# IwakuraRein/CIS-565-Final-VR-Raytracer

Hardware: AMD Instinct MI355X
Metric: Mrays/s (ClosestHit+AnyHit ray queries per second) of the 1080p ReSTIR DI+GI+denoise frame; ms_per_step = ms/frame (higher is better)
Workload: dtype f32

## Files before the change

cis-565-final-vr-raytracer_amd/csrc/dev_scene.h:

```cpp
#pragma once
#include <hip/hip_runtime.h>
#include "bvh8.h"
#include "../../include/rt_abi.h"

namespace rt {

struct DevInstance {
  float o2w[12];
  float w2o[12];
  uint32_t primMesh;
  uint32_t flags;
  uint32_t pad[2];
};

struct DevTexture {
  const uint8_t* bgra;
  int32_t w, h, wrapS, wrapT, filter, pad;
};

struct DevScene {
  const Node8* nodes;
  const Tri48* tris;
  const TriRef* triRef;
  const AlphaRec* alphaRec;
  const AlphaRec* alphaByTri;
  const DevInstance* instances;
  const rt_prim_mesh* primMeshes;
  const rt_vertex* vertices;
  const uint32_t* indices;
  const rt_material* materials;
  const DevTexture* textures;
  const rt_punc_light* puncLights;
  const rt_trig_light* trigLights;
  const float* env;
  const rt_impt_samp* envAccel;
  rt_light_buf_info lightInfo;
  int32_t envW, envH;
  uint32_t numTris, numNodes;
  const struct SkyPre* sky;
  int32_t stackEntries;
  int32_t coopLive;
  float triPad;
  int32_t stackTotal;
  uint2* stackOvf; uint2* stackOvfInd;
  uint32_t stackOvfThreads;
  int32_t gangMax;
};

struct SurfRec {
  rt_vec3 position, normal, ffnormal, emission;
  float roughness, metallic;
  uint32_t matID, seed;
};

struct DevFrame {
  uint4* thisG; const uint4* lastG;
  short2* motion;
  rt_direct_reservoir* thisDirectResv; const rt_direct_reservoir* lastDirectResv;
  rt_indirect_reservoir* thisIndirectResv; const rt_indirect_reservoir* lastIndirectResv;
  uint32_t* thisLightId; const uint32_t* lastLightId;
  float4* thisDirectResult; float4* thisIndirectResult;
  float4* denoiseDirA; float4* denoiseDirB; float4* denoiseIndA; float4* denoiseIndB;
  unsigned long long* counters;
  SurfRec* surf; uint32_t* status; uint32_t* qcount; uint32_t* waveProf;
  float4* geomN; float4* geomP; float4* geomNh; float4* geomPh;
  rt_direct_reservoir* tempDirectResv;
  double* postRowSums; float* postMean;
  float4* postMipD; float4* postMipI;
  uint32_t* tileOrder;
  int32_t W, H;
  int32_t histRow0, histRow1;
  uint32_t* histMiss;
  int32_t stackLds;
  int32_t pad4;
};

struct OmCamera {
  rt_mat4 lastProjView;
  rt_vec3 lastPosition; float pad;
};
struct DevObjMotion {
  uint32_t* instImage;
  const OmCamera* cams;
  uint32_t numInst, pad;
};

}
```

cis-565-final-vr-raytracer_amd/csrc/rt_api.cpp:

```cpp
#include <hip/hip_runtime.h>
#include <array>
#include <atomic>
#include <memory>
#include <mutex>
#include <cmath>
#include <cstdio>
#include <map>
#include <cstdlib>
#include <chrono>
#include <cstring>
#include <string>
#include <thread>
#include <unordered_map>
#include <vector>
#include "../../include/rt_abi.h"
#include "../../include/rt_cpus.h"
#include "bvh8_builder.h"
#include "stages.h"
#include "reference.h"
#include "svgf.h"
#include "gi_spatial.h"
#include "taa.h"
#include "refit.h"
#include "accel_build.h"
// ... 304 lines not shown
  return e;
}

template <class T> static int upload(rt_ctx* c, std::vector<void*>& pool, const T* src, size_t count, const T** out)
{
  void* d = nullptr;
  size_t bytes = std::max<size_t>(count, 1) * sizeof(T);
  RT_HIP(c, hipMalloc(&d, bytes));
  pool.push_back(d);
  if(count && src) RT_HIP(c, hipMemcpy(d, src, count * sizeof(T), hipMemcpyHostToDevice));
  else RT_HIP(c, hipMemset(d, 0, bytes));
  *out = static_cast<const T*>(d);
  return RT_OK;
}
template <class T> static int allocZeroed(rt_ctx* c, std::vector<void*>& pool, size_t count, T** out)
{
  const T* const noSource = nullptr;
  const T* p = nullptr;
  const int rc = upload(c, pool, noSource, count, &p);
  *out = const_cast<T*>(p);
  return rc;
}
static void freePool(std::vector<void*>& pool) { for(void* p : pool) (void)hipFree(p); pool.clear(); }
struct LoadTimer {
  const bool on = getenv("RESTIR_BVH_TIMING") && atoi(getenv("RESTIR_BVH_TIMING")) != 0;
  std::chrono::steady_clock::time_point t = std::chrono::steady_clock::now();
  void lap(const char* what) { if(!on) return; const auto n = std::chrono::steady_clock::now(); fprintf(stderr, "[scene load] %-34s %.3f s\n", what, std::chrono::duration<double>(n - t).count()); t = n; }
};
static int ensureStackOverflow(rt_ctx* c);
static int syncHostVertices(rt_ctx* c, int mesh = -1);
static int allocObjectMotion(rt_ctx* c);
static void reopenPriorityDecision(rt_ctx* c);
static void hashBytes(const void* p, size_t n, uint64_t& h0, uint64_t& h1);
static int stackLdsEnv() { static const int v = getenv("RESTIR_STACK_LDS") ? std::max(2, atoi(getenv("RESTIR_STACK_LDS"))) : 0; return v; }
static int stackLdsMin() { return stackLdsEnv() ? stackLdsEnv() : 6; }

static size_t elemBytes(int id)
{
  switch(id) {
    case RT_BUF_GBUFFER0: case RT_BUF_GBUFFER1: return 16;
    case RT_BUF_MOTION: return 4;
    case RT_BUF_DIRECT_RESV0: case RT_BUF_DIRECT_RESV1: case RT_BUF_DIRECT_RESV_TEMP: return sizeof(rt_direct_reservoir);
    case RT_BUF_INDIRECT_RESV0: case RT_BUF_INDIRECT_RESV1: case RT_BUF_INDIRECT_RESV_TEMP: return sizeof(rt_indirect_reservoir);
    case RT_BUF_LIGHT_ID0: case RT_BUF_LIGHT_ID1: case RT_BUF_LDR: return 4;
    default: return 16;
  }
}
#ifndef RT_WAVEPROF
#define RT_WAVEPROF 0
#endif
static constexpr size_t WAVEPROF_RECORDS = 1 << 17;
static constexpr int RT_PAD_ROWS = 128;
static bool halfRes(int id) { return id == RT_BUF_INDIRECT_RESV0 || id == RT_BUF_INDIRECT_RESV1 || id == RT_BUF_INDIRECT_RESV_TEMP; }

extern "C" {

uint32_t rt_abi_version(void) { return (RT_ABI_VERSION_MAJOR << 16) | RT_ABI_VERSION_MINOR; }

const char* rt_last_error(rt_ctx* ctx) { return ctx ? ctx->err.c_str() : g_createErr.c_str(); }

}
int rtCreateWithLevels(rt_ctx** out, int device, const int* levels);
extern "C" {
int rt_create(rt_ctx** out, int device) { return rtCreateWithLevels(out, device, nullptr); }
}
int rtCreateWithLevels(rt_ctx** out, int device, const int* levels)
{
  if(!out) { g_createErr = "rt_create: out is NULL"; return RT_ERR_INVALID_ARG; }
  *out = nullptr;
  int n = 0;
  if(hipGetDeviceCount(&n) != hipSuccess || n <= 0) { g_createErr = "rt_create: no HIP device (this library has no CPU path)"; return RT_ERR_NO_DEVICE; }
  if(device < 0 || device >= n) { g_createErr = "rt_create: device index out of range"; return RT_ERR_INVALID_ARG; }
  if(hipSetDevice(device) != hipSuccess) { g_createErr = "rt_create: hipSetDevice failed"; return RT_ERR_HIP; }
  rt_ctx* c = new(std::nothrow) rt_ctx();
  if(!c) { g_createErr = "rt_create: out of host memory"; return RT_ERR_OOM; }
  g_liveCtx.fetch_add(1);
  c->device = device;
  {
    prioSpec(c->prio); c->prioFromEnv = getenv("RESTIR_PRIO") != nullptr; c->prioDecided = c->prioFromEnv;
    if(levels) { for(int i = 0; i < 3; i++) c->prio[i] = std::max(-1, std::min(1, levels[i])); c->prioDecided = c->prioExplicit = true; }
    bool ok = createStreamLevel(&c->ownStream, c->prio[0]) == hipSuccess;
    if(!ok) { g_createErr = "rt_create: hipStreamCreate failed"; rt_destroy(c); return RT_ERR_HIP; }
    c->mainIdx = g_streamsCreated.load() - 1;
    c->stream = c->ownStream;
    for(int i = 0; i < 4; i++) {
      ok = ok && hipEventCreateWithFlags(&c->evD[i], hipEventDisableTiming) == hipSuccess;
      ok = ok && hipEventCreateWithFlags(&c->evI[i], hipEventDisableTiming) == hipSuccess;
      ok = ok && hipEventCreateWithFlags(&c->evDone[i], hipEventDisableTiming) == hipSuccess;
    }
    ok = ok && hipEventCreateWithFlags(&c->evFork, hipEventDisableTiming) == hipSuccess;
    ok = ok && hipEventCreateWithFlags(&c->evJoin, hipEventDisableTiming) == hipSuccess;
    if(!ok) { g_createErr = "rt_create: creating the internal events failed"; rt_destroy(c); return RT_ERR_HIP; }
  }
  if(const char* e = getenv("RESTIR_OVERLAP")) c->overlap = atoi(e);
  if(hipMalloc(reinterpret_cast<void**>(&c->dCounters), 8 * sizeof(unsigned long long)) != hipSuccess) { g_createErr = "rt_create: hipMalloc failed"; rt_destroy(c); return RT_ERR_OOM; }
  (void)hipMemset(c->dCounters, 0, 8 * sizeof(unsigned long long));
  *out = c;
  return RT_OK;
}

extern "C" {

int rt_destroy(rt_ctx* c)
{
  if(!c) return RT_ERR_INVALID_ARG;
  (void)hipSetDevice(c->device);
  (void)syncAll(c);
  freePool(c->sceneAllocs); freePool(c->accelAllocs); freePool(c->scratchAllocs); freePool(c->ovfAllocs); freePool(c->rebuildAllocs);
  freePool(c->skinAllocs); freePool(c->deformAllocs);
  for(int i = 0; i < RT_BUF_COUNT; i++) if(c->bufs[i]) (void)hipFree(c->bufs[i]);
  for(void* p : {c->spareG, c->spareMotion, c->spareG2, c->spareMotion2, c->spareDirRes, c->omInst, c->omInstSpare, c->omInstSpare2, c->omTable}) if(p) (void)hipFree(p);
  for(void* p : c->indA) if(p && p != c->bufs[RT_BUF_DENOISE_IND_A]) (void)hipFree(p);
  for(hipStream_t& q : c->indStreams) { if(q) (void)hipStreamDestroy(q); q = nullptr; }
  for(hipStream_t& q : c->sideStreams) { if(q) (void)hipStreamDestroy(q); q = nullptr; }
  c->indStream = c->sideStream = nullptr;
  if(c->indStream) (void)hipStreamDestroy(c->indStream);
  for(int i = 0; i < 4; i++) { if(c->evD[i]) (void)hipEventDestroy(c->evD[i]); if(c->evI[i]) (void)hipEventDestroy(c->evI[i]); if(c->evDone[i]) (void)hipEventDestroy(c->evDone[i]); }
  if(c->dCounters) (void)hipFree(c->dCounters);
  if(c->dSky) (void)hipFree(c->dSky);
  if(c->dPick) (void)hipFree(c->dPick);
  if(c->refAcc) (void)hipFree(c->refAcc);
  if(c->refMean) (void)hipFree(c->refMean);
  freeSvgfHistory(c);
  freeGiSpatial(c);
  freeTaaHistory(c);
  for(auto& E : c->evSets) for(int i = 0; i < rt_ctx::MAX_EV; i++) (void)hipEventDestroy(E.ev[i]);
  if(c->ownStream) (void)hipStreamDestroy(c->ownStream);
  if(c->sideStream) (void)hipStreamDestroy(c->sideStream);
  if(c->evFork) (void)hipEventDestroy(c->evFork);
  if(c->evJoin) (void)hipEventDestroy(c->evJoin);
  for(hipEvent_t e : c->evRefit) if(e) (void)hipEventDestroy(e);
  for(hipEvent_t e : c->evDeform) if(e) (void)hipEventDestroy(e);
  for(hipEvent_t e : c->evRebuild) if(e) (void)hipEventDestroy(e);
  delete c;
  if(g_liveCtx.fetch_sub(1) == 1) { std::lock_guard<std::mutex> one(g_accelMutex); g_accelCache.reset(); }
  return RT_OK;
}

int rt_set_stream(rt_ctx* c, void* s)
{
  if(!c) return RT_ERR_INVALID_ARG;
  c->stream = s ? static_cast<hipStream_t>(s) : c->ownStream;
  return RT_OK;
}

int rt_sync(rt_ctx* c)
{
  if(!c) return RT_ERR_INVALID_ARG;
  RT_HIP(c, hipSetDevice(c->device));
  RT_HIP(c, syncAll(c));
  return RT_OK;
}

int rt_upload_scene(rt_ctx* c, const rt_scene_desc* d)
{
  if(!c) return RT_ERR_INVALID_ARG;
  if(!d || !d->primMeshes || !d->vertices || !d->indices || !d->instances || !d->materials || d->numMaterials == 0)
    return fail(c, RT_ERR_INVALID_ARG, "rt_upload_scene: missing geometry/material arrays");
  for(uint32_t i = 0; i < d->numInstances; i++)
    if(d->instances[i].primMesh >= d->numPrimMeshes) return fail(c, RT_ERR_INVALID_ARG, "rt_upload_scene: instance references a missing prim mesh");
  for(uint32_t i = 0; i < d->numPrimMeshes; i++) {
    const rt_prim_mesh& pm = d->primMeshes[i];
    if(uint64_t(pm.firstIndex) + pm.indexCount > d->numIndices || uint64_t(pm.vertexOffset) + pm.vertexCount > d->numVertices || pm.indexCount % 3 != 0)
      return fail(c, RT_ERR_INVALID_ARG, "rt_upload_scene: prim mesh range out of bounds");
    if(pm.materialIndex >= int32_t(d->numMaterials)) return fail(c, RT_ERR_INVALID_ARG, "rt_upload_scene: material index out of range");
    for(uint32_t k = 0; k < pm.indexCount; k++)
      if(d->indices[pm.firstIndex + k] >= pm.vertexCount) return fail(c, RT_ERR_INVALID_ARG, "rt_upload_scene: vertex index beyond the prim mesh's vertex range");
  }
  const int32_t nTex = d->textures ? int32_t(d->numTextures) : 0;
  for(uint32_t i = 0; i < d->numMaterials; i++) {
    const rt_material& m = d->materials[i];
    const int32_t ids[5] = {m.pbrBaseColorTexture, m.pbrMetallicRoughnessTexture, m.emissiveTexture, m.normalTexture, m.transmissionTexture};
    for(int32_t id : ids)
      if(id < -1 || id >= nTex) return fail(c, RT_ERR_INVALID_ARG, "rt_upload_scene: material references a missing texture");
  }
  if(d->trigLights)
    for(uint32_t i = 0; i < d->lightInfo.trigLightSize; i++)
      if(d->trigLights[i].matIndex >= d->numMaterials || d->trigLights[i].impSamp.alias < 0 || uint32_t(d->trigLights[i].impSamp.alias) >= d->lightInfo.trigLightSize)
        return fail(c, RT_ERR_INVALID_ARG, "rt_upload_scene: triangle light with a bad material or alias index");
  if(d->puncLights)
    for(uint32_t i = 0; i < d->lightInfo.puncLightSize; i++)
      if(d->puncLights[i].impSamp.alias < 0 || uint32_t(d->puncLights[i].impSamp.alias) >= d->lightInfo.puncLightSize)
        return fail(c, RT_ERR_INVALID_ARG, "rt_upload_scene: punctual light with a bad alias index");
  if(d->envRgba32f && d->envAccel && d->envWidth > 0 && d->envHeight > 0) {
    const int64_t n = int64_t(d->envWidth) * d->envHeight;
    for(int64_t i = 0; i < n; i++)
      if(d->envAccel[i].alias < 0 || d->envAccel[i].alias >= n) return fail(c, RT_ERR_INVALID_ARG, "rt_upload_scene: environment alias table entry out of range");
  }
  RT_HIP(c, hipSetDevice(c->device));
  RT_HIP(c, syncAll(c));
  LoadTimer lt;
  freePool(c->sceneAllocs); freePool(c->accelAllocs); freePool(c->rebuildAllocs);
  freePool(c->skinAllocs); freePool(c->deformAllocs);
  c->deform = rt_ctx::Deform{};
  c->refit = rt_ctx::Refit{};
  c->rebuild = rt_ctx::Rebuild{};
  c->haveScene = c->haveAccel = false;
  c->refN = 0;
  c->svgfValid = false;
  c->taaValid = false;
  c->omPrev.clear(); c->omMoved.clear(); c->omPending = false;
  c->ds = DevScene{};
  c->ds.sky = (c->sunAndSky.in_use == 1) ? static_cast<const SkyPre*>(c->dSky) : nullptr;
  c->primMeshes.assign(d->primMeshes, d->primMeshes + d->numPrimMeshes);
  c->vertices.assign(d->vertices, d->vertices + d->numVertices);
  c->indices.assign(d->indices, d->indices + d->numIndices);
  c->instances.assign(d->instances, d->instances + d->numInstances);
  c->materials.assign(d->materials, d->materials + d->numMaterials);

  int rc;
  if((rc = upload(c, c->sceneAllocs, d->primMeshes, d->numPrimMeshes, &c->ds.primMeshes))) return rc;
  if((rc = upload(c, c->sceneAllocs, d->vertices, size_t(d->numVertices), &c->ds.vertices))) return rc;
  if((rc = upload(c, c->sceneAllocs, d->indices, size_t(d->numIndices), &c->ds.indices))) return rc;
  if((rc = upload(c, c->sceneAllocs, d->materials, d->numMaterials, &c->ds.materials))) return rc;
  if((rc = upload(c, c->sceneAllocs, d->puncLights, d->puncLights ? d->lightInfo.puncLightSize : 0, &c->ds.puncLights))) return rc;
  if((rc = upload(c, c->sceneAllocs, d->trigLights, d->trigLights ? d->lightInfo.trigLightSize : 0, &c->ds.trigLights))) return rc;
  c->ds.lightInfo = d->lightInfo;
  if(!d->puncLights) c->ds.lightInfo.puncLightSize = 0;
  if(!d->trigLights) c->ds.lightInfo.trigLightSize = 0;
  lt.lap("geometry copies + uploads");
  c->hostAlpha.clear();
  std::vector<const uint8_t*> alphaSrc;
  std::vector<DevTexture> texs(std::max<uint32_t>(d->numTextures, 1));
  static const uint8_t white[4] = {255, 255, 255, 255};
  for(uint32_t i = 0; i < uint32_t(texs.size()); i++) {
    rt_texture t{white, 1, 1, RT_WRAP_REPEAT, RT_WRAP_REPEAT, RT_FILTER_LINEAR, 0};
    if(i < d->numTextures && d->textures && d->textures[i].bgra8 && d->textures[i].width > 0 && d->textures[i].height > 0) t = d->textures[i];
    const uint8_t* dp = nullptr;
    if((rc = upload(c, c->sceneAllocs, t.bgra8, size_t(t.width) * t.height * 4, &dp))) return rc;
    texs[i] = DevTexture{dp, t.width, t.height, t.wrapS, t.wrapT, t.magFilter, 0};
    c->hostAlpha.emplace_back(size_t(t.width) * t.height);
    alphaSrc.push_back(t.bgra8);
  }
  lt.lap("texture uploads");
  {
    c->alphaHash.assign(c->hostAlpha.size(), {0ull, 0ull});
    std::atomic<size_t> next{0};
    auto work = [&] {
      for(;;) {
        const size_t i = next.fetch_add(1);
        if(i >= c->hostAlpha.size()) return;
        std::vector<uint8_t>& a = c->hostAlpha[i];
        const uint8_t* src = alphaSrc[i];
        for(size_t k = 0; k < a.size(); k++) a[k] = src[k * 4 + 3];
        uint64_t h0 = 0x243F6A8885A308D3ull, h1 = 0x13198A2E03707344ull;
        hashBytes(a.data(), a.size(), h0, h1);
        c->alphaHash[i] = {h0, h1};
      }
    };
    const size_t nt = std::min<size_t>(c->hostAlpha.size(), size_t(rt_cpu_budget()));
    std::vector<std::thread> pool;
    for(size_t k = 1; k < nt; k++) pool.emplace_back(work);
    work();
    for(auto& th : pool) th.join();
  }
  lt.lap("alpha planes + hashes");
  if((rc = upload(c, c->sceneAllocs, texs.data(), texs.size(), &c->ds.textures))) return rc;
  c->devTextures = texs;
  if(d->envRgba32f && d->envWidth > 0 && d->envHeight > 0) {
    const size_t n = size_t(d->envWidth) * d->envHeight;
    if((rc = upload(c, c->sceneAllocs, d->envRgba32f, n * 4, &c->ds.env))) return rc;
    if(d->envAccel) { if((rc = upload(c, c->sceneAllocs, d->envAccel, n, &c->ds.envAccel))) return rc; }
    else {
      std::vector<rt_impt_samp> a(n, rt_impt_samp{0, 1.0f, 0.0f, 0.0f});
      if((rc = upload(c, c->sceneAllocs, a.data(), n, &c->ds.envAccel))) return rc;
    }
    c->ds.envW = d->envWidth; c->ds.envH = d->envHeight;
  } else {
    const float black[4] = {0, 0, 0, 0};
    const rt_impt_samp one{0, 1.0f, 0.0f, 0.0f};
    if((rc = upload(c, c->sceneAllocs, black, 4, &c->ds.env))) return rc;
    if((rc = upload(c, c->sceneAllocs, &one, 1, &c->ds.envAccel))) return rc;
    c->ds.envW = c->ds.envH = 1;
  }
  RT_HIP(c, hipDeviceSynchronize());
  c->haveScene = true;
  reopenPriorityDecision(c);
  return RT_OK;
}


static void hashBytes(const void* p, size_t n, uint64_t& h0, uint64_t& h1)
{
  const unsigned char* b = static_cast<const unsigned char*>(p);
  size_t i = 0;
  for(; i + 8 <= n; i += 8) {
    uint64_t w; memcpy(&w, b + i, 8);
    h0 = (h0 ^ w) * 0x9E3779B97F4A7C15ull; h0 ^= h0 >> 29;
    h1 = (h1 + w) * 0xC2B2AE3D27D4EB4Full; h1 ^= h1 >> 31;
  }
  uint64_t w = 0; memcpy(&w, b + i, n - i); w |= uint64_t(n) << 56;
  h0 = (h0 ^ w) * 0x9E3779B97F4A7C15ull; h0 ^= h0 >> 29;
  h1 = (h1 + w) * 0xC2B2AE3D27D4EB4Full; h1 ^= h1 >> 31;
}
#define RT_HASH_VEC(v) do { const uint64_t n_ = (v).size(); hashBytes(&n_, 8, h0, h1); if(n_) hashBytes((v).data(), n_ * sizeof((v)[0]), h0, h1); } while(0)
static void sceneKey(const rt_ctx* c, uint64_t& h0, uint64_t& h1)
{
  h0 = 0x243F6A8885A308D3ull; h1 = 0x13198A2E03707344ull;
  RT_HASH_VEC(c->primMeshes); RT_HASH_VEC(c->vertices); RT_HASH_VEC(c->indices); RT_HASH_VEC(c->instances); RT_HASH_VEC(c->materials);
  for(size_t i = 0; i < c->devTextures.size(); i++) {
    const DevTexture& t = c->devTextures[i];
    const int meta[5] = {t.w, t.h, t.wrapS, t.wrapT, t.filter};
    hashBytes(meta, sizeof(meta), h0, h1);
    if(i < c->alphaHash.size()) { const uint64_t n_ = c->hostAlpha[i].size(); hashBytes(&n_, 8, h0, h1); hashBytes(c->alphaHash[i].data(), 16, h0, h1); }
  }
  for(const char* name : {"RESTIR_BVH_SPLIT", "RESTIR_BVH_SPLIT_BUDGET", "RESTIR_BVH_SPLIT_ALPHA", "RESTIR_BVH_SPLIT_WORK", "RESTIR_BVH_ROTATE", "RESTIR_BVH_ROTATE_GG",
                           "RESTIR_BVH_REINSERT", "RESTIR_BVH_PAR_MIN", "RESTIR_BVH_SEQ_MAX"}) {
    const char* v = getenv(name);
    hashBytes(name, strlen(name), h0, h1);
    if(v) hashBytes(v, strlen(v) + 1, h0, h1);
  }
}
#undef RT_HASH_VEC
static int buildHostAccel(rt_ctx* c, HostAccel& out)
{
  LoadTimer lt;
  rt_scene_desc d{};
  d.numPrimMeshes = uint32_t(c->primMeshes.size()); d.primMeshes = c->primMeshes.data();
  d.numVertices = c->vertices.size(); d.vertices = c->vertices.data();
  d.numIndices = c->indices.size(); d.indices = c->indices.data();
  d.numInstances = uint32_t(c->instances.size()); d.instances = c->instances.data();
  BuildOutput& bo = out.bo;
  int threads = rt_cpu_budget();
  if(!buildBvh8(d, bo, threads > 0 ? threads : 1)) return fail(c, RT_ERR_INVALID_ARG, "rt_build_accel: BVH8 build failed");
  if(bo.maxDepth > STACK_MAX) {
    bo = BuildOutput{};
    if(!buildBvh8(d, bo, threads > 0 ? threads : 1, true)) return fail(c, RT_ERR_INVALID_ARG, "rt_build_accel: BVH8 build failed");
  }
  if(bo.maxDepth > STACK_MAX) return fail(c, RT_ERR_INVALID_ARG, "rt_build_accel: BVH8 deeper than the traversal stack");
  lt.lap("buildBvh8");
  std::vector<AlphaRec>& alpha = out.alpha; alpha.assign(1, AlphaRec{});
  std::vector<int32_t>& alphaTex = out.alphaTex; alphaTex.assign(1, -1);
  struct KeyHash { size_t operator()(const std::array<uint32_t, 12>& k) const { uint64_t h = 1469598103934665603ull; for(uint32_t w : k) { h ^= w; h *= 1099511628211ull; } return size_t(h ^ (h >> 29)); } };
  std::unordered_map<std::array<uint32_t, 12>, std::array<uint32_t, 4>, KeyHash> ommCache;
  ommCache.reserve(1 << 16);
  std::vector<uint32_t> alphaOf;
  if(bo.tris.size() > bo.triRef.size()) alphaOf.assign(bo.triRef.size(), 0u);
  std::vector<std::array<uint32_t, 4>> ommOf;
  for(Tri48& T : bo.tris) {
    if(T.flags & TRI_OPAQUE) continue;
    if(!alphaOf.empty() && alphaOf[T.globalId]) { T.alphaIdx = alphaOf[T.globalId]; memcpy(T.omm, ommOf[T.alphaIdx].data(), sizeof(T.omm)); continue; }
    const TriRef ref = bo.triRef[T.globalId];
    const rt_prim_mesh& pm = c->primMeshes[c->instances[ref.inst].primMesh];
    const rt_material& m = c->materials[size_t(pm.materialIndex > 0 ? pm.materialIndex : 0)];
    const uint32_t* ix = &c->indices[pm.firstIndex + 3 * ref.prim];
    AlphaRec a{};
    int32_t tex = -1;
    const rt_vec2 t0 = c->vertices[pm.vertexOffset + ix[0]].texcoord, t1 = c->vertices[pm.vertexOffset + ix[1]].texcoord, t2 = c->vertices[pm.vertexOffset + ix[2]].texcoord;
    a.uv0x = t0.x; a.uv0y = t0.y; a.uv1x = t1.x; a.uv1y = t1.y; a.uv2x = t2.x; a.uv2y = t2.y;
    a.baseAlpha = m.pbrBaseColorFactor.w; a.cutoff = m.alphaCutoff; a.alphaMode = m.alphaMode;
    if(m.pbrBaseColorTexture > -1 && size_t(m.pbrBaseColorTexture) < c->devTextures.size()) {
      const DevTexture& t = c->devTextures[size_t(m.pbrBaseColorTexture)];
      tex = m.pbrBaseColorTexture; a.w = t.w; a.h = t.h; a.wrapS = t.wrapS; a.wrapT = t.wrapT; a.filter = t.filter;
    }
    T.alphaIdx = uint32_t(alpha.size());
    alpha.push_back(a); alphaTex.push_back(tex);
    std::array<uint32_t, 12> key{};
    memcpy(key.data(), &a.uv0x, 8 * sizeof(float));
    key[8] = uint32_t(m.pbrBaseColorTexture); key[9] = uint32_t(a.alphaMode); key[10] = uint32_t(a.wrapS) ^ (uint32_t(a.wrapT) << 16); key[11] = uint32_t(a.filter);
    auto it = ommCache.find(key);
    if(it == ommCache.end()) {
      std::array<uint32_t, 4> o{};
      const std::vector<uint8_t>* al = (tex >= 0 && size_t(tex) < c->hostAlpha.size()) ? &c->hostAlpha[size_t(m.pbrBaseColorTexture)] : nullptr;
      buildOpacityMap(a, al, o.data());
      it = ommCache.emplace(key, o).first;
    }
    memcpy(T.omm, it->second.data(), sizeof(T.omm));
    if(!alphaOf.empty()) { alphaOf[T.globalId] = T.alphaIdx; ommOf.resize(alpha.size()); ommOf[T.alphaIdx] = it->second; }
  }
  lt.lap("alpha records + micro-maps");
  return RT_OK;
}

int rt_build_accel(rt_ctx* c)
{
  if(!c) return RT_ERR_INVALID_ARG;
  if(!c->haveScene) return fail(c, RT_ERR_NO_SCENE, "rt_build_accel: no scene uploaded");
  RT_HIP(c, hipSetDevice(c->device));
  RT_HIP(c, syncAll(c));
  { const int rc = syncHostVertices(c); if(rc) return rc; }
  freePool(c->accelAllocs); freePool(c->rebuildAllocs);
  c->refit = rt_ctx::Refit{};
  c->rebuild = rt_ctx::Rebuild{};
  c->haveAccel = false;
  c->refN = 0;
  c->svgfValid = false;
  c->taaValid = false;
  std::shared_ptr<const HostAccel> ha;
  LoadTimer lt;
  {
    std::lock_guard<std::mutex> one(g_accelMutex);
    uint64_t k0, k1;
    sceneKey(c, k0, k1);
    lt.lap("scene key");
    if(g_accelCache && g_accelCache->key0 == k0 && g_accelCache->key1 == k1) ha = g_accelCache;
    else {
      auto fresh = std::make_shared<HostAccel>();
      fresh->key0 = k0; fresh->key1 = k1;
      const int rc = buildHostAccel(c, *fresh);
      if(rc) return rc;
      ha = fresh; g_accelCache = ha;
    }
  }
  lt.lap("host products (build or cache)");
  const BuildOutput& bo = ha->bo;
  int rc;
  {
    std::vector<AlphaRec> alpha = ha->alpha;
    for(size_t i = 0; i < alpha.size(); i++) if(ha->alphaTex[i] >= 0) alpha[i].bgra = c->devTextures[size_t(ha->alphaTex[i])].bgra;
    if((rc = upload(c, c->accelAllocs, alpha.data(), alpha.size(), &c->ds.alphaRec))) return rc;
    std::vector<AlphaRec> byTri(bo.tris.size(), AlphaRec{});
    for(size_t i = 0; i < bo.tris.size(); i++) if(!(bo.tris[i].flags & TRI_OPAQUE)) byTri[i] = alpha[bo.tris[i].alphaIdx];
    if((rc = upload(c, c->accelAllocs, byTri.data(), byTri.size(), &c->ds.alphaByTri))) return rc;
  }
  if((rc = upload(c, c->accelAllocs, bo.nodes.data(), bo.nodes.size(), &c->ds.nodes))) return rc;
  if((rc = upload(c, c->accelAllocs, bo.tris.data(), bo.tris.size(), &c->ds.tris))) return rc;
  if((rc = upload(c, c->accelAllocs, bo.triRef.data(), bo.triRef.size(), &c->ds.triRef))) return rc;
  if((rc = upload(c, c->accelAllocs, bo.instances.data(), bo.instances.size(), &c->ds.instances))) return rc;
  c->ds.numNodes = uint32_t(bo.nodes.size()); c->ds.numTris = uint32_t(bo.tris.size());
  c->ds.stackTotal = std::max(8, ((bo.maxDepth + 1 + 3) / 4) * 4);
  c->ds.stackEntries = c->ds.stackTotal;
  c->ds.triPad = bo.pad;
  { const char* e = getenv("RESTIR_COOP"); c->ds.coopLive = e ? std::max(0, std::min(64, atoi(e))) : 4; }
  { const char* e = getenv("RESTIR_GANG"); c->ds.gangMax = e ? std::max(0, std::min(7, atoi(e))) : 4; }
  c->numNodes = bo.nodes.size(); c->numTris = bo.triRef.size(); c->maxDepth = bo.maxDepth;
  c->numRefs = bo.tris.size(); c->spatialSplits = size_t(bo.spatialSplits); c->sahNodeSteps = bo.sahNodeSteps; c->sahTriSteps = bo.sahTriSteps;
  RT_HIP(c, hipDeviceSynchronize());
  lt.lap("uploads (tree, alpha records)");
  c->haveAccel = true;
  reopenPriorityDecision(c);
  return ensureStackOverflow(c);
}

int rt_resize(rt_ctx* c, int w, int h)
{
  if(!c) return RT_ERR_INVALID_ARG;
  if(w <= 0 || h <= 0 || w > 32767 || h > 32767) return fail(c, RT_ERR_INVALID_ARG, "rt_resize: size must be in 1..32767 (RG16_SINT motion vectors)");
  RT_HIP(c, hipSetDevice(c->device));
  RT_HIP(c, syncAll(c));
  reopenPriorityDecision(c);
  for(void*& p : c->indA) { if(p && p != c->bufs[RT_BUF_DENOISE_IND_A]) (void)hipFree(p); p = nullptr; }
  for(int i = 0; i < RT_BUF_COUNT; i++) { if(c->bufs[i]) (void)hipFree(c->bufs[i]); c->bufs[i] = nullptr; c->bufBytes[i] = 0; }
  for(void** p : {&c->spareG, &c->spareMotion, &c->spareG2, &c->spareMotion2, &c->spareDirRes}) if(*p) { (void)hipFree(*p); *p = nullptr; }
  c->W = c->H = 0;
  for(void* p : {static_cast<void*>(c->refAcc), static_cast<void*>(c->refMean)}) if(p) (void)hipFree(p);
  c->refAcc = nullptr; c->refMean = nullptr; c->refN = 0;
  freeSvgfHistory(c);
  freeGiSpatial(c);
  freeTaaHistory(c);
  freeObjectMotion(c);
  const size_t n = size_t(w) * h, nh = size_t(w / 2) * (h / 2);
  for(int i = 0; i < RT_BUF_COUNT; i++) {
    const size_t bytes = (halfRes(i) ? nh : n) * elemBytes(i);
    const size_t alloc = bytes + (halfRes(i) ? size_t(w / 2) * (RT_PAD_ROWS / 2) : size_t(w) * RT_PAD_ROWS) * elemBytes(i) + 16;
    RT_HIP(c, hipMalloc(&c->bufs[i], alloc));
    RT_HIP(c, hipMemset(c->bufs[i], (i == RT_BUF_LIGHT_ID0 || i == RT_BUF_LIGHT_ID1) ? 0xff : 0, alloc));
    c->bufBytes[i] = bytes; c->bufAlloc[i] = alloc;
    if(i == RT_BUF_DENOISE_IND_A) {
      c->indA[0] = c->bufs[i];
      RT_HIP(c, hipMalloc(&c->indA[1], alloc));
      RT_HIP(c, hipMemset(c->indA[1], 0, alloc));
    }
    if(i == RT_BUF_GBUFFER0 || i == RT_BUF_MOTION) {
      for(void** spare : {(i == RT_BUF_MOTION) ? &c->spareMotion : &c->spareG, (i == RT_BUF_MOTION) ? &c->spareMotion2 : &c->spareG2}) {
        RT_HIP(c, hipMalloc(spare, alloc));
        RT_HIP(c, hipMemset(*spare, 0, alloc));
      }
    }
    if(i == RT_BUF_DIRECT_RESULT0) {
      RT_HIP(c, hipMalloc(&c->spareDirRes, alloc));
      RT_HIP(c, hipMemset(c->spareDirRes, 0, alloc));
    }
  }
  freePool(c->scratchAllocs);
  c->scratch = DevFrame{};
  auto alloc = [&](size_t bytes, void** out) -> int {
    RT_HIP(c, hipMalloc(out, std::max<size_t>(bytes, 256)));
    c->scratchAllocs.push_back(*out);
    RT_HIP(c, hipMemset(*out, 0, std::max<size_t>(bytes, 256)));
    return RT_OK;
  };
  DevFrame& X = c->scratch;
  int rc;
#define RT_SCRATCH(field, count, T) if((rc = alloc(size_t(count) * sizeof(T), reinterpret_cast<void**>(&X.field)))) return rc
  RT_SCRATCH(surf, n, SurfRec); RT_SCRATCH(status, n, uint32_t); RT_SCRATCH(qcount, 256, uint32_t);
  RT_SCRATCH(geomN, n, float4); RT_SCRATCH(geomP, n, float4); RT_SCRATCH(geomNh, nh, float4); RT_SCRATCH(geomPh, nh, float4);
  RT_SCRATCH(postRowSums, size_t(h) * 6, double); RT_SCRATCH(postMean, 8, float);
  RT_SCRATCH(postMipD, n + 64, float4); RT_SCRATCH(postMipI, n + 64, float4);
  RT_SCRATCH(tileOrder, (size_t(w / 2 + 7) / 8) * (size_t(h / 2 + 7) / 8 + 16 * 2) + 64 + 4096, uint32_t);
#if RT_WAVEPROF
  RT_SCRATCH(waveProf, WAVEPROF_RECORDS * 16, uint32_t);
#endif
#undef RT_SCRATCH
  RT_HIP(c, hipDeviceSynchronize());
  c->W = w; c->H = h;
  if(c->objMotion != RT_OBJECT_MOTION_OFF && (rc = allocObjectMotion(c))) return rc;
  return ensureStackOverflow(c);
}

static int ensureStackOverflow(rt_ctx* c)
{
  freePool(c->ovfAllocs);
  c->ds.stackOvf = c->ds.stackOvfInd = nullptr; c->ds.stackOvfThreads = 0;
  if(!(stackLdsEnv() || c->overlap >= 2)) return RT_OK;
  if(!c->haveAccel || c->W <= 0 || c->ds.stackTotal <= stackLdsMin()) return RT_OK;
  const size_t tilesX = size_t(c->W + 7) / 8, tilesY = size_t(c->H + 7) / 8;
  const size_t blocks = std::max<size_t>(16384, tilesX * tilesY + 8 * tilesX + 1024);
  const size_t bytes = blocks * 64 * size_t(c->ds.stackTotal - stackLdsMin()) * sizeof(uint2);
  void* p[2] = {nullptr, nullptr};
  for(int i = 0; i < 2; i++) { RT_HIP(c, hipMalloc(&p[i], bytes)); c->ovfAllocs.push_back(p[i]); }
  c->ds.stackOvf = static_cast<uint2*>(p[0]); c->ds.stackOvfInd = static_cast<uint2*>(p[1]);
  c->ds.stackOvfThreads = uint32_t(blocks * 64);
  return RT_OK;
}

int rt_set_camera(rt_ctx* c, const rt_scene_camera* cam)
{
  if(!c || !cam) return RT_ERR_INVALID_ARG;
  if(std::memcmp(&c->cam.viewInverse, &cam->viewInverse, sizeof(rt_mat4)) != 0 || std::memcmp(&c->cam.projInverse, &cam->projInverse, sizeof(rt_mat4)) != 0) c->refN = 0;
  c->cam = *cam;
  return RT_OK;
}

static void selectFrame(rt_ctx* c, int frames) { if(c->indA[0]) c->bufs[RT_BUF_DENOISE_IND_A] = c->indA[frames & 1]; }

static hipError_t ensureOverlapStreams(rt_ctx* c)
{
  if(c->sideStream && c->indStream) return hipSuccess;
  hipError_t e = hipSuccess;
  hipStream_t& side = c->sideStreams[c->prio[2] + 1];
  hipStream_t& ind = c->indStreams[c->prio[1] + 1];
  if(!side) { e = createStreamLevel(&side, c->prio[2]); if(e == hipSuccess) c->sideIdx[c->prio[2] + 1] = g_streamsCreated.load() - 1; }
  if(e == hipSuccess && !ind) { e = createStreamLevel(&ind, c->prio[1]); if(e == hipSuccess) c->indIdx[c->prio[1] + 1] = g_streamsCreated.load() - 1; }
  c->sideStream = side; c->indStream = ind;
  return e;
}

static constexpr float PRIO_FILTER_SHARE = 0.30f;
static int prioProbeFrames() { static const int n = getenv("RESTIR_PRIO_PROBE") ? std::max(1, atoi(getenv("RESTIR_PRIO_PROBE"))) : 3; return n; }
static void reopenPriorityDecision(rt_ctx* c)
{
  if(c->prioExplicit || c->prioFromEnv) return;
  c->prioDecided = false; c->filterShare = -1.f; c->probeFrames = 0; c->denoiseSeen = -1;
  c->prio[1] = 1; c->prio[2] = 0;
  c->indStream = c->sideStream = nullptr;
}

static int allocSvgfHistory(rt_ctx* c)
{
  const size_t n = size_t(c->W) * c->H, nh = size_t(c->W / 2) * (c->H / 2);
  const size_t bytes[4] = {n * sizeof(float4), nh * sizeof(float4), n * sizeof(float2), nh * sizeof(float2)};
  for(auto& par : c->svgfHist)
    for(int k = 0; k < 4; k++) {
      if(hipMalloc(&par[k], std::max<size_t>(bytes[k], 256)) != hipSuccess) { par[k] = nullptr; freeSvgfHistory(c); return fail(c, RT_ERR_OOM, "rt_render_frame: hipMalloc of the SVGF history failed"); }
      RT_HIP(c, hipMemset(par[k], 0, std::max<size_t>(bytes[k], 256)));
    }
  RT_HIP(c, hipDeviceSynchronize());
  c->svgfValid = false; c->svgfParity = -1;
  return RT_OK;
}

static SvgfArgs svgfArgs(const rt_ctx* c, const DevFrame& F, const rt_state& st, int frames, bool ind, bool histValid)
{
  SvgfArgs A{};
  const int cur = frames & 1, prev = (frames + 1) & 1, k = ind ? 1 : 0;
  A.thisG = F.thisG; A.lastG = F.lastG; A.motion = F.motion;
  A.noisy = ind ? F.denoiseIndA : F.thisDirectResult;
  A.bufA = ind ? F.thisIndirectResult : F.denoiseDirA;
  A.bufB = ind ? F.denoiseIndA : F.denoiseDirB;
  A.out = ind ? F.denoiseIndB : F.thisDirectResult;
  A.geomN = ind ? F.geomNh : F.geomN; A.geomP = ind ? F.geomPh : F.geomP;
  A.prevC = static_cast<const float4*>(c->svgfHist[prev][k]); A.prevM = static_cast<const float2*>(c->svgfHist[prev][2 + k]);
  A.histC = static_cast<float4*>(c->svgfHist[cur][k]); A.histM = static_cast<float2*>(c->svgfHist[cur][2 + k]);
  A.W = c->W; A.H = c->H;
  A.bx = ind ? c->W / 2 : c->W; A.by = ind ? c->H / 2 : c->H;
  A.histValid = histValid ? 1 : 0;
  A.cap = c->den.historyCap;
  A.alphaC = c->den.alphaColor; A.alphaM = c->den.alphaMoments;
  A.phiLum = ind ? c->den.phiLumIndirect : c->den.phiLumDirect;
  A.sigN = ind ? st.sigNormalIndirect : st.sigNormalDirect;
  A.sigD = ind ? st.sigDepthIndirect : st.sigDepthDirect;
  return A;
}

static int allocGiSpatial(rt_ctx* c)
{
  const size_t bytes = std::max<size_t>(size_t(c->W / 2) * (c->H / 2) * sizeof(rt_indirect_reservoir), 256);
  if(hipMalloc(&c->gisResv, bytes) != hipSuccess) { c->gisResv = nullptr; return fail(c, RT_ERR_OOM, "rt_render_frame: hipMalloc of the GI spatial reservoirs failed"); }
  RT_HIP(c, hipMemset(c->gisResv, 0, bytes));
  RT_HIP(c, hipDeviceSynchronize());
  c->gisWritten = false;
  return RT_OK;
}

static GiSpatialArgs giSpatialArgs(const rt_ctx* c, const DevFrame& F)
{
  GiSpatialArgs A{};
  A.thisG = F.thisG; A.resv = F.thisIndirectResv;
  A.out = static_cast<rt_indirect_reservoir*>(c->gisResv);
  A.indA = F.denoiseIndA;
  A.W = c->W; A.H = c->H;
  A.mode = c->gis.mode; A.samples = c->gis.samples; A.radius = c->gis.radius;
  A.normalThreshold = c->gis.normalThreshold; A.depthThreshold = c->gis.depthThreshold; A.jacobianMax = c->gis.jacobianMax;
  return A;
}

static int allocObjectMotion(rt_ctx* c)
{
  const size_t bytes = size_t(c->W) * c->H * sizeof(uint32_t);
  for(void** p : {&c->omInst, &c->omInstSpare, &c->omInstSpare2}) {
    if(*p) continue;
    RT_HIP(c, hipMalloc(p, std::max<size_t>(bytes, 256)));
    RT_HIP(c, hipMemset(*p, 0xff, std::max<size_t>(bytes, 256)));
  }
  RT_HIP(c, hipDeviceSynchronize());
  return RT_OK;
}
static int allocTaaHistory(rt_ctx* c)
{
  const size_t n = size_t(c->W) * c->H;
  const size_t bytes[3] = {n * sizeof(float4), n * sizeof(float4), n * sizeof(float)};
  for(auto& par : c->taaHist)
    for(int k = 0; k < 3; k++) {
      if(hipMalloc(&par[k], std::max<size_t>(bytes[k], 256)) != hipSuccess) { par[k] = nullptr; freeTaaHistory(c); return fail(c, RT_ERR_OOM, "rt_render_frame: hipMalloc of the TAA history failed"); }
      RT_HIP(c, hipMemset(par[k], 0, std::max<size_t>(bytes[k], 256)));
    }
  RT_HIP(c, hipDeviceSynchronize());
  c->taaValid = false; c->taaLast = -1; c->taaHeld[0] = c->taaHeld[1] = false;
  return RT_OK;
}

static TaaArgs taaArgs(const rt_ctx* c, const DevFrame& F, int frames, bool histValid)
{
  TaaArgs A{};
  const int cur = frames & 1, prev = (frames + 1) & 1;
  A.thisG = F.thisG; A.lastG = F.lastG;
  A.curD = F.thisDirectResult; A.curI = F.thisIndirectResult;
  A.prevD = static_cast<const float4*>(c->taaHist[prev][0]); A.prevI = static_cast<const float4*>(c->taaHist[prev][1]);
  A.prevN = static_cast<const float*>(c->taaHist[prev][2]);
  A.outD = static_cast<float4*>(c->taaHist[cur][0]); A.outI = static_cast<float4*>(c->taaHist[cur][1]); A.outN = static_cast<float*>(c->taaHist[cur][2]);
  A.W = c->W; A.H = c->H;
  A.histValid = histValid ? 1 : 0;
  A.alpha = c->taa.alpha; A.clipGamma = c->taa.clipGamma;
  return A;
}

static DevFrame makeFrame(rt_ctx* c, int frames)
{
  selectFrame(c, frames);
  const int cur = frames & 1, last = (frames + 1) & 1;
  DevFrame F{};
  F.stackLds = stackLdsEnv() ? stackLdsEnv() : (c->overlap >= 2 ? 6 : 0);
  F.thisG = static_cast<uint4*>(c->bufs[RT_BUF_GBUFFER0 + cur]); F.lastG = static_cast<const uint4*>(c->bufs[RT_BUF_GBUFFER0 + last]);
  F.motion = static_cast<short2*>(c->bufs[RT_BUF_MOTION]);
  F.thisDirectResv = static_cast<rt_direct_reservoir*>(c->bufs[RT_BUF_DIRECT_RESV0 + cur]);
  F.lastDirectResv = static_cast<const rt_direct_reservoir*>(c->bufs[RT_BUF_DIRECT_RESV0 + last]);
  F.thisIndirectResv = static_cast<rt_indirect_reservoir*>(c->bufs[RT_BUF_INDIRECT_RESV0 + cur]);
  F.lastIndirectResv = static_cast<const rt_indirect_reservoir*>(c->bufs[RT_BUF_INDIRECT_RESV0 + last]);
  F.tempDirectResv = static_cast<rt_direct_reservoir*>(c->bufs[RT_BUF_DIRECT_RESV_TEMP]);
  F.thisLightId = static_cast<uint32_t*>(c->bufs[RT_BUF_LIGHT_ID0 + cur]); F.lastLightId = static_cast<const uint32_t*>(c->bufs[RT_BUF_LIGHT_ID0 + last]);
  F.thisDirectResult = static_cast<float4*>(c->bufs[RT_BUF_DIRECT_RESULT0 + cur]);
  F.thisIndirectResult = static_cast<float4*>(c->bufs[RT_BUF_INDIRECT_RESULT0 + cur]);
  F.denoiseDirA = static_cast<float4*>(c->bufs[RT_BUF_DENOISE_DIR_A]); F.denoiseDirB = static_cast<float4*>(c->bufs[RT_BUF_DENOISE_DIR_B]);
  F.denoiseIndA = static_cast<float4*>(c->bufs[RT_BUF_DENOISE_IND_A]); F.denoiseIndB = static_cast<float4*>(c->bufs[RT_BUF_DENOISE_IND_B]);
  F.counters = c->counting ? c->dCounters : nullptr;
  F.W = c->W; F.H = c->H;
  const DevFrame& X = c->scratch;
  F.surf = X.surf; F.status = X.status; F.qcount = X.qcount; F.waveProf = X.waveProf;
  F.histRow0 = c->histRow0; F.histRow1 = c->histRow1; F.histMiss = X.qcount + 250;
  F.geomN = X.geomN; F.geomP = X.geomP; F.geomNh = X.geomNh; F.geomPh = X.geomPh; F.tileOrder = X.tileOrder; F.postRowSums = X.postRowSums; F.postMean = X.postMean;
  return F;
}

static int checkReady(rt_ctx* c, const rt_state* st)
{
  if(!c || !st) return RT_ERR_INVALID_ARG;
  if(!c->haveScene) return fail(c, RT_ERR_NO_SCENE, "no scene uploaded");
  if(!c->haveAccel) return fail(c, RT_ERR_NO_ACCEL, "rt_build_accel has not been called");
  if(c->W == 0 || st->size.x != c->W || st->size.y != c->H) return fail(c, RT_ERR_NO_TARGET, "RtxState.size does not match rt_resize");
  return RT_OK;
}

int rt_run_stage(rt_ctx* c, const rt_state* st, int frames, int stage, int level, int rowBegin, int rowEnd)
{
  int rc = checkReady(c, st);
  if(rc) return rc;
  if(stage < 0 || stage >= RT_STAGE_COUNT) return fail(c, RT_ERR_INVALID_ARG, "rt_run_stage: unknown stage");
  if(c->den.mode == RT_DENOISER_SVGF && (stage == RT_STAGE_DENOISE_DIRECT || stage == RT_STAGE_DENOISE_INDIRECT))
    return fail(c, RT_ERR_INVALID_ARG, "rt_run_stage: the denoise stages are the A-Trous chain; this context is in SVGF mode (rt_set_denoiser), which only rt_render_frame runs");
  if(c->gis.mode != RT_GI_SPATIAL_OFF && stage == RT_STAGE_INDIRECT)
    return fail(c, RT_ERR_INVALID_ARG, "rt_run_stage: this context has GI spatial reuse on (rt_set_gi_spatial), whose pass after the indirect stage only rt_render_frame runs");
  if(c->taa.mode != RT_TAA_OFF)
    return fail(c, RT_ERR_INVALID_ARG, "rt_run_stage: this context has TAA on (rt_set_taa), whose jittered camera and resolve pass only rt_render_frame runs");
  if(rowBegin < 0 || (rowBegin & 7)) return fail(c, RT_ERR_INVALID_ARG, "rt_run_stage: rowBegin must be a non-negative multiple of 8");
  {
    const bool spatial = st->ReSTIRState == RT_RESTIR_SPATIAL || st->ReSTIRState == RT_RESTIR_SPATIOTEMPORAL;
    const int maxLevel = stage == RT_STAGE_DENOISE_DIRECT ? 3 : (stage == RT_STAGE_DENOISE_INDIRECT ? 4 : ((stage == RT_STAGE_DIRECT && spatial) ? 2 : 0));
    if(level < 0 || level > maxLevel)
      return fail(c, RT_ERR_INVALID_ARG, "rt_run_stage: level out of range for this stage (RT_STAGE_DIRECT levels 1 / 2 exist in the spatial modes only)");
  }
  RT_HIP(c, hipSetDevice(c->device));
  RT_HIP(c, joinInFlight(c));
  DevFrame F = makeFrame(c, frames);
  if(stage == RT_STAGE_INDIRECT) F.histMiss = c->scratch.qcount + 251;
  const hipError_t e = stageLauncher(c, *st, stage, rowBegin, rowEnd)(c->stream, c->ds, F, *st, c->cam, stage, level, rowBegin, rowEnd);
  if(e == hipErrorInvalidValue) return fail(c, RT_ERR_INVALID_ARG, "rt_run_stage: level out of range for this stage (RT_STAGE_DIRECT levels 1 / 2 exist in the spatial modes only)");
  if(e == hipErrorInvalidConfiguration) return fail(c, RT_ERR_HIP, "rt_run_stage: the traversal-stack overflow area is missing or too small for this launch (internal sizing error)");
  RT_HIP(c, e);
  return RT_OK;
}

int rt_render_frame(rt_ctx* c, const rt_state* st, int frames)
{
  int rc = checkReady(c, st);
  if(rc) return rc;
  RT_HIP(c, hipSetDevice(c->device));
  if(c->evUsed == rt_ctx::MAX_SETS) { RT_HIP(c, syncAll(c)); harvestTimings(c); }
  if(c->evUsed == c->evSets.size()) {
    rt_ctx::EvSet E{};
    for(int i = 0; i < rt_ctx::MAX_EV; i++) RT_HIP(c, hipEventCreate(&E.ev[i]));
    c->evSets.push_back(E);
  }
  if(c->prioDecided && !c->prioExplicit && !c->prioFromEnv && c->denoiseSeen >= 0 && (st->denoise > 0) != (c->denoiseSeen > 0)) { RT_HIP(c, syncAll(c)); reopenPriorityDecision(c); }
  const bool svgf = c->den.mode == RT_DENOISER_SVGF && st->denoise > 0;
  if(svgf && !c->svgfHist[0][0]) { RT_HIP(c, syncAll(c)); if((rc = allocSvgfHistory(c))) return rc; }
  const bool gis = c->gis.mode != RT_GI_SPATIAL_OFF;
  if(gis && !c->gisResv) { RT_HIP(c, syncAll(c)); if((rc = allocGiSpatial(c))) return rc; }
  const bool taa = c->taa.mode == RT_TAA_ON && st->debugging_mode == 0;
  if(taa && !c->taaHist[0][0]) { RT_HIP(c, syncAll(c)); if((rc = allocTaaHistory(c))) return rc; }
  rt_scene_camera cam = c->cam;
  if(taa) (void)rt_taa_jitter_camera(&c->cam, frames, c->taa.jitterPhases, c->W, c->H, &cam);
  const bool om = c->objMotion == RT_OBJECT_MOTION_ON && !c->counting && c->omInst;
  bool omMotion = false;
  if(c->objMotion == RT_OBJECT_MOTION_ON) {
    const size_t nInst = c->instances.size();
    if(c->omPending) for(size_t i = 0; i < nInst && !omMotion; i++) omMotion = c->omMoved[i] && std::memcmp(c->omPrev[i].data(), c->instances[i].objectToWorld, 48) != 0;
    if(omMotion && c->counting)
      return fail(c, RT_ERR_INVALID_ARG, "rt_render_frame: instances are in motion with object motion vectors on (rt_set_object_motion) and counting on (rt_set_counting): the counting build has no object-motion form");
    if(omMotion) {
      if(c->omTableRows < nInst) {
        RT_HIP(c, syncAll(c));
        if(c->omTable) { (void)hipFree(c->omTable); c->omTable = nullptr; c->omTableRows = 0; }
        RT_HIP(c, hipMalloc(&c->omTable, nInst * sizeof(OmCamera)));
        c->omTableRows = nInst;
      }
      c->omHost.resize(nInst);
      for(size_t i = 0; i < nInst; i++) {
        rt_scene_camera ci = cam;
        if(c->omMoved[i]) (void)rt_object_motion_camera(&cam, c->omPrev[i].data(), c->instances[i].objectToWorld, &ci);
        c->omHost[i].lastProjView = ci.lastProjView; c->omHost[i].lastPosition = ci.lastPosition; c->omHost[i].pad = 0.f;
      }
    }
  }
  const bool decide = c->overlap >= 2 && !c->prioDecided && c->spareG && c->spareMotion;
  if(decide) { RT_HIP(c, syncAll(c)); harvestTimings(c); }
  const double tracedBefore = c->accStage[RT_STAGE_DIRECT] + c->accStage[RT_STAGE_INDIRECT];
  const double filterBefore = c->accStage[RT_STAGE_DENOISE_DIRECT] + c->accStage[RT_STAGE_DENOISE_INDIRECT] + c->accStage[RT_STAGE_COMPOSE];
  rt_ctx::EvSet& E = c->evSets[c->evUsed];
  if(c->overlap >= 1 && !decide) RT_HIP(c, ensureOverlapStreams(c));
  const bool pipelined = !decide && c->overlap >= 2 && c->sideStream && c->indStream && c->spareG && c->spareMotion;
  if(pipelined) {
    if(c->overlap >= 3 && c->spareG2 && c->spareMotion2 && c->spareDirRes) {
      void*& g = c->bufs[RT_BUF_GBUFFER0 + (frames & 1)]; void* t = g; g = c->spareG; c->spareG = c->spareG2; c->spareG2 = t;
      void*& m = c->bufs[RT_BUF_MOTION]; t = m; m = c->spareMotion; c->spareMotion = c->spareMotion2; c->spareMotion2 = t;
      if(c->omInst) { t = c->omInst; c->omInst = c->omInstSpare; c->omInstSpare = c->omInstSpare2; c->omInstSpare2 = t; }
      std::swap(c->bufs[RT_BUF_DIRECT_RESULT0 + (frames & 1)], c->spareDirRes);
    } else {
      std::swap(c->bufs[RT_BUF_GBUFFER0 + (frames & 1)], c->spareG);
      std::swap(c->bufs[RT_BUF_MOTION], c->spareMotion);
      if(c->omInst) std::swap(c->omInst, c->omInstSpare);
    }
  } else {
    RT_HIP(c, joinInFlight(c));
  }
  const DevFrame F = makeFrame(c, frames);
  const DevObjMotion OM{static_cast<uint32_t*>(c->omInst), omMotion ? static_cast<const OmCamera*>(c->omTable) : nullptr, uint32_t(c->instances.size()), 0u};
  int k = 0, lastMain = 0, lastSide = 0, lastInd = 0;
  auto record = [&](hipStream_t strm, int stage) -> int {
    const hipError_t e = hipEventRecord(E.ev[k], strm);
    if(e != hipSuccess) { c->err = std::string("hipEventRecord: ") + hipGetErrorString(e); return RT_ERR_HIP; }
    int& last = (strm == c->stream) ? lastMain : (strm == c->indStream ? lastInd : lastSide);
    E.stage[k] = stage; E.prev[k] = last; last = k; k++;
    return RT_OK;
  };
  auto run = [&](hipStream_t strm, int stage, int level) -> int {
    hipError_t e = (om && (stage == RT_STAGE_DIRECT || stage == RT_STAGE_INDIRECT)) ? omStageLauncher(c, *st, stage)(strm, c->ds, F, OM, *st, cam, stage, level, 0, 0)
                                                                                     : stageLauncher(c, *st, stage, 0, 0)(strm, c->ds, F, *st, cam, stage, level, 0, 0);
    if(e != hipSuccess) { c->err = std::string("launchStage: ") + hipGetErrorString(e); return RT_ERR_HIP; }
    return record(strm, stage);
  };
  auto direct = [&](hipStream_t strm) -> int {
    if(om && omMotion) RT_HIP(c, hipMemcpyAsync(c->omTable, c->omHost.data(), c->omHost.size() * sizeof(OmCamera), hipMemcpyHostToDevice, strm));
    const int r = run(strm, RT_STAGE_DIRECT, 0);
    if(r == RT_OK) {
      if(om) c->omInstValid = true;
      if(c->omPending) { std::fill(c->omMoved.begin(), c->omMoved.end(), uint8_t(0)); c->omPending = false; }
    }
    return r;
  };
  SvgfArgs svgfA[2] = {};
  if(svgf) {
    const bool histOk = c->svgfValid && c->svgfParity == ((frames + 1) & 1);
    svgfA[0] = svgfArgs(c, F, *st, frames, false, histOk);
    svgfA[1] = svgfArgs(c, F, *st, frames, true, histOk);
    c->svgfParity = frames & 1;
  }
  if(st->denoise == 0 || svgf) c->svgfValid = false;
  auto svgfEnqueued = [&]() { if(svgf) c->svgfValid = true; };
  auto filters = [&](hipStream_t strm, bool ind) -> int {
    const int stage = ind ? RT_STAGE_DENOISE_INDIRECT : RT_STAGE_DENOISE_DIRECT;
    int r;
    if(!svgf) {
      for(int i = 0; i < (ind ? 5 : 4); i++) if((r = run(strm, stage, i))) return r;
      return RT_OK;
    }
    for(int s = 0; s < svgfSteps(ind); s++) {
      const hipError_t e = launchSvgfStep(strm, svgfA[ind ? 1 : 0], cam, ind, s);
      if(e != hipSuccess) { c->err = std::string("launchSvgfStep: ") + hipGetErrorString(e); return RT_ERR_HIP; }
      if((r = record(strm, stage))) return r;
    }
    return RT_OK;
// ... 774 lines not shown
  if(int rc = needTree(c, "rt_update_instances")) return rc;
  if(count && (!ids || !xf)) return fail(c, RT_ERR_INVALID_ARG, "rt_update_instances: NULL ids / matrices");
  const size_t nInst = c->instances.size();
  std::vector<DevInstance> rows(count);
  std::vector<uint8_t> flip(count, 0);
  {
    std::vector<bool> seen(nInst, false);
    for(uint32_t k = 0; k < count; k++) {
      if(ids[k] >= nInst) return fail(c, RT_ERR_INVALID_ARG, "rt_update_instances: instance id out of range");
      if(seen[ids[k]]) return fail(c, RT_ERR_INVALID_ARG, "rt_update_instances: duplicate instance id");
      seen[ids[k]] = true;
      for(int a = 0; a < 12; a++) if(!std::isfinite(xf[12 * k + a])) return fail(c, RT_ERR_INVALID_ARG, "rt_update_instances: non-finite matrix entry");
      DevInstance& di = rows[k];
      memcpy(di.o2w, xf + 12 * k, sizeof(di.o2w));
      float det;
      inverseAffine(di.o2w, di.w2o, &det);
      if(!(det != 0.0f) || !std::isfinite(det)) return fail(c, RT_ERR_INVALID_ARG, "rt_update_instances: singular matrix");
      for(int a = 0; a < 12; a++) if(!std::isfinite(di.w2o[a])) return fail(c, RT_ERR_INVALID_ARG, "rt_update_instances: the matrix has no finite inverse");
      di.primMesh = c->instances[ids[k]].primMesh; di.flags = c->instances[ids[k]].flags; di.pad[0] = di.pad[1] = 0;
      flip[k] = det < 0.0f;
    }
  }
  RT_HIP(c, hipSetDevice(c->device));
  RT_HIP(c, syncAll(c));
  int rc;
  if((rc = ensureRefitState(c))) return rc;
  rt_ctx::Refit& R = c->refit;
  for(uint32_t k = 0; k < count; k++) if((rc = syncHostVertices(c, int(c->instances[ids[k]].primMesh)))) return rc;
  std::vector<uint8_t> moved(nInst, 0);
  if(c->omPrev.size() != nInst) { c->omPrev.assign(nInst, std::array<float, 12>{}); c->omMoved.assign(nInst, 0); c->omPending = false; }
  for(uint32_t k = 0; k < count; k++) {
    const uint32_t i = ids[k];
    if(!c->omMoved[i]) {
      memcpy(c->omPrev[i].data(), c->instances[i].objectToWorld, sizeof(rows[k].o2w));
      c->omMoved[i] = 1; c->omPending = true;
    }
    memcpy(c->instances[i].objectToWorld, rows[k].o2w, sizeof(rows[k].o2w));
    R.inst[i] = rows[k];
    R.instMax[i] = instanceCoordMax(c, i, rows[k].o2w);
    R.flip[i] = flip[k];
    moved[i] = 1;
  }
  hipStream_t s = c->stream;
  RT_HIP(c, hipEventRecord(c->evRefit[0], s));
  DevInstance* dInst = const_cast<DevInstance*>(c->ds.instances);
  if(count * 4 > nInst) RT_HIP(c, hipMemcpyAsync(dInst, R.inst.data(), nInst * sizeof(DevInstance), hipMemcpyHostToDevice, s));
  else for(uint32_t k = 0; k < count; k++) RT_HIP(c, hipMemcpyAsync(dInst + ids[k], &rows[k], sizeof(DevInstance), hipMemcpyHostToDevice, s));
  return refitTail(c, moved);
}

int rt_update_lights(rt_ctx* c, const rt_trig_light* trig, uint32_t numTrig, const rt_punc_light* punc, uint32_t numPunc, const rt_light_buf_info* info)
{
  if(!c) return RT_ERR_INVALID_ARG;
  if(!c->haveScene) return fail(c, RT_ERR_NO_SCENE, "rt_update_lights: no scene uploaded");
  if(!info || numTrig != c->ds.lightInfo.trigLightSize || numPunc != c->ds.lightInfo.puncLightSize || info->trigLightSize != numTrig || info->puncLightSize != numPunc)
    return fail(c, RT_ERR_INVALID_ARG, "rt_update_lights: the light counts must equal the uploaded ones");
  if((numTrig && !trig) || (numPunc && !punc)) return fail(c, RT_ERR_INVALID_ARG, "rt_update_lights: NULL light array");
  for(uint32_t i = 0; i < numTrig; i++)
    if(trig[i].matIndex >= c->materials.size() || trig[i].impSamp.alias < 0 || uint32_t(trig[i].impSamp.alias) >= numTrig)
      return fail(c, RT_ERR_INVALID_ARG, "rt_update_lights: triangle light with a bad material or alias index");
  for(uint32_t i = 0; i < numPunc; i++)
    if(punc[i].impSamp.alias < 0 || uint32_t(punc[i].impSamp.alias) >= numPunc) return fail(c, RT_ERR_INVALID_ARG, "rt_update_lights: punctual light with a bad alias index");
  RT_HIP(c, hipSetDevice(c->device));
  RT_HIP(c, syncAll(c));
  if(numTrig) RT_HIP(c, hipMemcpy(const_cast<rt_trig_light*>(c->ds.trigLights), trig, numTrig * sizeof(rt_trig_light), hipMemcpyHostToDevice));
  if(numPunc) RT_HIP(c, hipMemcpy(const_cast<rt_punc_light*>(c->ds.puncLights), punc, numPunc * sizeof(rt_punc_light), hipMemcpyHostToDevice));
  c->ds.lightInfo.trigSampProb = info->trigSampProb;
  c->refN = 0;
  return RT_OK;
}

int rt_rebuild_accel(rt_ctx* c)
{
  if(int rc = needTree(c, "rt_rebuild_accel")) return rc;
  RT_HIP(c, hipSetDevice(c->device));
  RT_HIP(c, syncAll(c));
  int rc;
  if((rc = ensureRefitState(c))) return rc;
  rt_ctx::Refit& R = c->refit;
  rt_ctx::Rebuild& B = c->rebuild;
  const uint32_t n = uint32_t(c->numTris);
  hipStream_t s = c->stream;
  if(!B.ready) {
    const hipError_t e = accelBuildAlloc(B.work, B.set, n, c->rebuildAllocs);
    if(e != hipSuccess) {
      freePool(c->rebuildAllocs); B = rt_ctx::Rebuild{};
      c->err = std::string("rt_rebuild_accel: ") + hipGetErrorString(e);
      return e == hipErrorOutOfMemory ? RT_ERR_OOM : RT_ERR_HIP;
    }
    hipError_t e1 = launchAccelTable(s, c->ds.tris, c->ds.numTris, B.work);
    for(hipEvent_t& e2 : c->evRebuild) if(e1 == hipSuccess && !e2) e1 = hipEventCreate(&e2);
    if(e1 != hipSuccess) {
      (void)hipStreamSynchronize(s);
      freePool(c->rebuildAllocs); B = rt_ctx::Rebuild{};
      c->err = std::string("rt_rebuild_accel: ") + hipGetErrorString(e1);
      return e1 == hipErrorOutOfMemory ? RT_ERR_OOM : RT_ERR_HIP;
    }
    B.ready = true;
  }
  const float triPad = triPadOf(R.instMax);
  const std::vector<uint32_t> flipBits = instanceBits(c->instances.size(), [&](size_t i) { return R.flip[i] != 0; });
  const size_t words = flipBits.size();
  const std::vector<uint32_t> all(words, 0xffffffffu);
  rt_rebuild_stats st{};
  st.triangles = n; st.triPad = triPad;
  RT_HIP(c, hipEventRecord(c->evRebuild[0], s));
  if(n > 0) {
    const int target = B.cur == 0 ? 1 : 0;
    const AccelBuildSet& T = B.set[target];
    RT_HIP(c, hipMemcpyAsync(R.dDirty, all.data(), words * 4, hipMemcpyHostToDevice, s));
    RT_HIP(c, hipMemcpyAsync(R.dFlip, flipBits.data(), words * 4, hipMemcpyHostToDevice, s));
    RT_HIP(c, hipMemsetAsync(R.dCounters, 0, 16, s));
    RefitArgs a{};
    a.nodes = T.nodes; a.tris = T.tris; a.triRef = c->ds.triRef; a.instances = c->ds.instances;
    a.primMeshes = c->ds.primMeshes; a.vertices = c->ds.vertices; a.indices = c->ds.indices;
    a.dirtyBits = R.dDirty; a.flipBits = R.dFlip; a.recNode = T.recNode; a.nodeDirty = B.work.nodeDirty; a.counters = R.dCounters;
    a.numRecs = n; a.pad = triPad; a.full = 1;
    AccelBuildResult res;
    hipError_t he = hipSuccess;
    const int br = accelBuildRun(s, B.work, T, a, c->ds.alphaRec, STACK_MAX, c->evRebuild + 1, res, &he);
    if(br == ACCEL_BUILD_HIP) { c->err = std::string("rt_rebuild_accel: ") + hipGetErrorString(he); return he == hipErrorOutOfMemory ? RT_ERR_OOM : RT_ERR_HIP; }
    if(br == ACCEL_BUILD_TOO_DEEP) return fail(c, RT_ERR_INVALID_ARG, "rt_rebuild_accel: BVH8 deeper than the traversal stack");
    if(br != ACCEL_BUILD_OK) { c->err = std::string("rt_rebuild_accel: ") + accelBuildWhy(br); return RT_ERR_HIP; }
    RT_HIP(c, hipEventRecord(c->evRebuild[3], s));
    RT_HIP(c, hipStreamSynchronize(s));
    const int depth = int(res.levels.size());
    const int stackTotal = std::max(8, ((depth + 1 + 3) / 4) * 4);
    const DevScene old = c->ds;
    c->ds.nodes = T.nodes; c->ds.tris = T.tris; c->ds.alphaByTri = T.alphaByTri;
    c->ds.numNodes = res.nodes; c->ds.numTris = n;
    if(stackTotal != old.stackTotal) {
      c->ds.stackTotal = stackTotal; c->ds.stackEntries = stackTotal;
      if((rc = ensureStackOverflow(c))) {
        const std::string msg = c->err;
        c->ds = old; c->ds.stackOvf = c->ds.stackOvfInd = nullptr; c->ds.stackOvfThreads = 0;
        (void)ensureStackOverflow(c);
        c->err = msg;
        return rc;
      }
    }
    B.cur = target;
    c->ds.triPad = triPad;
    c->numNodes = res.nodes; c->numRefs = n; c->spatialSplits = 0; c->maxDepth = depth;
    c->sahNodeSteps = c->sahTriSteps = 0;
    R.levels = res.levels; R.dRecNode = T.recNode; R.dNodeDirty = B.work.nodeDirty; R.treePad = triPad;
    st.nodes = res.nodes; st.levels = uint32_t(depth); st.maxDepth = uint32_t(depth);
    (void)hipEventElapsedTime(&st.ms, c->evRebuild[0], c->evRebuild[3]);
    (void)hipEventElapsedTime(&st.sortMs, c->evRebuild[1], c->evRebuild[2]);
  } else {
    st.nodes = uint32_t(c->numNodes); st.levels = st.maxDepth = uint32_t(c->maxDepth);
  }
  c->refN = 0;
  B.stats = st;
  return RT_OK;
}

int rt_get_rebuild_stats(rt_ctx* c, rt_rebuild_stats* out)
{
  if(!c || !out) return RT_ERR_INVALID_ARG;
  *out = c->rebuild.stats;
  return RT_OK;
}

int rt_get_refit_stats(rt_ctx* c, rt_refit_stats* out)
{
  if(!c || !out) return RT_ERR_INVALID_ARG;
  *out = c->refit.stats;
  return RT_OK;
}

int rt_accel_readback(rt_ctx* c, int which, void* dst, size_t bytes)
{
  if(!c) return RT_ERR_INVALID_ARG;
  if(!c->haveAccel) return fail(c, RT_ERR_NO_ACCEL, "rt_accel_readback: rt_build_accel has not run");
  const void* src = nullptr; size_t want = 0;
  switch(which) {
    case RT_ACCEL_NODES: src = c->ds.nodes; want = size_t(c->ds.numNodes) * sizeof(Node8); break;
    case RT_ACCEL_TRIS: src = c->ds.tris; want = size_t(c->ds.numTris) * sizeof(Tri48); break;
    case RT_ACCEL_INSTANCES: src = c->ds.instances; want = c->instances.size() * sizeof(DevInstance); break;
    default: return fail(c, RT_ERR_INVALID_ARG, "rt_accel_readback: which must be RT_ACCEL_NODES / _TRIS / _INSTANCES");
  }
  if(bytes != want || (want && !dst)) return fail(c, RT_ERR_INVALID_ARG, "rt_accel_readback: size mismatch");
  RT_HIP(c, hipSetDevice(c->device));
  RT_HIP(c, syncAll(c));
  if(want) RT_HIP(c, hipMemcpy(dst, src, want, hipMemcpyDeviceToHost));
  return RT_OK;
}

}

static int syncHostVertices(rt_ctx* c, int mesh)
{
  rt_ctx::Deform& D = c->deform;
  for(size_t k = 0; k < D.skins.size(); k++) {
    if(!D.stale[k] || (mesh >= 0 && uint32_t(mesh) != D.skins[k].primMesh)) continue;
    const rt_prim_mesh& pm = c->primMeshes[D.skins[k].primMesh];
    if(pm.vertexCount) RT_HIP(c, hipMemcpy(c->vertices.data() + pm.vertexOffset, c->ds.vertices + pm.vertexOffset, size_t(pm.vertexCount) * sizeof(rt_vertex), hipMemcpyDeviceToHost));
    D.stale[k] = 0;
  }
  return RT_OK;
}

static int ensureDeformBuffers(rt_ctx* c)
{
  rt_ctx::Deform& D = c->deform;
  if(D.dOut) return RT_OK;
  const size_t nInst = c->instances.size();
  int rc;
  if((rc = allocZeroed(c, c->deformAllocs, std::max<size_t>(nInst, 1), &D.dCoordJobs))) return rc;
  if((rc = allocZeroed(c, c->deformAllocs, nInst + 1, &D.dOut))) return rc;
  for(hipEvent_t& e : c->evDeform) if(!e) RT_HIP(c, hipEventCreate(&e));
  return RT_OK;
}

static int deformRefit(rt_ctx* c, const char* who, const std::vector<uint32_t>& meshes, const std::vector<SkinJob>* skinJobs, const std::vector<uint32_t>* skinIds,
                       uint32_t verticesWritten, uint32_t bytesCopied)
{
  rt_ctx::Refit& R = c->refit;
  rt_ctx::Deform& D = c->deform;
  const size_t nInst = c->instances.size();
  hipStream_t s = c->stream;
  std::vector<uint8_t> deformed(c->primMeshes.size(), 0);
  for(uint32_t m : meshes) deformed[m] = 1;
  std::vector<CoordJob> jobs;
  std::vector<uint8_t> dirty(nInst, 0);
  uint32_t threads = 0;
  for(uint32_t i = 0; i < nInst; i++) {
    const uint32_t m = c->instances[i].primMesh;
    if(!deformed[m]) continue;
    dirty[i] = 1;
    const rt_prim_mesh& pm = c->primMeshes[m];
    CoordJob j{};
    j.threadBase = threads; j.indexCount = pm.indexCount; j.firstIndex = pm.firstIndex; j.instance = i;
    j.vertexBase = skinJobs ? D.restFirst[size_t(D.skinOfMesh[m])] : pm.vertexOffset;
    jobs.push_back(j);
    threads += (pm.indexCount + 63u) & ~63u;
  }
  std::vector<uint32_t> out(jobs.size() + 1, 0u);
  if(!skinJobs) RT_HIP(c, hipMemsetAsync(D.dOut, 0, 4, s));
  if(!jobs.empty()) {
    RT_HIP(c, hipMemsetAsync(D.dOut + 1, 0, jobs.size() * 4, s));
    RT_HIP(c, hipMemcpyAsync(D.dCoordJobs, jobs.data(), jobs.size() * sizeof(CoordJob), hipMemcpyHostToDevice, s));
    CoordMaxArgs ca{};
    ca.vertices = skinJobs ? D.dStaged : c->ds.vertices; ca.indices = c->ds.indices; ca.instances = c->ds.instances; ca.jobs = D.dCoordJobs;
    ca.numJobs = uint32_t(jobs.size()); ca.numThreads = threads; ca.out = D.dOut + 1;
    RT_HIP(c, launchInstCoordMax(s, ca));
  }
  RT_HIP(c, hipMemcpyAsync(out.data(), D.dOut, out.size() * 4, hipMemcpyDeviceToHost, s));
  RT_HIP(c, hipStreamSynchronize(s));
  if(skinJobs && out[0] != 0u) { c->err = std::string(who) + ": the pose yields a non-finite position"; return RT_ERR_INVALID_ARG; }
  if(skinJobs) {
    for(size_t k = 0; k < skinJobs->size(); k++) {
      const SkinJob& j = (*skinJobs)[k];
      const rt_prim_mesh& pm = c->primMeshes[D.skins[(*skinIds)[k]].primMesh];
      if(j.count) RT_HIP(c, hipMemcpyAsync(const_cast<rt_vertex*>(c->ds.vertices) + pm.vertexOffset, D.dStaged + j.restFirst, size_t(j.count) * sizeof(rt_vertex), hipMemcpyDeviceToDevice, s));
      D.stale[(*skinIds)[k]] = 1;
    }
    RT_HIP(c, hipEventRecord(c->evDeform[1], s));
  }
  for(size_t k = 0; k < jobs.size(); k++) memcpy(&R.instMax[jobs[k].instance], &out[1 + k], 4);
  if(const int rc = refitTail(c, dirty)) return rc;
  D.stats = rt_deform_stats{};
  D.stats.meshes = uint32_t(meshes.size()); D.stats.vertices = verticesWritten; D.stats.instances = uint32_t(jobs.size()); D.stats.vertexBytesCopied = bytesCopied;
  D.stats.ms = R.stats.ms;
  if(skinJobs) (void)hipEventElapsedTime(&D.stats.skinMs, c->evDeform[0], c->evDeform[1]);
  return RT_OK;
}

extern "C" {

int rt_update_vertices(rt_ctx* c, uint32_t primMesh, uint32_t firstVertex, uint32_t count, const rt_vertex* rows)
{
  if(int rc = needTree(c, "rt_update_vertices")) return rc;
  if(primMesh >= c->primMeshes.size()) return fail(c, RT_ERR_INVALID_ARG, "rt_update_vertices: prim mesh out of range");
  const rt_prim_mesh& pm = c->primMeshes[primMesh];
  if(uint64_t(firstVertex) + count > pm.vertexCount) return fail(c, RT_ERR_INVALID_ARG, "rt_update_vertices: vertex range outside the prim mesh");
  if(count && !rows) return fail(c, RT_ERR_INVALID_ARG, "rt_update_vertices: NULL rows");
  if(!c->deform.skinOfMesh.empty() && c->deform.skinOfMesh[primMesh] >= 0) return fail(c, RT_ERR_INVALID_ARG, "rt_update_vertices: the prim mesh has a skin");
  const size_t base = size_t(pm.vertexOffset) + firstVertex;
  for(uint32_t k = 0; k < count; k++) {
    const rt_vertex& v = rows[k];
    if(!std::isfinite(v.position.x) || !std::isfinite(v.position.y) || !std::isfinite(v.position.z)) return fail(c, RT_ERR_INVALID_ARG, "rt_update_vertices: non-finite position");
    if(memcmp(&v.texcoord, &c->vertices[base + k].texcoord, sizeof(rt_vec2)) != 0)
      return fail(c, RT_ERR_INVALID_ARG, "rt_update_vertices: texcoord differs from the uploaded row (alpha records and micro-maps were derived from it)");
  }
  RT_HIP(c, hipSetDevice(c->device));
  RT_HIP(c, syncAll(c));
  int rc;
  if((rc = ensureRefitState(c))) return rc;
  if((rc = ensureDeformBuffers(c))) return rc;
  hipStream_t s = c->stream;
  RT_HIP(c, hipEventRecord(c->evRefit[0], s));
  std::vector<uint32_t> meshes;
  if(count) {
    memcpy(c->vertices.data() + base, rows, size_t(count) * sizeof(rt_vertex));
    RT_HIP(c, hipMemcpyAsync(const_cast<rt_vertex*>(c->ds.vertices) + base, c->vertices.data() + base, size_t(count) * sizeof(rt_vertex), hipMemcpyHostToDevice, s));
    meshes.push_back(primMesh);
  }
  return deformRefit(c, "rt_update_vertices", meshes, nullptr, nullptr, count, count * uint32_t(sizeof(rt_vertex)));
}

int rt_set_skins(rt_ctx* c, uint32_t numSkins, const rt_skin* skins, uint64_t numInfluences, const rt_skin_influence* influences)
{
  if(!c) return RT_ERR_INVALID_ARG;
  if(!c->haveScene) return fail(c, RT_ERR_NO_SCENE, "rt_set_skins: no scene uploaded");
  if(numSkins && !skins) return fail(c, RT_ERR_INVALID_ARG, "rt_set_skins: NULL skins");
  std::vector<int32_t> skinOfMesh(c->primMeshes.size(), -1);
// ... 159 lines not shown
```

cis-565-final-vr-raytracer_amd/csrc/shading.h:

```cpp
#pragma once
#include "traverse.h"
#include "sky.h"
#ifndef RT_SKY
#define RT_SKY 0
#endif

namespace rt {

RT_DEV uint32_t tea(uint32_t val0, uint32_t val1)
{
  uint32_t v0 = val0, v1 = val1, s0 = 0;
#pragma unroll
  for(uint32_t n = 0; n < 16; n++) {
    s0 += 0x9e3779b9u;
    v0 += ((v1 << 4) + 0xa341316cu) ^ (v1 + s0) ^ ((v1 >> 5) + 0xc8013ea4u);
    v1 += ((v0 << 4) + 0xad90777du) ^ (v0 + s0) ^ ((v0 >> 5) + 0x7e95761eu);
  }
  return v0;
}

constexpr float M_PI_F = 3.14159265358979323846f;
constexpr float M_1_OVER_PI_F = 0.318309886183790671538f;
constexpr float InvalidPdf = -1.0f;
constexpr float Pi = M_PI_F;
// ... 71 lines not shown
  if((nv.x < 3.402823466e+38f) && !rt_isinf(nv.x)) {
    const float d = 32767.0f / ((rt_abs(nv.x) + rt_abs(nv.y)) + rt_abs(nv.z));
    int x = rt_ftoi(rintf(nv.x * d));
    int y = rt_ftoi(rintf(nv.y * d));
    if(nv.z < 0.0f) {
      const int maskx = x >> 31, masky = y >> 31;
      const int tmp = 32767 + maskx + masky;
      const int tmpx = x;
      x = (tmp - (y ^ masky)) ^ maskx;
      y = (tmp - (tmpx ^ maskx)) ^ masky;
    }
    uint32_t packed = (uint32_t(y + 32767) << 16) | (uint32_t(x + 32767) & 0xffffu);
    if(packed == ~0u) return ~0x1u;
    return packed;
  }
  return ~0u;
}
RT_DEV float short_to_floatm11(int v)
{
  return (v >= 0) ? (rt_u2f(0x3F800000u | (uint32_t(v) << 8)) - 1.0f) : (rt_u2f((0x80000000u | 0x3F800000u) | (uint32_t(-v) << 8)) + 1.0f);
}
RT_DEV f3 decompress_unit_vec(uint32_t packed)
{
  if(packed != ~0u) {
    int x = int(packed & 0xFFFFu) - 32767;
    int y = int(packed >> 16) - 32767;
    const int maskx = x >> 31, masky = y >> 31;
    const int tmp0 = 32767 + maskx + masky;
    const int ymask = y ^ masky;
    const int tmp1 = tmp0 - (x ^ maskx);
    const int z = tmp1 - ymask;
    float zf;
    if(z < 0) {
      x = (tmp0 - ymask) ^ maskx;
      y = tmp1 ^ masky;
      zf = rt_u2f((0x80000000u | 0x3F800000u) | (uint32_t(-z) << 8)) + 1.0f;
    } else {
      zf = rt_u2f(0x3F800000u | (uint32_t(z) << 8)) - 1.0f;
    }
    return normalize(mk3(short_to_floatm11(x), short_to_floatm11(y), zf));
  }
  return mk3(3.402823466e+38f);
}

RT_DEV float resvToScalar(f3 x) { return luminance(x); }
RT_DEV bool resvInvalidW(float w) { return rt_isnan(w) || w < 0.0f; }

RT_DEV m3 localRefMatrix(f3 n)
{
  f3 t = (rt_abs(n.y) > 0.9999f) ? mk3(0.0f, 0.0f, 1.0f) : mk3(0.0f, 1.0f, 0.0f);
  f3 b = normalize(cross(n, t));
  t = cross(b, n);
  return m3{t, b, n};
}
RT_DEV f3 localToWorld(f3 n, f3 v) { return normalize(mul(localRefMatrix(n), v)); }
RT_DEV f3 sampleHemisphereCosine(f3 n, f2 r)
{
  f2 d = toConcentricDisk(r);
  float z = rt_sqrt(1.0f - dot(d, d));
  return localToWorld(n, mk3(d.x, d.y, z));
}
RT_DEV float satDot(f3 a, f3 b) { return rt_max(dot(a, b), 0.0f); }
RT_DEV float absDot(f3 a, f3 b) { return rt_abs(dot(a, b)); }
RT_DEV f3 FresnelSchlick(float cosTheta, f3 f0)
{
  float cos4 = 1.0f - cosTheta;
  cos4 *= cos4;
  cos4 *= cos4;
  return mix(f0, mk3(1.0f), cos4 * (1.0f - cosTheta));
}
RT_DEV float SchlickG(float cosTheta, float alpha) { float a = alpha * 0.5f; return cosTheta / (cosTheta * (1.0f - a) + a); }
RT_DEV float SmithG(float cosWo, float cosWi, float alpha) { return SchlickG(rt_abs(cosWo), alpha) * SchlickG(rt_abs(cosWi), alpha); }
RT_DEV float GTR2Distrib(float cosTheta, float alpha)
{
  if(cosTheta < 1e-6f) return 0.0f;
  float aa = alpha * alpha;
  float nom = aa;
  float denom = cosTheta * cosTheta * (aa - 1.0f) + 1.0f;
  denom = denom * denom * Pi;
  return nom / denom;
}
RT_DEV float GTR2Pdf(f3 n, f3 m, f3 wo, float alpha)
{
  return GTR2Distrib(dot(n, m), alpha) * SchlickG(dot(n, wo), alpha) * absDot(m, wo) / absDot(n, wo);
}
RT_DEV f3 GTR2Sample(f3 n, f3 wo, float alpha, f2 r)
{
  m3 transMat = localRefMatrix(n);
  m3 transInv = inverse(transMat);
  f3 vh = normalize(mul(transInv, wo) * mk3(alpha, alpha, 1.0f));
  float lenSq = vh.x * vh.x + vh.y * vh.y;
  f3 t = lenSq > 0.0f ? mk3(-vh.y, vh.x, 0.0f) / rt_sqrt(lenSq) : mk3(1.0f, 0.0f, 0.0f);
  f3 b = cross(vh, t);
  f2 p = toConcentricDisk(r);
  float s = 0.5f * (vh.z + 1.0f);
  p.y = (1.0f - s) * rt_sqrt(1.0f - p.x * p.x) + s * p.y;
  f3 h = (t * p.x + b * p.y) + vh * rt_sqrt(rt_max(0.0f, 1.0f - dot(p, p)));
  h = mk3(h.x * alpha, h.y * alpha, rt_max(0.0f, h.z));
  return normalize(mul(transMat, h));
}
RT_DEV f3 metallicWorkflowBSDF(const Material& mat, f3 n, f3 wo, f3 wi)
{
  f3 baseColor = mat.albedo;
  float alpha = mat.roughness, metallic = mat.metallic;
  f3 h = normalize(wo + wi);
  float cosO = dot(n, wo), cosI = dot(n, wi);
  if(cosI * cosO < 1e-7f) return mk3(0.0f);
  f3 f = FresnelSchlick(dot(h, wo), mix(mk3(.08f), baseColor, metallic));
  float g = SmithG(cosO, cosI, alpha);
  float d = GTR2Distrib(dot(n, h), alpha);
  return mix(baseColor * PiInv * (1.0f - metallic), mk3(g * d / (4.0f * cosI * cosO)), f);
}
RT_DEV float metallicWorkflowPdf(const Material& mat, f3 n, f3 wo, f3 wi)
{
  float alpha = mat.roughness, metallic = mat.metallic;
  f3 h = normalize(wo + wi);
  return mixf(satDot(n, wi) * PiInv, GTR2Pdf(n, h, wo, alpha) / (4.0f * absDot(h, wo)), 1.0f / (2.0f - metallic));
}
RT_DEV float metallicWorkflowSample(const Material& mat, f3 n, f3 wo, f3 r, f3& bsdf, f3& dir)
{
  float alpha = mat.roughness, metallic = mat.metallic;
  if(r.z > (1.0f / (2.0f - metallic))) dir = sampleHemisphereCosine(n, mk2(r.x, r.y));
  else {
    f3 h = GTR2Sample(n, wo, alpha, mk2(r.x, r.y));
    dir = -reflect(wo, h);
  }
  if(dot(n, dir) < 0.0f) return InvalidPdf;
  bsdf = metallicWorkflowBSDF(mat, n, wo, dir);
  return metallicWorkflowPdf(mat, n, wo, dir);
}

struct Ctx {
  const DevScene& S;
  const rt_state& rtx;
  const rt_scene_camera& cam;
  uint2* stack;
  uint32_t seed;
  i2 imageCoords;
  RayHit hit;
  uint32_t lastLightId;
  TravCounters tc;
  uint32_t nClosest, nAny, nShaded, nRis;

  RT_DEV Ctx(const DevScene& s, const rt_state& r, const rt_scene_camera& c, uint2* st)
      : S(s), rtx(r), cam(c), stack(st), seed(0), imageCoords{0, 0}, lastLightId(0xffffffffu), tc{0, 0}, nClosest(0), nAny(0), nShaded(0), nRis(0)
  {
    hit.t = RT_INFINITY; hit.gid = 0xffffffffu; hit.u = hit.v = 0.f;
  }

#if RT_WAVEPROF
  uint32_t cycClosest = 0, cycAny = 0;
  RT_DEV void ClosestHit(const Ray& r) { nClosest++; const uint64_t c0 = clock64(); traceRay<false>(S, r.origin, r.direction, RT_INFINITY, seed, stack, hit, tc); cycClosest += uint32_t(clock64() - c0); }
  RT_DEV bool AnyHit(const Ray& r, float maxDist) { nAny++; RayHit h; const uint64_t c0 = clock64(); const bool f = traceRay<true>(S, r.origin, r.direction, maxDist, seed, stack, h, tc); cycAny += uint32_t(clock64() - c0); return f; }
#else
  RT_DEV void ClosestHit(const Ray& r) { nClosest++; traceRay<false>(S, r.origin, r.direction, RT_INFINITY, seed, stack, hit, tc); }
  RT_DEV bool AnyHit(const Ray& r, float maxDist) { nAny++; RayHit h; return traceRay<true>(S, r.origin, r.direction, maxDist, seed, stack, h, tc); }
#endif

  RT_DEV static f4 SRGBtoLINEAR(f4 c) { return mk4(rt_pow(c.x, 2.2f), rt_pow(c.y, 2.2f), rt_pow(c.z, 2.2f), c.w); }
  RT_DEV void GetMaterials(State& state, const Ray& r) const
  {
    const rt_material material = S.materials[state.matID];
    m3 TBN{state.tangent, state.bitangent, state.normal};
    if(material.normalTexture > -1) {
      f3 normalVector = xyz(sampleTexture(S, material.normalTexture, state.texCoord));
      normalVector = normalize(normalVector * 2.0f - mk3(1.0f));
      normalVector = normalVector * mk3(material.normalTextureScale, material.normalTextureScale, 1.0f);
      state.normal = normalize(mul(TBN, normalVector));
      state.ffnormal = dot(state.normal, r.direction) <= 0.0f ? state.normal : -state.normal;
      CreateCoordinateSystem(state.ffnormal, state.tangent, state.bitangent);
    }
    state.mat.emission = mk3(material.emissiveFactor);
    if(material.emissiveTexture > -1) state.mat.emission *= xyz(SRGBtoLINEAR(sampleTexture(S, material.emissiveTexture, state.texCoord)));
    state.isEmitter = ((state.mat.emission.x + state.mat.emission.y + state.mat.emission.z) > 1e-3f);
    {
      float perceptualRoughness = material.pbrRoughnessFactor;
      float metallic = material.pbrMetallicFactor;
      if(material.pbrMetallicRoughnessTexture > -1) {
        f4 mr = sampleTexture(S, material.pbrMetallicRoughnessTexture, state.texCoord);
        perceptualRoughness = mr.y * perceptualRoughness;
        metallic = mr.z * metallic;
      }
      f4 baseColor = mk4(material.pbrBaseColorFactor.x, material.pbrBaseColorFactor.y, material.pbrBaseColorFactor.z, material.pbrBaseColorFactor.w);
      if(material.pbrBaseColorTexture > -1) baseColor = baseColor * SRGBtoLINEAR(sampleTexture(S, material.pbrBaseColorTexture, state.texCoord));
      state.mat.albedo = xyz(baseColor);
      state.mat.metallic = metallic;
      state.mat.roughness = perceptualRoughness;
    }
    state.mat.roughness = rt_max(state.mat.roughness, 0.001f);
    state.mat.transmission = material.transmissionFactor;
    if(material.transmissionTexture > -1) state.mat.transmission *= sampleTexture(S, material.transmissionTexture, state.texCoord).x;
    state.mat.ior = material.ior;
    state.eta = dot(state.normal, state.ffnormal) > 0.0f ? (1.0f / state.mat.ior) : state.mat.ior;
  }

  RT_DEV State GetState(f3 rayDir)
  {
    nShaded++;
    State state = zeroState();
    const TriRef ref = S.triRef[hit.gid];
    const DevInstance* inst = &S.instances[ref.inst];
    const rt_prim_mesh geo = S.primMeshes[inst->primMesh];
    const float* o2w = inst->o2w;
    const float* w2o = inst->w2o;
    const f3 bary = mk3((1.0f - hit.u) - hit.v, hit.u, hit.v);
    const uint32_t* tri = &S.indices[geo.firstIndex + 3 * ref.prim];
    const rt_vertex attr0 = S.vertices[geo.vertexOffset + tri[0]];
    const rt_vertex attr1 = S.vertices[geo.vertexOffset + tri[1]];
    const rt_vertex attr2 = S.vertices[geo.vertexOffset + tri[2]];
    const uint32_t matIndex = uint32_t(geo.materialIndex > 0 ? geo.materialIndex : 0);

    const f3 pos0 = mk3(attr0.position), pos1 = mk3(attr1.position), pos2 = mk3(attr2.position);
    const f3 position = (pos0 * bary.x + pos1 * bary.y) + pos2 * bary.z;
    const f3 world_position = xformPoint(o2w, position);
    const f3 wpos0 = xformPoint(o2w, pos0), wpos1 = xformPoint(o2w, pos1), wpos2 = xformPoint(o2w, pos2);

    const f3 nrm0 = decompress_unit_vec(attr0.normal), nrm1 = decompress_unit_vec(attr1.normal), nrm2 = decompress_unit_vec(attr2.normal);
    const f3 normal = normalize((nrm0 * bary.x + nrm1 * bary.y) + nrm2 * bary.z);
    const f3 world_normal = normalize(xformNormal(w2o, normal));
    const f3 geom_normal = normalize(cross(pos1 - pos0, pos2 - pos0));
    const f3 wgeom_normal = normalize(xformNormal(w2o, geom_normal));

    const float h0 = (rt_f2u(attr0.texcoord.y) & 1u) == 1u ? 1.0f : -1.0f;
    const f3 tng0 = decompress_unit_vec(attr0.tangent), tng1 = decompress_unit_vec(attr1.tangent), tng2 = decompress_unit_vec(attr2.tangent);
    f3 tangent = (tng0 * bary.x + tng1 * bary.y) + tng2 * bary.z;
    tangent = normalize(tangent);
    f3 world_tangent = normalize(xformDir(o2w, tangent));
    world_tangent = normalize(world_tangent - dot(world_tangent, world_normal) * world_normal);
    const f3 world_binormal = cross(world_normal, world_tangent) * h0;

    const f2 uv0 = mk2(attr0.texcoord.x, rt_u2f(rt_f2u(attr0.texcoord.y) & ~1u));
    const f2 uv1 = mk2(attr1.texcoord.x, rt_u2f(rt_f2u(attr1.texcoord.y) & ~1u));
    const f2 uv2 = mk2(attr2.texcoord.x, rt_u2f(rt_f2u(attr2.texcoord.y) & ~1u));
    const f2 texcoord0 = (uv0 * bary.x + uv1 * bary.y) + uv2 * bary.z;

    state.position = world_position;
    state.normal = (dot(world_normal, wgeom_normal) > 0.0f) ? world_normal : -world_normal;
    state.ffnormal = dot(state.normal, rayDir) <= 0.0f ? state.normal : -state.normal;
    state.texCoord = texcoord0;
    state.tangent = world_tangent;
    state.bitangent = world_binormal;
    state.matID = matIndex;
    state.area = length(cross(wpos1 - wpos0, wpos2 - wpos0)) * 0.5f;
    return state;
  }

  RT_DEV f4 EnvSample(f3& radiance)
  {
    if(RT_SKY && S.sky) {
      const SkyPre& P = *S.sky;
      f3 T, B;
      CreateCoordinateSystem(P.rawSunDir, T, B);
      f3 d;
      d.x = rnd(seed) * P.sampleRadius;
      d.y = rnd(seed) * P.sampleRadius;
      d.z = rt_sqrt(rt_max(0.0f, (1.0f - d.x * d.x) - d.y * d.y));
      const f3 lightDir = normalize((T * d.x + B * d.y) + P.rawSunDir * d.z);
      radiance = skyfn::evaluate(P, lightDir);
      lastLightId = 0xBFFFFFFFu;
      radiance *= rtx.hdrMultiplier;
      return mk4(lightDir, 0.5f);
    }
    float r0 = rnd(seed), r1 = rnd(seed), r2 = rnd(seed);
    f3 xi = mk3(r0, r1, r2);
    const uint32_t width = uint32_t(S.envW), height = uint32_t(S.envH);
    const uint32_t size = width * height;
    const uint32_t idx = min(rt_ftou(xi.x * float(size)), size - 1);
    const rt_impt_samp sample_data = S.envAccel[idx];
    uint32_t env_idx; float pdf;
    if(xi.y < sample_data.q) { env_idx = idx; xi.y /= sample_data.q; pdf = sample_data.pdf; }
    else { env_idx = uint32_t(sample_data.alias); xi.y = (xi.y - sample_data.q) / (1.0f - sample_data.q); pdf = sample_data.aliasPdf; }
    lastLightId = 0x80000000u | env_idx;
    const uint32_t px = env_idx % width;
    const uint32_t py = env_idx / width;
    const float u = (float(px) + xi.y) / float(width);
    const float phi = u * (2.0f * M_PI_F) - M_PI_F;
    const float sin_phi = rt_sin(phi), cos_phi = rt_cos(phi);
    const float step_theta = M_PI_F / float(height);
    const float theta0 = float(py) * step_theta;
    const float cos_theta = rt_cos(theta0) * (1.0f - xi.z) + rt_cos(theta0 + step_theta) * xi.z;
    const float theta = rt_acos(cos_theta);
    const float sin_theta = rt_sin(theta);
    const float v = theta * M_1_OVER_PI_F;
    f3 lightDir = mk3(cos_phi * sin_theta, cos_theta, sin_phi * sin_theta);
    radiance = xyz(sampleEnv(S, mk2(u, v)));
    radiance *= rtx.hdrMultiplier;
    return mk4(lightDir, pdf);
  }

  RT_DEV static bool IsPdfInvalid(float p) { return p <= 1e-8f || rt_isnan(p); }
  RT_DEV bool Occlusion(const Ray& ray, f3 statePos, float dist)
  {
    return AnyHit(ray, ((dist - rt_abs(ray.origin.x - statePos.x)) - rt_abs(ray.origin.y - statePos.y)) - rt_abs(ray.origin.z - statePos.z));
  }
  RT_DEV f3 Sample(const Material& mat, f3 V, f3 N, f3& L, float& pdf)
  {
    float r0 = rnd(seed), r1 = rnd(seed), r2 = rnd(seed);
    f3 bsdf = mk3(0.0f);
    pdf = metallicWorkflowSample(mat, N, V, mk3(r0, r1, r2), bsdf, L);
    return bsdf;
  }
  RT_DEV f3 EnvRadiance(f3 dir) const
  {
    if(RT_SKY && S.sky) return skyfn::evaluate(*S.sky, dir) * rtx.hdrMultiplier;
    return xyz(sampleEnv(S, GetSphericalUv(dir))) * rtx.hdrMultiplier;
  }
  RT_DEV f3 EnvEval(f3 dir, float& pdf) const
  {
    if(RT_SKY && S.sky) { pdf = 0.5f * rtx.environmentProb; return skyfn::evaluate(*S.sky, dir) * rtx.hdrMultiplier; }
// ... 133 lines not shown
```

cis-565-final-vr-raytracer_amd/csrc/stages.hip:

```cpp
#ifndef RT_SKY
#define RT_SKY 0
#endif
#ifndef RT_COUNT
#define RT_COUNT 0
#endif
#ifndef RT_LAT
#define RT_LAT 0
#endif
#ifndef RT_OM
#define RT_OM 0
#endif
#if RT_OM && RT_COUNT
#error "object motion vectors have no counting build"
#endif
#if RT_OM
#define RT_OM_PARAM , const DevObjMotion& OM
#define RT_OM_KPARAM , DevObjMotion OM
#define RT_OM_ARG , OM
#else
#define RT_OM_PARAM
#define RT_OM_KPARAM
#define RT_OM_ARG
#endif
#if RT_LAT && RT_COUNT
// ... 26 lines not shown
#else
#define RT_VARIANT base
#endif
#include "stage_common.h"
#include <algorithm>

namespace rt {
namespace RT_VARIANT {

#ifndef RT_DIRECT_LB
#define RT_DIRECT_LB 5
#endif
struct DirectCont {
  State state; f3 wo, radiance; i2 motionIdx;
  rt_direct_reservoir resv; uint32_t lid;
  float pdf;
#if RT_OM
  uint32_t inst;
#endif
  int kind;
};
RT_DEV float occlusionDist(const Ray& ray, f3 statePos, float dist)
{
  return ((dist - rt_abs(ray.origin.x - statePos.x)) - rt_abs(ray.origin.y - statePos.y)) - rt_abs(ray.origin.z - statePos.z);
}
RT_DEV bool directPre(Ctx& c, const DevFrame& F RT_OM_PARAM, const rt_state& st, i2 px, const Ray& r, DirectCont& K, Ray& shadowRay, float& shadowDist)
{
  const size_t index = size_t(px.y) * st.size.x + px.x;
  K.kind = 0; K.radiance = mk3(0.0f);
  if(c.hit.t >= RT_INFINITY) {
    F.thisG[index] = make_uint4(rt_f2u(RT_INFINITY), 0u, 0u, RT_INVALID_MAT_ID);
    storeMotion(F, px, i2{0, 0});
#if RT_OM
    OM.instImage[index] = 0xffffffffu;
#endif
    K.radiance = c.EnvRadiance(r.direction);
    return false;
  }
  State& state = K.state;
  state = c.GetState(r.direction);
  c.GetMaterials(state, r);
#if RT_OM
  K.inst = gLoadU32(&c.S.triRef[c.hit.gid].inst);
  OM.instImage[index] = K.inst;
  K.motionIdx = createMotionIndexOm(c, OM, K.inst, state.position);
#else
  K.motionIdx = createMotionIndex(c, state.position);
#endif
  const uint4 gInfo = encodeGeometryInfo(state, c.hit.t);
  storeMotion(F, px, K.motionIdx);
  F.thisG[index] = gInfo;
  if(st.debugging_mode > RT_DBG_INDIRECT_STAGE) { K.radiance = c.DebugInfo(state); return false; }
  if(state.isEmitter) { K.radiance = state.mat.emission; return false; }
  K.wo = -r.direction;
  state.mat.albedo = mk3(1.0f);
  K.resv = zeroDirectResv();
  K.lid = 0xffffffffu;
  if(st.ReSTIRState == RT_RESTIR_NONE) {
    K.kind = 2;
    rt_light_sample ls;
    K.pdf = c.SampleDirectLightNoVisibility(state.position, ls);
    K.resv.lightSample = ls;
    if(Ctx::IsPdfInvalid(K.pdf)) return false;
    shadowRay = Ray{OffsetRay(state.position, state.ffnormal), mk3(ls.wi)};
    shadowDist = occlusionDist(shadowRay, state.position, ls.dist);
    return true;
  }
  K.kind = 1;
  return risCandidatesNoVisibility(c, state, K.wo, K.resv, K.lid, shadowRay, shadowDist);
}
RT_DEV void directPost(Ctx& c, const DevFrame& F RT_OM_PARAM, const rt_state& st, const rt_scene_camera& cam, i2 px, DirectCont& K, bool occluded)
{
  const size_t index = size_t(px.y) * st.size.x + px.x;
  const bool spatial = st.ReSTIRState == RT_RESTIR_SPATIAL || st.ReSTIRState == RT_RESTIR_SPATIOTEMPORAL;
  bool deferred = false;
  f3 radiance = K.radiance;
  if(K.kind != 0) {
    State& state = K.state;
    const f3 wo = K.wo;
    f3 direct = mk3(0.0f);
    if(K.kind == 2) {
      const rt_light_sample ls = K.resv.lightSample;
      if(!Ctx::IsPdfInvalid(K.pdf) && !occluded)
        direct = mk3(ls.Li) * metallicWorkflowBSDF(state.mat, state.ffnormal, wo, mk3(ls.wi)) * rt_max(dot(state.ffnormal, mk3(ls.wi)), 0.0f) / K.pdf;
    } else {
      rt_direct_reservoir& resv = K.resv;
      uint32_t lid = K.lid;
      if(occluded) resv.weight = 0.0f;
      if(st.ReSTIRState == RT_RESTIR_TEMPORAL || st.ReSTIRState == RT_RESTIR_SPATIOTEMPORAL) {
#if RT_OM
        const float reprojDepth = length(omLastPosition(OM, cam, K.inst) - state.position);
#else
        const float reprojDepth = length(mk3(cam.lastPosition) - state.position);
#endif
        rt_direct_reservoir temporal; uint32_t tlid = 0xffffffffu;
        if(findTemporalNeighborDirect(F, st, state.normal, reprojDepth, state.matID, K.motionIdx, temporal, tlid)) {
          if(!resvInvalidW(temporal.weight)) { if(resvMerge(resv, temporal, rnd(c.seed))) lid = tlid; }
        }
      }
      rt_direct_reservoir tempResv = resv;
      if(resvInvalidW(tempResv.weight)) { tempResv.num = 0; tempResv.weight = 0.f; }
      resvClamp(tempResv, st.RISSampleNum * st.reservoirClamp);
      F.thisDirectResv[index] = tempResv;
      F.thisLightId[index] = lid;
      if(spatial) {
        if(resvInvalidW(resv.weight)) { resv.num = 0; resv.weight = 0.f; }
        F.tempDirectResv[index] = resv;
        SurfRec sr;
        sr.position = toR(state.position); sr.normal = toR(state.normal); sr.ffnormal = toR(state.ffnormal); sr.emission = toR(state.mat.emission);
        sr.roughness = state.mat.roughness; sr.metallic = state.mat.metallic; sr.matID = state.matID; sr.seed = c.seed;
        F.surf[index] = sr;
        deferred = true;
      } else {
        const rt_light_sample ls = resv.lightSample;
        if(!resvInvalidW(resv.weight)) {
          f3 LiBsdf = mk3(ls.Li) * metallicWorkflowBSDF(state.mat, state.ffnormal, wo, mk3(ls.wi));
          direct = LiBsdf / resvToScalar(LiBsdf) * resv.weight / float(resv.num);
        }
      }
    }
    if(rt_isnan(direct.x) || rt_isnan(direct.y) || rt_isnan(direct.z)) direct = mk3(0.0f);
    radiance = HDRToLDR(c.clampRadiance(state.mat.emission + direct));
  }
  if(spatial) F.status[index] = deferred ? 1u : 0u;
  if(!deferred) {
    const f3 pixelColor = c.clampRadiance(radiance);
    storeImg(F.thisDirectResult, F, px, mk4(pixelColor, 1.0f));
  }
}

#if RT_LAT
struct WideLds { uint2* stacks; float4* pool; unsigned char* list; uint32_t* ctrl; };
__host__ __device__ inline size_t wideWaveStride(int stackEntries) { return size_t(stackEntries) * WIDE_RAYS + GANG_BOX_UINT2; }
RT_DEV WideLds wideLds(uint2* base, int stackEntries, int nWaves)
{
  WideLds L;
  L.stacks = base;
  L.pool = reinterpret_cast<float4*>(base + size_t(nWaves) * wideWaveStride(stackEntries));
  L.list = reinterpret_cast<unsigned char*>(L.pool + 128 * POOL_SLOT_F4);
  L.ctrl = reinterpret_cast<uint32_t*>(L.list + 128);
  return L;
}
inline size_t wideLdsBytes(int stackEntries, int nWaves) { return size_t(nWaves) * wideWaveStride(stackEntries) * sizeof(uint2) + 128 * 32 + 128 + 16; }
RT_DEV void poolPublish(const WideLds& L, bool hasC, bool hasS)
{
  const int lane = int(threadIdx.x) & 63;
  const unsigned long long lt = (1ull << lane) - 1ull;
  const unsigned long long mC = __ballot(hasC ? 1 : 0), mS = __ballot(hasS ? 1 : 0);
  const int nC = __popcll(mC);
  if(hasC) L.list[__popcll(mC & lt)] = (unsigned char)(lane * 2);
  if(hasS) L.list[nC + __popcll(mS & lt)] = (unsigned char)((lane * 2 + 1) | 0x80);
  if(lane == 0) { L.ctrl[0] = uint32_t(nC + __popcll(mS)); L.ctrl[1] = 0u; L.ctrl[2] = 0u; }
}
RT_DEV void groupTrace(const DevScene& S, const WideLds& L, TravCounters& tc)
{
  __syncthreads();
  const int wave = int(threadIdx.x) >> 6;
  tracePoolWide(S, L.pool, L.list, int(L.ctrl[0]), &L.ctrl[1], L.stacks + size_t(wave) * wideWaveStride(S.stackEntries), tc);
  __syncthreads();
}

#ifndef RT_LAT_DIRECT_WAVES
#define RT_LAT_DIRECT_WAVES 4
#endif
__global__ __launch_bounds__(512, RT_LAT_DIRECT_WAVES) void k_direct_stage(DevScene S, DevFrame F RT_OM_KPARAM, rt_state st, rt_scene_camera cam, int rowBegin, int rowEnd, int tilesX, int tilesY)
{
  extern __shared__ uint2 s_stack[];
  const TileCoord tile = tileOf(tilesX, tilesY);
  if(!tile.valid) return;
  const int wave = int(threadIdx.x) >> 6, lane = int(threadIdx.x) & 63;
  const WideLds L = wideLds(s_stack, S.stackEntries, int(blockDim.x) >> 6);
  const i2 px{tile.x * 8 + (lane & 7), rowBegin + tile.y * 8 + (lane >> 3)};
  const bool mine = wave == 0 && !(px.x >= st.size.x || px.y >= rowEnd);
#if RT_WAVEPROF
  const uint64_t p0 = clock64(), w0 = wall_clock64();
  uint64_t p1 = 0, p2 = 0, p3 = 0, p4 = 0;
#endif
  Ctx c(S, st, cam, nullptr);
  Ray r{mk3(0.0f), mk3(0.0f)};
  if(mine) {
    c.imageCoords = px;
    c.seed = tea(uint32_t(st.size.x) * uint32_t(px.y) + uint32_t(px.x), st.time);
    r = c.raySpawn(px, i2{st.size.x, st.size.y});
    c.nClosest++;
    poolPut(L.pool, lane * 2, r.origin, r.direction, RT_INFINITY, c.seed);
  }
  if(wave == 0) poolPublish(L, mine, false);
#if RT_WAVEPROF
  p1 = clock64();
#endif
  groupTrace(S, L, c.tc);
#if RT_WAVEPROF
  p2 = clock64();
#endif
  DirectCont K;
  Ray shadowRay{mk3(0.0f), mk3(0.0f)};
  float shadowDist = 0.0f;
  bool wantShadow = false;
  if(mine) {
    c.hit = poolGet(L.pool, lane * 2);
    wantShadow = directPre(c, F RT_OM_ARG, st, px, r, K, shadowRay, shadowDist);
    if(wantShadow) { c.nAny++; poolPut(L.pool, lane * 2 + 1, shadowRay.origin, shadowRay.direction, shadowDist, c.seed); }
  }
  if(wave == 0) poolPublish(L, false, wantShadow);
#if RT_WAVEPROF
  p3 = clock64();
#endif
  groupTrace(S, L, c.tc);
#if RT_WAVEPROF
  p4 = clock64();
#endif
  if(mine) directPost(c, F RT_OM_ARG, st, cam, px, K, wantShadow && poolGet(L.pool, lane * 2 + 1).gid != 0xffffffffu);
#if RT_WAVEPROF
  {
    uint32_t* rec = F.waveProf + size_t(blockIdx.x) * 16;
    const uint64_t p5 = clock64();
    if(wave == 0 && lane == 0) {
      rec[0] = uint32_t(tile.x); rec[1] = uint32_t(tile.y); rec[2] = uint32_t(p5 - p0); rec[3] = uint32_t(p2 - p1); rec[4] = uint32_t(p4 - p3);
      rec[7] = uint32_t(p1 - p0); rec[10] = uint32_t(p3 - p2); rec[11] = uint32_t(p5 - p4); rec[15] = uint32_t(wall_clock64() - w0);
    }
    if(lane == 0) { atomicMax(&rec[5], c.tc.rN); atomicMax(&rec[6], c.tc.rT); atomicMax(&rec[8], c.tc.cN); atomicMax(&rec[9], c.tc.cT); atomicAdd(&rec[12], c.tc.rC); atomicAdd(&rec[13], c.tc.rN + c.tc.rT);
      uint32_t* acc = F.waveProf + size_t(65535) * 16;
      for(int k = 0; k < 7; k++) atomicAdd(&acc[k], c.tc.ph[k] >> 4);
      atomicAdd(&acc[7], c.tc.ph[7]);
      atomicAdd(&acc[8], c.tc.cT >> 4);
      for(int k = 0; k < 3; k++) atomicAdd(&acc[9 + k], c.tc.nph[k] >> 4);
      atomicAdd(&acc[12], c.tc.nph[3]); }
  }
#endif
}
#else
__global__ __launch_bounds__(64, RT_DIRECT_LB) void k_direct_stage(DevScene S, DevFrame F RT_OM_KPARAM, rt_state st, rt_scene_camera cam, int rowBegin, int rowEnd, int tilesX, int tilesY)
{
  extern __shared__ uint2 s_stack[];
#if RT_WAVEPROF
  const uint64_t prof_c0 = clock64(), prof_w0 = wall_clock64();
#endif
  const TileCoord tile = tileOf(tilesX, tilesY);
  if(!tile.valid) return;
  const int lane = int(threadIdx.x);
  const i2 px{tile.x * 8 + (lane & 7), rowBegin + tile.y * 8 + (lane >> 3)};
  if(px.x >= st.size.x || px.y >= rowEnd) return;

  Ctx c(S, st, cam, s_stack + lane);
  c.imageCoords = px;
  c.seed = tea(uint32_t(st.size.x) * uint32_t(px.y) + uint32_t(px.x), st.time);
  const Ray r = c.raySpawn(px, i2{st.size.x, st.size.y});
  c.ClosestHit(r);
  DirectCont K;
  Ray shadowRay{mk3(0.0f), mk3(0.0f)};
  float shadowDist = 0.0f;
  const bool wantShadow = directPre(c, F RT_OM_ARG, st, px, r, K, shadowRay, shadowDist);
  const bool occluded = wantShadow && c.AnyHit(shadowRay, shadowDist);
  directPost(c, F RT_OM_ARG, st, cam, px, K, occluded);
  flushCounters(F, c);
#if RT_WAVEPROF
  waveProfFlush(F, c, tile.x, tile.y, prof_c0, prof_w0);
#endif
}
#endif

#if !RT_LAT && !RT_OM
__global__ __launch_bounds__(64) void k_direct_spatial(DevScene S, DevFrame F, rt_state st, rt_scene_camera cam, int rowBegin, int rowEnd, int tilesX, int tilesY)
{
  __shared__ uint32_t s_nb[100 * 9];
  const TileCoord tile = tileOf(tilesX, tilesY);
  if(!tile.valid) return;
  const int lane = int(threadIdx.x);
  const i2 px{tile.x * 8 + (lane & 7), rowBegin + tile.y * 8 + (lane >> 3)};
  const int nbx0 = tile.x * 8 - 1, nby0 = rowBegin + tile.y * 8 - 1;
  {
    const uint32_t* src = reinterpret_cast<const uint32_t*>(F.tempDirectResv);
    for(int k = lane; k < 100; k += 64) {
      const int rx = nbx0 + k % 10, ry = nby0 + k / 10;
      if(rx >= 0 && ry >= 0 && rx < st.size.x && ry < st.size.y) {
        const size_t o = (size_t(ry) * st.size.x + rx) * 9;
#pragma unroll
        for(int w = 0; w < 9; w++) s_nb[k * 9 + w] = src[o + w];
      }
    }
    __syncthreads();
  }
  if(px.x >= st.size.x || px.y >= rowEnd) return;
  const size_t index = size_t(px.y) * st.size.x + px.x;
  if(F.status[index] != 1u) return;
  Ctx c(S, st, cam, nullptr);
  c.imageCoords = px;
  const SurfRec sr = F.surf[index];
  c.seed = sr.seed;
  rt_direct_reservoir resv = F.tempDirectResv[index];
  const uint4 g = F.thisG[index];
  const f3 pnorm = decompress_unit_vec(g.y);
  const float pdepth = rt_u2f(g.x), depth = pdepth;
  const f3 normal = mk3(sr.normal), ffnormal = mk3(sr.ffnormal);
  const i2 size{st.size.x, st.size.y};
  rt_direct_reservoir spatial = zeroDirectResv();
  for(int round = 0; round < 2; round++) {
    rt_direct_reservoir agg = zeroDirectResv();
    bool valid = false;
    for(int i = 0; i < 5; i++) {
      const float r0 = rnd(c.seed), r1 = rnd(c.seed);
      const f2 p = toConcentricDisk(mk2(r0, r1));
      const i2 q{rt_ftoi((float(px.x) + p.x) + 0.5f), rt_ftoi((float(px.y) + p.y) + 0.5f)};
      if(!inBound(q, size)) continue;
      if(dot(normal, pnorm) < 0.5f || rt_abs(depth - pdepth) > depth * 0.1f) continue;
      rt_direct_reservoir nb;
      {
        const uint32_t* e = s_nb + ((q.y - nby0) * 10 + (q.x - nbx0)) * 9;
        uint32_t* d = reinterpret_cast<uint32_t*>(&nb);
#pragma unroll
        for(int w = 0; w < 9; w++) d[w] = e[w];
      }
      if(!resvInvalidW(nb.weight)) { resvMerge(agg, nb, rnd(c.seed)); valid = true; }
    }
    if(valid && !resvInvalidW(agg.weight)) resvMerge(spatial, agg, rnd(c.seed));
  }
  if(!resvInvalidW(spatial.weight)) resvMerge(resv, spatial, rnd(c.seed));
  const Ray r = c.raySpawn(px, size);
  const f3 wo = -r.direction;
  Material mat;
  mat.albedo = mk3(1.0f); mat.emission = mk3(sr.emission); mat.metallic = sr.metallic; mat.roughness = sr.roughness; mat.ior = 0.f; mat.transmission = 0.f;
  f3 direct = mk3(0.0f);
  const rt_light_sample ls = resv.lightSample;
  if(!resvInvalidW(resv.weight)) {
    const f3 LiBsdf = mk3(ls.Li) * metallicWorkflowBSDF(mat, ffnormal, wo, mk3(ls.wi));
    direct = LiBsdf / resvToScalar(LiBsdf) * resv.weight / float(resv.num);
  }
  if(rt_isnan(direct.x) || rt_isnan(direct.y) || rt_isnan(direct.z)) direct = mk3(0.0f);
  const f3 radiance = HDRToLDR(c.clampRadiance(mat.emission + direct));
  storeImg(F.thisDirectResult, F, px, mk4(c.clampRadiance(radiance), 1.0f));
}

__global__ __launch_bounds__(64) void k_direct_gen(DevScene S, DevFrame F, rt_state st, rt_scene_camera cam, int rowBegin, int rowEnd, int tilesX, int tilesY)
{
  extern __shared__ uint2 s_stack[];
  const TileCoord tile = tileOf(tilesX, tilesY);
  if(!tile.valid) return;
  const int lane = int(threadIdx.x);
  const i2 px{tile.x * 8 + (lane & 7), rowBegin + tile.y * 8 + (lane >> 3)};
  if(px.x >= st.size.x || px.y >= rowEnd) return;
  Ctx c(S, st, cam, s_stack + lane);
  c.imageCoords = px;
  const size_t index = size_t(px.y) * st.size.x + px.x;
  c.seed = tea(uint32_t(st.size.x) * uint32_t(px.y) + uint32_t(px.x), st.time);
  const Ray r = c.raySpawn(px, i2{st.size.x, st.size.y});
  c.ClosestHit(r);
  rt_direct_reservoir resv = zeroDirectResv();
  uint32_t lid = 0xffffffffu;
  if(c.hit.t >= RT_INFINITY * 0.8f) {
    uint4 g = make_uint4(rt_f2u(RT_INFINITY), 0u, 0u, RT_INVALID_MAT_ID);
    updateGeometryAlbedo(g, c.EnvRadiance(r.direction));
    F.thisG[index] = g;
    storeMotion(F, px, i2{0, 0});
  } else {
    State state = c.GetState(r.direction);
    c.GetMaterials(state, r);
    storeMotion(F, px, createMotionIndex(c, state.position));
    uint4 g = encodeGeometryInfo(state, c.hit.t);
    if(st.debugging_mode > RT_DBG_INDIRECT_STAGE) updateGeometryAlbedo(g, c.DebugInfo(state));
    else if(state.isEmitter) updateGeometryAlbedo(g, state.mat.emission);
    else {
      state.mat.albedo = mk3(1.0f);
      risCandidates(c, state, -r.direction, resv, lid);
    }
    F.thisG[index] = g;
  }
  F.thisDirectResv[index] = resv;
  F.thisLightId[index] = lid;
  flushCounters(F, c);
}

__global__ __launch_bounds__(64) void k_direct_reuse(DevScene S, DevFrame F, rt_state st, rt_scene_camera cam, int rowBegin, int rowEnd, int tilesX, int tilesY)
{
  const TileCoord tile = tileOf(tilesX, tilesY);
  if(!tile.valid) return;
  const int lane = int(threadIdx.x);
  const i2 px{tile.x * 8 + (lane & 7), rowBegin + tile.y * 8 + (lane >> 3)};
  if(px.x >= st.size.x || px.y >= rowEnd) return;
  Ctx c(S, st, cam, nullptr);
  c.imageCoords = px;
  const int index = px.y * st.size.x + px.x;
  c.seed = tea(uint32_t(index + st.size.x * st.size.y), st.time);
  const Ray ray = c.raySpawn(px, i2{st.size.x, st.size.y});
  GState state; float depth;
  if(!stateFromGBuffer(F.thisG[index], ray, state, depth)) { storeImg(F.thisDirectResult, F, px, mk4(0, 0, 0, 0)); return; }
  f3 direct = mk3(0.0f);
  rt_direct_reservoir resv = F.thisDirectResv[index];
  uint32_t lid = F.thisLightId[index];
  const rt_light_sample ls = resv.lightSample;
  const i2 motionIdx = loadMotion(F, px);
  if(st.ReSTIRState == RT_RESTIR_TEMPORAL || st.ReSTIRState == RT_RESTIR_SPATIOTEMPORAL) {
    const float reprojDepth = length(mk3(cam.lastPosition) - state.position);
    rt_direct_reservoir temporal; uint32_t tlid = 0xffffffffu;
    if(findTemporalNeighborDirect(F, st, state.normal, reprojDepth, state.matID, motionIdx, temporal, tlid)) {
      if(!resvInvalidW(temporal.weight)) { if(resvMerge(resv, temporal, rnd(c.seed))) lid = tlid; }
    }
  }
  if(!resvInvalidW(resv.weight)) direct = mk3(ls.Li);
  resvClamp(resv, st.RISSampleNum * st.reservoirClamp);
  if(resvInvalidW(resv.weight)) { resv.num = 0; resv.weight = 0.f; }
  if(rt_isnan(direct.x) || rt_isnan(direct.y) || rt_isnan(direct.z)) direct = mk3(0.0f);
// ... 63 lines not shown
template <int K>
RT_DEV void indirectSingleBounceTiles(const DevScene& S, const DevFrame& F RT_OM_PARAM, const rt_state& st, const rt_scene_camera& cam, int rowBegin, int rowEnd, int tilesX,
                                      const uint32_t* tiles , int nTilesHere, uint2* s_stack)
{
  const int lane = int(threadIdx.x);
  const i2 indSize{st.size.x / 2, st.size.y / 2};
  float4* pool = reinterpret_cast<float4*>(s_stack + size_t(S.stackEntries) * 64);
#if RT_WAVEPROF
  const uint64_t prof_c0 = clock64(), prof_w0 = wall_clock64();
#endif
  Ctx c(S, st, cam, s_stack + lane);
  struct Path { i2 px; uint32_t seed; float primSamplePdf; f3 a, b, pend; bool hasSurface, nvSet, shadow; };
  Path P[K];
  uint32_t have = 0;
#pragma unroll
  for(int k = 0; k < K; k++) {
    Path& p = P[k];
    p.hasSurface = false; p.nvSet = false; p.shadow = false; p.primSamplePdf = 0.0f; p.a = mk3(0.0f); p.b = mk3(0.0f); p.pend = mk3(0.0f);
    const int t = int(tiles[k < nTilesHere ? k : 0]);
    const int ty = t / tilesX, tx = t - ty * tilesX;
    p.px = i2{tx * 8 + (lane & 7), rowBegin + ty * 8 + (lane >> 3)};
    p.seed = tea(uint32_t(indSize.x) * uint32_t(p.px.y) + uint32_t(p.px.x), st.time);
    if(lane == 0) (void)rnd(p.seed);
    const bool inImage = k < nTilesHere && !(p.px.x >= indSize.x || p.px.y >= indSize.y || p.px.y >= rowEnd);
    if(!inImage) continue;
    const Ray ray = c.raySpawn(p.px, indSize);
    GState g0; float depth;
    if(!stateFromGBuffer(loadG(F.thisG, F, i2{p.px.x * 2, p.px.y * 2}), ray, g0, depth)) { storeImg(F.denoiseIndA, F, p.px, mk4(0, 0, 0, 0)); continue; }
    p.hasSurface = true;
    g0.position += g0.ffnormal * 2e-2f;
    Material m = g0.mat; m.albedo = mk3(1.0f);
    if(st.maxDepth < 1) continue;
    c.seed = p.seed;
    f3 wi = mk3(0.0f); float pdf = 0.0f;
    (void)c.Sample(m, -ray.direction, g0.ffnormal, wi, pdf);
    p.seed = c.seed;
    if(Ctx::IsPdfInvalid(pdf)) continue;
    p.primSamplePdf = pdf; p.nvSet = true; p.a = wi;
    c.nClosest++;
    poolPut(pool, k * 64 + lane, OffsetRay(g0.position, g0.ffnormal), wi, RT_INFINITY, p.seed);
    have |= 1u << k;
  }
  tracePoolTiles<K, false>(S, pool, have, c.stack, c.tc);
  uint32_t haveS = 0;
#pragma unroll
  for(int k = 0; k < K; k++) {
    Path& p = P[k];
    if(!((have >> k) & 1u)) continue;
    const f3 wi = p.a;
    c.hit = poolGet(pool, k * 64 + lane);
    const Ray ray0 = c.raySpawn(p.px, indSize);
    GState g0; float depth;
    stateFromGBuffer(loadG(F.thisG, F, i2{p.px.x * 2, p.px.y * 2}), ray0, g0, depth);
    g0.position += g0.ffnormal * 2e-2f;
    if(c.hit.t >= RT_INFINITY - 1e-4f) {
      p.a = g0.position + wi * RT_INFINITY * 0.8f; p.b = -wi;
      continue;
    }
    const Ray ray{OffsetRay(g0.position, g0.ffnormal), wi};
    State state = c.GetState(ray.direction);
    c.GetMaterials(state, ray);
    p.a = state.position; p.b = state.ffnormal;
    if(state.isEmitter || st.maxDepth < 2) continue;
    c.seed = p.seed;
    const f3 wo = -ray.direction;
    if(st.MIS > 0) {
      rt_light_sample ls;
      const float lightPdf = c.SampleDirectLightNoVisibility(state.position, ls);
      if(!Ctx::IsPdfInvalid(lightPdf)) {
        const f3 lwi = mk3(ls.wi);
        const f3 so = OffsetRay(state.position, state.ffnormal);
        const float maxDist = ((ls.dist - rt_abs(so.x - state.position.x)) - rt_abs(so.y - state.position.y)) - rt_abs(so.z - state.position.z);
        c.nAny++;
        poolPut(pool, k * 64 + lane, so, lwi, maxDist, c.seed);
        haveS |= 1u << k; p.shadow = true;
        const float BSDFPdf = metallicWorkflowPdf(state.mat, state.ffnormal, wo, lwi);
        const float weight = MISw(st, lightPdf, BSDFPdf);
        p.pend = mk3(ls.Li) * metallicWorkflowBSDF(state.mat, state.ffnormal, wo, lwi) * absDot(state.ffnormal, lwi) * mk3(1.0f) / lightPdf * weight;
      }
    }
    f3 w2 = mk3(0.0f); float pdf2 = 0.0f;
    (void)c.Sample(state.mat, wo, state.ffnormal, w2, pdf2);
    p.seed = c.seed;
  }
  tracePoolTiles<K, true>(S, pool, haveS, c.stack, c.tc);
#pragma unroll
  for(int k = 0; k < K; k++) {
    Path& p = P[k];
    if(!p.hasSurface) continue;
    rt_gi_sample gi = newGISample();
    const Ray ray0 = c.raySpawn(p.px, indSize);
    GState primState; float depth;
    stateFromGBuffer(loadG(F.thisG, F, i2{p.px.x * 2, p.px.y * 2}), ray0, primState, depth);
    primState.position += primState.ffnormal * 2e-2f;
    if(p.nvSet) { gi.xv = toR(primState.position); gi.nv = toR(primState.ffnormal); gi.xs = toR(p.a); gi.ns = toR(p.b); }
    if(p.shadow && poolGet(pool, k * 64 + lane).gid == 0xffffffffu) gi.L = toR(mk3(gi.L) + p.pend);
    c.seed = p.seed;
    c.imageCoords = p.px;
    restirIndirectFinish(c, F RT_OM_ARG, st, cam, p.px, indSize, primState, -ray0.direction, gi, p.primSamplePdf);
  }
#if RT_WAVEPROF
  { const int t0 = int(tiles[0]); waveProfFlush(F, c, (t0 % tilesX) | 0x20000, t0 / tilesX, prof_c0, prof_w0); }
#endif
  flushCounters(F, c);
}

#endif

#ifndef RT_INDIRECT_LB
#define RT_INDIRECT_LB 5
#endif
#if RT_LAT
__global__ __launch_bounds__(512, 4) void k_indirect_stage(DevScene S, DevFrame F RT_OM_KPARAM, rt_state st, rt_scene_camera cam, int rowBegin, int rowEnd, int tilesX, int tilesY, int cap,
                                                       const uint32_t* lists, uint32_t* counts, int subShift, int sbK, int genericBlocks)
#else
__global__ __launch_bounds__(64, RT_INDIRECT_LB) void k_indirect_stage(DevScene S, DevFrame F RT_OM_KPARAM, rt_state st, rt_scene_camera cam, int rowBegin, int rowEnd, int tilesX, int tilesY, int cap,
                                                          const uint32_t* lists, uint32_t* counts, int subShift, int sbK, int genericBlocks)
#endif
{
  extern __shared__ uint2 s_stack[];
#if RT_WAVEPROF
  const uint64_t prof_c0 = clock64(), prof_w0 = wall_clock64();
#endif
  TileCoord tile;
  const int part = (int(blockIdx.x) >> 3) & ((1 << subShift) - 1);
  {
    const int L = int(blockIdx.x), xcd = L & 7;
    const int nf = int(counts[xcd * 2]), nb = int(counts[xcd * 2 + 1]);
#if !RT_LAT
    if(sbK > 0 && L >= genericBlocks) {
      const int w = (L - genericBlocks) >> 3, first = w * sbK;
      if(first >= nb) return;
      uint32_t t[3] = {0u, 0u, 0u};
      const int n = min(sbK, nb - first);
      for(int k = 0; k < n; k++) t[k] = lists[size_t(xcd) * cap + (cap - 1 - (first + k))];
      if(sbK == 3) indirectSingleBounceTiles<3>(S, F RT_OM_ARG, st, cam, rowBegin, rowEnd, tilesX, t, n, s_stack);
      else indirectSingleBounceTiles<2>(S, F RT_OM_ARG, st, cam, rowBegin, rowEnd, tilesX, t, n, s_stack);
      return;
    }
#endif
    const int k = (L >> 3) >> subShift;
    tile.valid = sbK > 0 ? (k < nf) : (k < nf + nb);
    const uint32_t t = tile.valid ? lists[size_t(xcd) * cap + (k < nf ? k : cap - 1 - (k - nf))] : 0u;
    tile.y = int(t) / tilesX; tile.x = int(t) - tile.y * tilesX;
  }
  if(!tile.valid) return;
#if RT_LAT
  const WideLds WL = wideLds(s_stack, S.stackEntries, int(blockDim.x) >> 6);
  if((int(threadIdx.x) >> 6) != 0) {
    TravCounters htc{};
    for(;;) {
      __syncthreads();
      if(WL.ctrl[2] != 0u) break;
      tracePoolWide(S, WL.pool, WL.list, int(WL.ctrl[0]), &WL.ctrl[1], WL.stacks + size_t(int(threadIdx.x) >> 6) * wideWaveStride(S.stackEntries), htc);
      __syncthreads();
    }
    return;
  }
#endif
  const int lane = int(threadIdx.x);
  const i2 indSize{st.size.x / 2, st.size.y / 2};
  const int rowsPerPart = 8 >> subShift;
  const bool hasPixel = (lane >> 3) < rowsPerPart;
  const i2 px{tile.x * 8 + (lane & 7), rowBegin + tile.y * 8 + part * rowsPerPart + (lane >> 3)};
#if RT_LAT
  Ctx c(S, st, cam, nullptr);
#else
  Ctx c(S, st, cam, s_stack + lane);
#endif
  c.imageCoords = px;
  c.seed = tea(uint32_t(indSize.x) * uint32_t(px.y) + uint32_t(px.x), st.time);
  int mb = 0;
  if(lane == 0) {
    if(part == 0) mb = rnd(c.seed) < 0.25f ? 1 : 0;
    else { uint32_t s0 = tea(uint32_t(indSize.x) * uint32_t(rowBegin + tile.y * 8) + uint32_t(tile.x * 8), st.time); mb = rnd(s0) < 0.25f ? 1 : 0; }
  }
  const bool multiBounce = __builtin_amdgcn_readfirstlane(mb) != 0;
#if RT_LAT
  float4* pool = WL.pool;
#else
  float4* pool = reinterpret_cast<float4*>(s_stack + size_t(S.stackEntries) * 64);
#endif
  const bool inImage = hasPixel && !(px.x >= indSize.x || px.y >= indSize.y || px.y >= rowEnd);
  Ray ray = c.raySpawn(px, indSize);

  GState g0; float depth;
  bool alive = inImage && stateFromGBuffer(loadG(F.thisG, F, i2{px.x * 2, px.y * 2}), ray, g0, depth);
  const bool hasSurface = alive;
  if(inImage && !hasSurface) storeImg(F.denoiseIndA, F, px, mk4(0, 0, 0, 0));
  if(!alive) { g0 = GState{}; }
  g0.position += g0.ffnormal * 2e-2f;

  f3 throughput = mk3(multiBounce ? 4.0f : 1.0f);
  const f3 primWo = -ray.direction;
  const GState primState = g0;
  rt_gi_sample gi = newGISample();
  float primSamplePdf = 0.0f;
  State state = zeroState();
  state.position = g0.position; state.normal = g0.normal; state.ffnormal = g0.ffnormal; state.mat = g0.mat; state.matID = g0.matID;
  state.mat.albedo = mk3(1.0f);
  for(int depthI = 1; depthI <= st.maxDepth; depthI++) {
    bool hasShadow = false, hasBounce = false;
    f3 pendingAdd = mk3(0.0f), sampleWi = mk3(0.0f);
    float samplePdf = 0.0f;
    if(alive) {
      const f3 wo = -ray.direction;
      if(depthI > 1 && st.MIS > 0) {
        rt_light_sample ls;
        const float lightPdf = c.SampleDirectLightNoVisibility(state.position, ls);
        if(!Ctx::IsPdfInvalid(lightPdf)) {
          const f3 wi = mk3(ls.wi);
          const f3 so = OffsetRay(state.position, state.ffnormal);
          const float maxDist = ((ls.dist - rt_abs(so.x - state.position.x)) - rt_abs(so.y - state.position.y)) - rt_abs(so.z - state.position.z);
          c.nAny++;
          poolPut(pool, lane * 2 + 1, so, wi, maxDist, c.seed);
          hasShadow = true;
          const float BSDFPdf = metallicWorkflowPdf(state.mat, state.ffnormal, wo, wi);
          const float weight = MISw(st, lightPdf, BSDFPdf);
          pendingAdd = mk3(ls.Li) * metallicWorkflowBSDF(state.mat, state.ffnormal, wo, wi) * absDot(state.ffnormal, wi) * throughput / lightPdf * weight;
        }
      }
      const f3 sampleBSDF = c.Sample(state.mat, wo, state.ffnormal, sampleWi, samplePdf);
      if(Ctx::IsPdfInvalid(samplePdf)) alive = false;
      else if(depthI > 1 && !multiBounce) alive = false;
      else {
        if(depthI > 1) throughput *= sampleBSDF / samplePdf * absDot(state.ffnormal, sampleWi);
        else {
          primSamplePdf = samplePdf;
          gi.xv = toR(state.position);
          gi.nv = toR(state.ffnormal);
        }
        ray.origin = OffsetRay(state.position, state.ffnormal);
        ray.direction = sampleWi;
        c.nClosest++;
        poolPut(pool, lane * 2, ray.origin, ray.direction, RT_INFINITY, c.seed);
        hasBounce = true;
      }
    }
    if(__ballot((hasShadow || hasBounce) ? 1 : 0) == 0ull) break;
#if RT_LAT
    poolPublish(WL, hasBounce, hasShadow);
#if RT_WAVEPROF
    { const uint64_t g0 = clock64(); groupTrace(S, WL, c.tc); c.cycClosest += uint32_t(clock64() - g0); c.cycAny++; }
#else
    groupTrace(S, WL, c.tc);
#endif
#else
    tracePool(S, pool, hasBounce, hasShadow, c.stack, c.tc);
#endif
    if(hasShadow && poolGet(pool, lane * 2 + 1).gid == 0xffffffffu) gi.L = toR(mk3(gi.L) + pendingAdd);
    if(hasBounce) {
      c.hit = poolGet(pool, lane * 2);
      if(c.hit.t >= RT_INFINITY - 1e-4f) {
        if(depthI > 1) {
          float lightPdf;
          const f3 Li = c.EnvEval(sampleWi, lightPdf);
          const float weight = MISw(st, samplePdf, lightPdf);
          gi.L = toR(mk3(gi.L) + Li * throughput * weight);
        } else {
          gi.xs = toR(state.position + sampleWi * RT_INFINITY * 0.8f);
          gi.ns = toR(-sampleWi);
        }
        alive = false;
      } else {
        state = c.GetState(ray.direction);
        c.GetMaterials(state, ray);
        if(state.isEmitter) {
          if(depthI > 1) {
            float lightPdf;
            const f3 Li = c.LightEval(state, c.hit.t, sampleWi, lightPdf);
            const float weight = MISw(st, samplePdf, lightPdf);
            gi.L = toR(mk3(gi.L) + Li * throughput * weight);
          } else {
            gi.xs = toR(state.position);
            gi.ns = toR(state.ffnormal);
          }
          alive = false;
        } else if(depthI == 1) { gi.xs = toR(state.position); gi.ns = toR(state.ffnormal); }
      }
    }
  }
#if RT_LAT
  if(lane == 0) WL.ctrl[2] = 1u;
  __syncthreads();
#endif
#if RT_WAVEPROF
  waveProfFlush(F, c, tile.x | (multiBounce ? 0x10000 : 0), tile.y, prof_c0, prof_w0);
#endif
  if(!hasSurface) { flushCounters(F, c); return; }

  restirIndirectFinish(c, F RT_OM_ARG, st, cam, px, indSize, primState, primWo, gi, primSamplePdf);
  flushCounters(F, c);
}

hipError_t launchStage(hipStream_t stream, const DevScene& Sin, const DevFrame& F RT_OM_PARAM, const rt_state& st, const rt_scene_camera& cam, int stage, int level,
                       int rowBegin, int rowEnd)
{
  DevScene S = Sin;
#if RT_LAT
  S.stackEntries = S.stackTotal + (S.gangMax > 0 ? GANG_EXTRA : 0);
  const int nWaves = 8;
#else
  S.stackEntries = F.stackLds > 0 ? std::min(F.stackLds, S.stackTotal) : S.stackTotal;
#endif
  if(stage == RT_STAGE_INDIRECT) S.stackOvf = Sin.stackOvfInd;
  const bool needOvf = S.stackTotal > S.stackEntries;
  const bool half = stage == RT_STAGE_INDIRECT;
  const int gw = half ? st.size.x / 2 : st.size.x, gh = half ? st.size.y / 2 : st.size.y;
  if(rowEnd <= 0 || rowEnd > gh) rowEnd = gh;
  if(rowBegin < 0) rowBegin = 0;
  if(rowBegin >= rowEnd || gw <= 0) return hipSuccess;
  const int tilesX = (gw + 7) / 8, tilesY = (rowEnd - rowBegin + 7) / 8;
  const dim3 grid(tileGrid(tilesX, tilesY)), block(64);
  const size_t lds = size_t(S.stackEntries) * 64 * sizeof(uint2);
  const bool spatial = st.ReSTIRState == RT_RESTIR_SPATIAL || st.ReSTIRState == RT_RESTIR_SPATIOTEMPORAL;
  switch(stage) {
    case RT_STAGE_DIRECT:
      if(level < 0 || level > 2 || (level != 0 && !spatial)) return hipErrorInvalidValue;
#if RT_LAT
      if(level != 2) hipLaunchKernelGGL(k_direct_stage, grid, dim3(64 * nWaves), wideLdsBytes(S.stackEntries, nWaves), stream, S, F RT_OM_ARG, st, cam, rowBegin, rowEnd, tilesX, tilesY);
      if(level != 1 && spatial) return rt::RT_FORWARD::launchStage(stream, Sin, F, st, cam, stage, 2, rowBegin, rowEnd);
#else
      if(needOvf && grid.x * 64u > S.stackOvfThreads) return hipErrorInvalidConfiguration;
      if(level != 2) hipLaunchKernelGGL(k_direct_stage, grid, block, lds, stream, S, F RT_OM_ARG, st, cam, rowBegin, rowEnd, tilesX, tilesY);
#if RT_OM
      if(level != 1 && spatial) return rt::RT_FORWARD::launchStage(stream, Sin, F, st, cam, stage, 2, rowBegin, rowEnd);
#else
      if(level != 1 && spatial) hipLaunchKernelGGL(k_direct_spatial, grid, block, 0, stream, S, F, st, cam, rowBegin, rowEnd, tilesX, tilesY);
#endif
#endif
      break;
    case RT_STAGE_INDIRECT: {
      const int cap = int(tileGrid(tilesX, tilesY) / 8);
      (void)launchIndTileOrder(stream, st, rowBegin, tilesX, tilesY, cap, F.tileOrder, F.qcount + 192);
#if RT_LAT
      hipLaunchKernelGGL(k_indirect_stage, grid, dim3(64 * nWaves), wideLdsBytes(S.stackEntries, nWaves), stream, S, F RT_OM_ARG, st, cam, rowBegin, rowEnd, tilesX, tilesY, cap,
                         (const uint32_t*)F.tileOrder, F.qcount + 192, 0, 0, int(grid.x));
#else
      static const int subEnv = getenv("RESTIR_IND_SUB") ? atoi(getenv("RESTIR_IND_SUB")) : -1;
      const int nTiles = tilesX * tilesY;
      const int subShift = subEnv >= 0 ? subEnv : (nTiles <= 1536 ? 2 : (nTiles <= 3072 ? 1 : 0));
      const int sbK = subShift > 0 ? 0 : 3;
      const unsigned genericBlocks = grid.x << subShift;
      const unsigned sbBlocks = sbK > 0 ? 8u * unsigned((cap + sbK - 1) / sbK) : 0u;
      const size_t poolBytes = std::max<size_t>(POOL_BYTES, size_t(sbK) * 64 * 33);
      if(needOvf && (genericBlocks + sbBlocks) * 64u > S.stackOvfThreads) return hipErrorInvalidConfiguration;
      hipLaunchKernelGGL(k_indirect_stage, dim3(genericBlocks + sbBlocks), block, lds + poolBytes, stream, S, F RT_OM_ARG, st, cam, rowBegin, rowEnd, tilesX, tilesY, cap,
                         (const uint32_t*)F.tileOrder, F.qcount + 192, subShift, sbK, int(genericBlocks));
#endif
      break;
    }
#if !RT_LAT && !RT_OM
    case RT_STAGE_DIRECT_GEN:
      if(needOvf && grid.x * 64u > S.stackOvfThreads) return hipErrorInvalidConfiguration;
      hipLaunchKernelGGL(k_direct_gen, grid, block, lds, stream, S, F, st, cam, rowBegin, rowEnd, tilesX, tilesY);
      break;
    case RT_STAGE_DIRECT_REUSE: hipLaunchKernelGGL(k_direct_reuse, grid, block, 0, stream, S, F, st, cam, rowBegin, rowEnd, tilesX, tilesY); break;
#endif
    default: return hipErrorInvalidValue;
  }
  return hipGetLastError();
}

}
}
```

cis-565-final-vr-raytracer_amd/csrc/traverse.h:

```cpp
#pragma once
#include "dev_math.h"
#include "dev_scene.h"
#include "stages.h"

namespace rt {



struct RayHit {
  float t;
  uint32_t gid;
  float u, v;
};

#ifndef RT_WAVEPROF
#define RT_WAVEPROF 0
#endif
struct TravCounters {
  uint32_t nodes, tris, rounds, live;
#if RT_WAVEPROF
  uint32_t rN, rT, rC, cN, cT, cC, aTex, aOmm;
  uint32_t ph[8];
  uint32_t nph[4];
  uint32_t hl[8], he[8];
// ... 49 lines not shown
}
RT_DEV f4 envTexel(const DevScene& S, int x, int y)
{
  const float4 p = gLoadF4(S.env + (size_t(y) * S.envW + x) * 4);
  return mk4(p.x, p.y, p.z, p.w);
}
RT_DEV f4 sampleEnv(const DevScene& S, f2 uv)
{
  float fx = uv.x * float(S.envW) - 0.5f, fy = uv.y * float(S.envH) - 0.5f;
  float x0f = rt_floor(fx), y0f = rt_floor(fy);
  float ax = fx - x0f, ay = fy - y0f;
  int x0 = rt_ftoi(x0f), y0 = rt_ftoi(y0f);
  int xa = wrapCoord(x0, S.envW, RT_WRAP_REPEAT), xb = wrapCoord(x0 + 1, S.envW, RT_WRAP_REPEAT);
  int ya = wrapCoord(y0, S.envH, RT_WRAP_CLAMP), yb = wrapCoord(y0 + 1, S.envH, RT_WRAP_CLAMP);
  f4 top = mix(envTexel(S, xa, ya), envTexel(S, xb, ya), ax);
  f4 bot = mix(envTexel(S, xa, yb), envTexel(S, xb, yb), ax);
  return mix(top, bot, ay);
}

RT_DEV uint32_t pcgNext(uint32_t& state)
{
  uint32_t prev = state * 747796405u + 2891336453u;
  uint32_t word = ((prev >> ((prev >> 28u) + 4u)) ^ prev) * 277803737u;
  state = prev;
  return (word >> 22u) ^ word;
}
RT_DEV float rnd(uint32_t& seed)
{
  uint32_t r = pcgNext(seed);
  return rt_u2f(0x3f800000u | (r >> 9)) - 1.0f;
}

RT_DEV uint32_t candidateSeed(uint32_t raySeed, uint32_t gid) { return (raySeed ^ 0x9e3779b9u) + (gid + 1u) * 2654435761u; }
struct AlphaRegs { uint4 r0, r1, r2, r3; };
struct AlphaFetch { const uint8_t* p00; const uint8_t* p10; const uint8_t* p01; const uint8_t* p11; float ax, ay; int kind; };
RT_DEV AlphaRegs alphaLoad(const DevScene& S, uint32_t alphaIdx)
{
  const uint4* rp = reinterpret_cast<const uint4*>(S.alphaRec + alphaIdx);
  AlphaRegs A; A.r0 = gLoadU4(rp); A.r1 = gLoadU4(rp + 1); A.r2 = gLoadU4(rp + 2); A.r3 = gLoadU4(rp + 3);
  return A;
}
RT_DEV AlphaFetch alphaAddr(const AlphaRegs& A, float u, float v, const uint8_t* safe)
{
  AlphaFetch F; F.p00 = F.p10 = F.p01 = F.p11 = safe; F.ax = F.ay = 0.0f; F.kind = 0;
  const uint8_t* bgra = reinterpret_cast<const uint8_t*>((uint64_t(A.r2.y) << 32) | uint64_t(A.r2.x));
  if(bgra) {
    const f3 bary = mk3((1.0f - u) - v, u, v);
    const f2 uv = (mk2(rt_u2f(A.r0.x), rt_u2f(A.r0.y)) * bary.x + mk2(rt_u2f(A.r0.z), rt_u2f(A.r0.w)) * bary.y) + mk2(rt_u2f(A.r1.x), rt_u2f(A.r1.y)) * bary.z;
    const int w = int(A.r2.z), h = int(A.r2.w), wrapS = int(A.r3.x), wrapT = int(A.r3.y), filter = int(A.r3.z);
    float fx = uv.x * float(w), fy = uv.y * float(h);
    const bool masks = waveNone(!wrapIsMask(w, h, wrapS, wrapT));
    if(filter == RT_FILTER_NEAREST) {
      const int xi = rt_ftoi(rt_floor(fx)), yi = rt_ftoi(rt_floor(fy));
      int x, y;
      if(masks) { x = xi & (w - 1); y = yi & (h - 1); }
      else { x = wrapCoord(xi, w, wrapS); y = wrapCoord(yi, h, wrapT); }
      F.p00 = F.p10 = F.p01 = F.p11 = bgra + (size_t(y) * w + x) * 4 + 3;
      F.kind = 1;
    } else {
      fx = fx - 0.5f; fy = fy - 0.5f;
      const float x0f = rt_floor(fx), y0f = rt_floor(fy);
      F.ax = fx - x0f; F.ay = fy - y0f;
      const int x0 = rt_ftoi(x0f), y0 = rt_ftoi(y0f);
      int xa, xb, ya, yb;
      if(masks) { xa = x0 & (w - 1); xb = (x0 + 1) & (w - 1); ya = y0 & (h - 1); yb = (y0 + 1) & (h - 1); }
      else {
        xa = wrapCoord(x0, w, wrapS); xb = wrapCoord(x0 + 1, w, wrapS);
        ya = wrapCoord(y0, h, wrapT); yb = wrapCoord(y0 + 1, h, wrapT);
      }
      F.p00 = bgra + (size_t(ya) * w + xa) * 4 + 3; F.p10 = bgra + (size_t(ya) * w + xb) * 4 + 3;
      F.p01 = bgra + (size_t(yb) * w + xa) * 4 + 3; F.p11 = bgra + (size_t(yb) * w + xb) * 4 + 3;
      F.kind = 2;
    }
  }
  return F;
}
RT_DEV bool alphaFinish(const AlphaRegs& A, const AlphaFetch& F, uint8_t a00, uint8_t a10, uint8_t a01, uint8_t a11, uint32_t gid, uint32_t raySeed)
{
  float baseColorAlpha = rt_u2f(A.r1.z);
  if(F.kind != 0) {
    float a;
    if(F.kind == 1) a = unorm8ToFloat(a00);
    else {
      const float top = mixf(unorm8ToFloat(a00), unorm8ToFloat(a10), F.ax);
      const float bot = mixf(unorm8ToFloat(a01), unorm8ToFloat(a11), F.ax);
      a = mixf(top, bot, F.ay);
    }
    baseColorAlpha = baseColorAlpha * a;
  }
  float opacity;
  if(int(A.r3.w) == RT_ALPHA_MASK) opacity = baseColorAlpha > rt_u2f(A.r1.w) ? 1.0f : 0.0f;
  else opacity = baseColorAlpha;
  uint32_t s = candidateSeed(raySeed, gid);
  const float r = rnd(s);
  return !(r > opacity);
}
RT_DEV bool hitTestAlpha(const DevScene& S, uint32_t alphaIdx, uint32_t gid, float u, float v, uint32_t raySeed)
{
  const AlphaRegs A = alphaLoad(S, alphaIdx);
  const AlphaFetch F = alphaAddr(A, u, v, reinterpret_cast<const uint8_t*>(S.alphaRec));
  uint8_t a00 = 0, a10 = 0, a01 = 0, a11 = 0;
  if(F.kind == 1) a00 = gLoadU8(F.p00);
  else if(F.kind == 2) { a00 = gLoadU8(F.p00); a10 = gLoadU8(F.p10); a01 = gLoadU8(F.p01); a11 = gLoadU8(F.p11); }
  return alphaFinish(A, F, a00, a10, a01, a11, gid, raySeed);
}

RT_DEV bool intersectTri(const Tri48& T, f3 o, f3 d, float& t, float& u, float& v)
{
  const f3 e1 = mk3(T.e1x, T.e1y, T.e1z), e2 = mk3(T.e2x, T.e2y, T.e2z), v0 = mk3(T.v0x, T.v0y, T.v0z);
  const f3 p = cross(d, e2);
  const float det = dot(e1, p);
  if(T.flags & TRI_NOCULL) { if(det == 0.0f || rt_isnan(det)) return false; }
  else {
    const float sdet = (T.flags & TRI_FLIP) ? -det : det;
    if(!(sdet > 0.0f)) return false;
  }
  const float inv = 1.0f / det;
  const f3 tv = o - v0;
  u = dot(tv, p) * inv;
  if(!(u >= 0.0f && u <= 1.0f)) return false;
  const f3 q = cross(tv, e1);
  v = dot(d, q) * inv;
  if(!(v >= 0.0f && u + v <= 1.0f)) return false;
  t = dot(e2, q) * inv;
  return !rt_isnan(t);
}
RT_DEV float hitPointPad(f3 o, f3 d, float pad, float t)
{
  const float om = fmaxf(fmaxf(rt_abs(o.x), rt_abs(o.y)), rt_abs(o.z)), dm = fmaxf(fmaxf(rt_abs(d.x), rt_abs(d.y)), rt_abs(d.z));
  return pad + (om + t * dm) * 4.76837158203125e-07f;
}
RT_DEV bool hitInsidePaddedBox(const Tri48& T, f3 o, f3 d, float buildPad, float t)
{
  const float pad = hitPointPad(o, d, buildPad, t);
  const f3 e1 = mk3(T.e1x, T.e1y, T.e1z), e2 = mk3(T.e2x, T.e2y, T.e2z), v0 = mk3(T.v0x, T.v0y, T.v0z);
  const f3 h = o + d * t;
  const f3 lo = mk3((v0.x + fminf(fminf(0.0f, e1.x), e2.x)) - pad, (v0.y + fminf(fminf(0.0f, e1.y), e2.y)) - pad, (v0.z + fminf(fminf(0.0f, e1.z), e2.z)) - pad);
  const f3 hi = mk3((v0.x + fmaxf(fmaxf(0.0f, e1.x), e2.x)) + pad, (v0.y + fmaxf(fmaxf(0.0f, e1.y), e2.y)) + pad, (v0.z + fmaxf(fmaxf(0.0f, e1.z), e2.z)) + pad);
  return h.x >= lo.x && h.x <= hi.x && h.y >= lo.y && h.y <= hi.y && h.z >= lo.z && h.z <= hi.z;
}

RT_DEV float cvtByte(uint32_t w, int j) { return float((w >> (8 * j)) & 0xffu); }

struct Trav {
  f3 o, d;
  float idx, idy, idz;
  uint32_t octinv;
  uint2 ngroup;
  uint2 tgroup;
  int sp;
  float tmax;
  uint32_t seed;
  RayHit hit;
  bool found;
  bool isAny;
};

RT_DEV bool travHasTris(const Trav& T) { return T.tgroup.y != 0u; }
RT_DEV bool travHasNodes(const Trav& T) { return T.ngroup.y > 0x00FFFFFFu || T.sp > 0; }

template <int MODE>
RT_DEV bool travInit(Trav& T, f3 o, f3 d, float tmax, uint32_t raySeed)
{
  const bool ANY = MODE == 2 ? T.isAny : MODE == 1;
  T.o = o; T.d = d; T.tmax = tmax; T.seed = raySeed; T.found = false; T.sp = 0;
  T.hit.t = ANY ? tmax : RT_INFINITY;
  T.hit.gid = 0xffffffffu; T.hit.u = 0.f; T.hit.v = 0.f;
  T.ngroup = make_uint2(0u, 0u);
  T.tgroup = make_uint2(0u, 0u);
  if(hasNan(o) || hasNan(d) || !(T.hit.t > 0.0f)) return false;
  const float eps = 1e-20f;
  T.idx = 1.0f / (rt_abs(d.x) > eps ? d.x : (d.x < 0.0f ? -eps : eps));
  T.idy = 1.0f / (rt_abs(d.y) > eps ? d.y : (d.y < 0.0f ? -eps : eps));
  T.idz = 1.0f / (rt_abs(d.z) > eps ? d.z : (d.z < 0.0f ? -eps : eps));
  T.octinv = (((d.x < 0.0f) ? 1u : 0u) | ((d.y < 0.0f) ? 2u : 0u) | ((d.z < 0.0f) ? 4u : 0u)) ^ 7u;
  T.ngroup = make_uint2(0u, 0x80000000u);
  return true;
}

RT_DEV uint2* stackOverflowSlot(const DevScene& S, int sp)
{
  const size_t thread = size_t(blockIdx.x) * blockDim.x + threadIdx.x;
  return S.stackOvf + (thread * size_t(S.stackTotal - S.stackEntries) + size_t(sp - S.stackEntries));
}
RT_DEV uint2 stackPop(const DevScene& S, Trav& T, uint2* stack)
{
  --T.sp;
  if(__builtin_expect(T.sp < S.stackEntries, 1)) return ldsLoadU2(stack + T.sp * 64);
  return gLoadU2(stackOverflowSlot(S, T.sp));
}
RT_DEV void stackPush(const DevScene& S, Trav& T, uint2* stack, uint2 g)
{
  if(__builtin_expect(T.sp < S.stackEntries, 1)) ldsStoreU2(stack + (T.sp++) * 64, g);
  else if(T.sp < S.stackTotal) { gStoreU2(stackOverflowSlot(S, T.sp), g); T.sp++; }
}

struct NodeRegs { uint4 n0, n1, n2, n3, n4; };
RT_DEV uint32_t travNodeSelect(const DevScene& S, Trav& T, uint2* stack)
{
  uint2 ngroup = T.ngroup;
  if(ngroup.y <= 0x00FFFFFFu) ngroup = stackPop(S, T, stack);
  const uint32_t hits = ngroup.y;
  const uint32_t bit = 31u - uint32_t(__clz(int(hits)));
  ngroup.y &= ~(1u << bit);
  if(ngroup.y > 0x00FFFFFFu) stackPush(S, T, stack, ngroup);
  const uint32_t slot = (bit - 24u) ^ T.octinv;
  const uint32_t rel = uint32_t(__popc(hits & ~(0xFFFFFFFFu << slot) & 0xFFu));
  T.ngroup.y = 0u;
  return ngroup.x + rel;
}
RT_DEV NodeRegs nodeLoad(const DevScene& S, uint32_t index)
{
  const uint4* np = reinterpret_cast<const uint4*>(S.nodes + index);
  NodeRegs N; N.n0 = gLoadU4(np); N.n1 = gLoadU4(np + 1); N.n2 = gLoadU4(np + 2); N.n3 = gLoadU4(np + 3); N.n4 = gLoadU4(np + 4);
  return N;
}
RT_DEV void travNodeTest(Trav& T, const NodeRegs& N)
{
  const uint4 n0 = N.n0, n1 = N.n1, n2 = N.n2, n3 = N.n3, n4 = N.n4;
  const bool nx = T.d.x < 0.0f, ny = T.d.y < 0.0f, nz = T.d.z < 0.0f;
  const uint32_t octinv = T.octinv;
  const uint32_t octinv4 = octinv * 0x01010101u;
  const float adjx = rt_u2f((n0.w & 0xffu) << 23) * T.idx;
  const float adjy = rt_u2f(((n0.w >> 8) & 0xffu) << 23) * T.idy;
  const float adjz = rt_u2f(((n0.w >> 16) & 0xffu) << 23) * T.idz;
  const float orgx = (rt_u2f(n0.x) - T.o.x) * T.idx, orgy = (rt_u2f(n0.y) - T.o.y) * T.idy, orgz = (rt_u2f(n0.z) - T.o.z) * T.idz;
  const uint32_t imask = n0.w >> 24;
  uint32_t hitmask = 0;
#pragma unroll
  for(int half = 0; half < 2; half++) {
    const uint32_t meta4 = half ? n1.w : n1.z;
    const uint32_t isInner4 = (meta4 & (meta4 << 1)) & 0x10101010u;
    const uint32_t innerMask4 = (isInner4 >> 4) * 0xffu;
    const uint32_t bitIndex4 = (meta4 ^ (octinv4 & innerMask4)) & 0x1F1F1F1Fu;
    const uint32_t childBits4 = (meta4 >> 5) & 0x07070707u;
    const uint32_t qlx = half ? n2.y : n2.x, qly = half ? n2.w : n2.z, qlz = half ? n3.y : n3.x;
    const uint32_t qhx = half ? n3.w : n3.z, qhy = half ? n4.y : n4.x, qhz = half ? n4.w : n4.z;
    const uint32_t nearx = nx ? qhx : qlx, farx = nx ? qlx : qhx;
    const uint32_t neary = ny ? qhy : qly, fary = ny ? qly : qhy;
    const uint32_t nearz = nz ? qhz : qlz, farz = nz ? qlz : qhz;
#pragma unroll
    for(int j = 0; j < 4; j++) {
      const float tlx = __builtin_fmaf(cvtByte(nearx, j), adjx, orgx), thx = __builtin_fmaf(cvtByte(farx, j), adjx, orgx);
      const float tly = __builtin_fmaf(cvtByte(neary, j), adjy, orgy), thy = __builtin_fmaf(cvtByte(fary, j), adjy, orgy);
      const float tlz = __builtin_fmaf(cvtByte(nearz, j), adjz, orgz), thz = __builtin_fmaf(cvtByte(farz, j), adjz, orgz);
      const float tn = fmaxf(fmaxf(tlx, tly), fmaxf(tlz, 0.0f));
      const float tf = fminf(fminf(thx, thy), fminf(thz, T.hit.t));
      if(tn <= tf) hitmask |= ((childBits4 >> (8 * j)) & 0xffu) << ((bitIndex4 >> (8 * j)) & 0xffu);
    }
  }
  T.ngroup = make_uint2(n1.x, (hitmask & 0xFF000000u) | imask);
  T.tgroup = make_uint2(n1.y, hitmask & 0x00FFFFFFu);
}
RT_DEV void travNode(const DevScene& S, Trav& T, uint2* stack, TravCounters& tc)
{
  const uint32_t index = travNodeSelect(S, T, stack);
  const NodeRegs N = nodeLoad(S, index);
  tc.nodes++;
  travNodeTest(T, N);
}

struct TriRegs { uint4 a, b, c, om; };
RT_DEV TriRegs triLoad(const DevScene& S, uint32_t triIndex)
{
  const uint4* tp = reinterpret_cast<const uint4*>(S.tris + triIndex);
  TriRegs Q; Q.a = gLoadU4(tp); Q.b = gLoadU4(tp + 1); Q.c = gLoadU4(tp + 2); Q.om = gLoadU4(tp + 3);
  return Q;
}
RT_DEV int triCandidateGeom(const DevScene& S, const TriRegs& Q, f3 o, f3 d, bool ANY, float tmax, float curT, uint32_t curG, uint32_t seed, float& t, float& u, float& v,
                            uint32_t& gid, uint32_t& alphaIdx, TravCounters& tc)
{
  const uint4 a = Q.a, b = Q.b, c = Q.c, om = Q.om;
  Tri48 R;
  R.v0x = rt_u2f(a.x); R.v0y = rt_u2f(a.y); R.v0z = rt_u2f(a.z); R.e1x = rt_u2f(a.w);
  R.e1y = rt_u2f(b.x); R.e1z = rt_u2f(b.y); R.e2x = rt_u2f(b.z); R.e2y = rt_u2f(b.w);
  R.e2z = rt_u2f(c.x); R.globalId = c.y; R.flags = c.z; R.alphaIdx = c.w;
  gid = R.globalId; alphaIdx = R.alphaIdx;
  if(!intersectTri(R, o, d, t, u, v)) return 0;
  if(ANY) {
    if(!(t > 0.0f && t < tmax)) return 0;
  } else {
    if(!(t > 0.0f && t < RT_INFINITY)) return 0;
    if(!(t < curT || (t == curT && R.globalId < curG))) return 0;
  }
  if(!hitInsidePaddedBox(R, o, d, S.triPad, t)) return 0;
  if(!(R.flags & TRI_OPAQUE)) {
    const int ci = min(int(u * 8.0f), 7), cj = min(int(v * 8.0f), 7);
    const int cell = cj * 8 + ci;
    const uint32_t word = (cell < 16) ? om.x : ((cell < 32) ? om.y : ((cell < 48) ? om.z : om.w));
    const uint32_t state = (word >> ((cell & 15) * 2)) & 3u;
#if RT_WAVEPROF
    if(state == 0u) tc.aTex++; else tc.aOmm++;
#else
    (void)tc;
#endif
    if(state == 1u) return 1;
    if(state == 2u) { uint32_t hs = candidateSeed(seed, R.globalId); return !(rnd(hs) > 0.0f) ? 1 : 0; }
    return 2;
  }
  return 1;
}
RT_DEV bool triCandidate(const DevScene& S, uint32_t triIndex, f3 o, f3 d, bool ANY, float tmax, float curT, uint32_t curG, uint32_t seed, float& t, float& u, float& v,
                         uint32_t& gid, TravCounters& tc)
{
  const TriRegs Q = triLoad(S, triIndex);
  uint32_t alphaIdx;
  const int s = triCandidateGeom(S, Q, o, d, ANY, tmax, curT, curG, seed, t, u, v, gid, alphaIdx, tc);
  if(s == 2) return hitTestAlpha(S, alphaIdx, gid, u, v, seed);
  return s == 1;
}

template <int MODE>
RT_DEV void travTri(const DevScene& S, Trav& T, TravCounters& tc)
{
  const bool ANY = MODE == 2 ? T.isAny : MODE == 1;
  const uint32_t bit = 31u - uint32_t(__clz(int(T.tgroup.y)));
  T.tgroup.y &= ~(1u << bit);
  tc.tris++;
  float t, u, v; uint32_t gid;
  if(!triCandidate(S, T.tgroup.x + bit, T.o, T.d, ANY, T.tmax, T.hit.t, T.hit.gid, T.seed, t, u, v, gid, tc)) return;
  T.hit.t = t; T.hit.gid = gid; T.hit.u = u; T.hit.v = v;
  T.found = true;
  if(ANY) { T.tgroup.y = 0u; T.ngroup.y = 0u; T.sp = 0; }
}

RT_DEV float laneF(float v, int l) { return rt_u2f(uint32_t(__builtin_amdgcn_readlane(int(rt_f2u(v)), l))); }
RT_DEV uint32_t laneU(uint32_t v, int l) { return uint32_t(__builtin_amdgcn_readlane(int(v), l)); }

template <int MODE>
RT_DEV void travTriCoop(const DevScene& S, Trav& T, unsigned long long triMask, TravCounters& tc)
{
  const int lane = int(threadIdx.x) & 63;
  const unsigned long long present = __ballot(1);
  const int rank = __popcll(present & ((1ull << lane) - 1ull)), np = __popcll(present);
  while(triMask != 0ull) {
    const int l = __builtin_ctzll(triMask);
    triMask &= triMask - 1ull;
    const f3 o = mk3(laneF(T.o.x, l), laneF(T.o.y, l), laneF(T.o.z, l)), d = mk3(laneF(T.d.x, l), laneF(T.d.y, l), laneF(T.d.z, l));
    const uint32_t tbase = laneU(T.tgroup.x, l), seed = laneU(T.seed, l);
    uint32_t tbits = laneU(T.tgroup.y, l);
    const float tmax = laneF(T.tmax, l);
    const bool ANY = MODE == 2 ? (laneU(T.isAny ? 1u : 0u, l) != 0u) : MODE == 1;
    float bt = laneF(T.hit.t, l), bu = 0.0f, bv = 0.0f;
    uint32_t bg = laneU(T.hit.gid, l);
    bool found = false;
    if(lane == l) tc.tris += uint32_t(__popc(tbits));
    while(tbits != 0u && !(ANY && found)) {
      int mine = -1, j = 0;
      while(tbits != 0u && j < np) {
        const int k = 31 - __clz(int(tbits));
        tbits &= ~(1u << k);
        if(rank == j) mine = k;
        j++;
      }
      float t = 0.0f, u = 0.0f, v = 0.0f; uint32_t gid = 0u;
      bool ok = false;
      if(mine >= 0) ok = triCandidate(S, tbase + uint32_t(mine), o, d, ANY, tmax, bt, bg, seed, t, u, v, gid, tc);
      unsigned long long okm = __ballot(ok ? 1 : 0);
      while(okm != 0ull) {
        const int w = __builtin_ctzll(okm);
        okm &= okm - 1ull;
        const float wt = laneF(t, w); const uint32_t wg = laneU(gid, w);
        if(ANY || wt < bt || (wt == bt && wg < bg)) { bt = wt; bg = wg; bu = laneF(u, w); bv = laneF(v, w); found = true; }
        if(ANY) break;
      }
    }
    if(lane == l) {
      T.tgroup.y = 0u;
      if(found) {
        T.hit.t = bt; T.hit.gid = bg; T.hit.u = bu; T.hit.v = bv; T.found = true;
        if(ANY) { T.ngroup.y = 0u; T.sp = 0; }
      }
    }
  }
}

template <int ANY>
RT_DEV bool travRound(const DevScene& S, Trav& T, bool live, uint2* stack, TravCounters& tc)
{
  tc.rounds++; tc.live += live ? 1u : 0u;
  const bool wantTri = live && travHasTris(T);
  const bool wantNode = live && !wantTri;
  const int nT = __popcll(__ballot(wantTri ? 1 : 0)), nN = __popcll(__ballot(wantNode ? 1 : 0));
  if(nT >= nN) { if(wantTri) travTri<ANY>(S, T, tc); }
  else { if(wantNode) travNode(S, T, stack, tc); }
  return live && (travHasTris(T) || travHasNodes(T));
}

template <int ANY>
RT_DEV bool travRoundMasked(const DevScene& S, Trav& T, bool live, unsigned long long liveMask, uint2* stack, TravCounters& tc)
{
  tc.rounds++; tc.live += live ? 1u : 0u;
  const bool wantTri = live && travHasTris(T);
  const unsigned long long triMask = __ballot(wantTri ? 1 : 0);
  const int nLive = __popcll(liveMask), nT = __popcll(triMask), nN = nLive - nT;
#if RT_WAVEPROF
  const uint64_t c0 = clock64();
#endif
  if(nLive <= S.coopLive) {
    if(nT > 0) travTriCoop<ANY>(S, T, triMask, tc);
    if(live && travHasNodes(T)) travNode(S, T, stack, tc);
  } else if(nT >= nN) { if(wantTri) travTri<ANY>(S, T, tc); }
  else { if(live && !wantTri) travNode(S, T, stack, tc); }
#if RT_WAVEPROF
  {
    const uint32_t dc = uint32_t(clock64() - c0);
    if(nLive <= S.coopLive) { tc.rC++; tc.cC += dc; } else if(nT >= nN) { tc.rT++; tc.cT += dc; } else { tc.rN++; tc.cN += dc; }
    const int ex = nLive <= S.coopLive ? nLive : (nT >= nN ? nT : nN);
    tc.hl[(nLive - 1) >> 3]++; tc.he[(max(ex, 1) - 1) >> 3]++;
  }
#endif
  return live && (travHasTris(T) || travHasNodes(T));
}

template <int ANY>
RT_DEV bool traceRay(const DevScene& S, f3 o, f3 d, float tmax, uint32_t raySeed, uint2* stack, RayHit& hit, TravCounters& tc)
{
  Trav T;
  bool live = travInit<ANY>(T, o, d, tmax, raySeed);
  unsigned long long liveMask = __ballot(live ? 1 : 0);
  while(liveMask != 0ull) {
    live = travRoundMasked<ANY>(S, T, live, liveMask, stack, tc);
    liveMask = __ballot(live ? 1 : 0);
  }
  hit = T.hit;
  return T.found;
}

constexpr int POOL_SLOT_F4 = 2;
constexpr int POOL_BYTES = 128 * 32 + 128;

RT_DEV void poolPut(float4* pool, int slot, f3 o, f3 d, float tmax, uint32_t seed)
{
  pool[slot * POOL_SLOT_F4] = make_float4(o.x, o.y, o.z, d.x);
  pool[slot * POOL_SLOT_F4 + 1] = make_float4(d.y, d.z, tmax, rt_u2f(seed));
}
RT_DEV RayHit poolGet(const float4* pool, int slot)
{
  const float4 r = pool[slot * POOL_SLOT_F4];
  RayHit h; h.t = r.x; h.gid = rt_f2u(r.y); h.u = r.z; h.v = r.w;
  return h;
}
RT_DEV void waveLdsSync() { __builtin_amdgcn_fence(__ATOMIC_SEQ_CST, "wavefront"); __builtin_amdgcn_wave_barrier(); }

RT_DEV void tracePool(const DevScene& S, float4* pool, bool hasC, bool hasS, uint2* stack, TravCounters& tc)
{
  unsigned char* list = reinterpret_cast<unsigned char*>(pool + 128 * POOL_SLOT_F4);
  const int lane = int(threadIdx.x) & 63;
  const unsigned long long lt = (1ull << lane) - 1ull;
  const unsigned long long mC = __ballot(hasC ? 1 : 0), mS = __ballot(hasS ? 1 : 0);
  const int nC = __popcll(mC), n = nC + __popcll(mS);
  if(n == 0) return;
  if(hasC) list[__popcll(mC & lt)] = (unsigned char)(lane * 2);
  if(hasS) list[nC + __popcll(mS & lt)] = (unsigned char)(lane * 2 + 1);
  waveLdsSync();
  int next = 0, mySlot = 0;
  bool live = false;
  Trav T;
  for(;;) {
    unsigned long long liveMask = __ballot(live ? 1 : 0);
    const unsigned long long idle = ~liveMask;
    if(next < n && idle != 0ull) {
      const int item = next + __popcll(idle & lt);
      if(!live && item < n) {
        mySlot = int(list[item]);
        const float4 a = pool[mySlot * POOL_SLOT_F4], b = pool[mySlot * POOL_SLOT_F4 + 1];
        T.isAny = (mySlot & 1) != 0;
        live = travInit<2>(T, mk3(a.x, a.y, a.z), mk3(a.w, b.x, b.y), b.z, rt_f2u(b.w));
        if(!live) pool[mySlot * POOL_SLOT_F4] = make_float4(T.hit.t, rt_u2f(T.hit.gid), T.hit.u, T.hit.v);
      }
      next = min(n, next + __popcll(idle));
      liveMask = __ballot(live ? 1 : 0);
    }
    if(liveMask == 0ull) {
      if(next >= n) break;
      continue;
    }
    const bool still = travRoundMasked<2>(S, T, live, liveMask, stack, tc);
    if(live && !still) pool[mySlot * POOL_SLOT_F4] = make_float4(T.hit.t, rt_u2f(T.hit.gid), T.hit.u, T.hit.v);
    live = still;
  }
  waveLdsSync();
}

template <int K, bool ANY>
RT_DEV void tracePoolTiles(const DevScene& S, float4* pool, uint32_t have , uint2* stack, TravCounters& tc)
{
  unsigned char* list = reinterpret_cast<unsigned char*>(pool + K * 64 * POOL_SLOT_F4);
  const int lane = int(threadIdx.x) & 63;
  const unsigned long long lt = (1ull << lane) - 1ull;
  int n = 0;
#pragma unroll
  for(int k = 0; k < K; k++) {
    const bool h = (have >> k) & 1u;
    const unsigned long long m = __ballot(h ? 1 : 0);
    if(h) list[n + __popcll(m & lt)] = (unsigned char)(k * 64 + lane);
    n += __popcll(m);
  }
  if(n == 0) return;
  waveLdsSync();
  int next = 0, mySlot = 0;
  bool live = false;
  Trav T;
  for(;;) {
    unsigned long long liveMask = __ballot(live ? 1 : 0);
    const unsigned long long idle = ~liveMask;
    if(next < n && idle != 0ull) {
      const int item = next + __popcll(idle & lt);
      if(!live && item < n) {
        mySlot = int(list[item]);
        const float4 a = pool[mySlot * POOL_SLOT_F4], b = pool[mySlot * POOL_SLOT_F4 + 1];
        live = travInit<ANY>(T, mk3(a.x, a.y, a.z), mk3(a.w, b.x, b.y), b.z, rt_f2u(b.w));
        if(!live) pool[mySlot * POOL_SLOT_F4] = make_float4(T.hit.t, rt_u2f(T.hit.gid), T.hit.u, T.hit.v);
      }
      next = min(n, next + __popcll(idle));
      liveMask = __ballot(live ? 1 : 0);
    }
    if(liveMask == 0ull) {
      if(next >= n) break;
      continue;
    }
    const bool still = travRoundMasked<ANY>(S, T, live, liveMask, stack, tc);
    if(live && !still) pool[mySlot * POOL_SLOT_F4] = make_float4(T.hit.t, rt_u2f(T.hit.gid), T.hit.u, T.hit.v);
    live = still;
  }
  waveLdsSync();
}

#ifndef RT_LAT
#define RT_LAT 0
#endif
#if RT_LAT
constexpr int WIDE_G = 8;
constexpr int WIDE_RAYS = 64 / WIDE_G;
#define RT_DPP_XOR1 0xB1
#define RT_DPP_XOR2 0x4E
#define RT_DPP_HALF_MIRROR 0x141
template <int CTRL> RT_DEV uint32_t dppU(uint32_t v) { return uint32_t(__builtin_amdgcn_update_dpp(0, int(v), CTRL, 0xf, 0xf, true)); }
template <int CTRL> RT_DEV float dppF(float v) { return rt_u2f(dppU<CTRL>(rt_f2u(v))); }
RT_DEV uint32_t groupOr(uint32_t v)
{
  v |= dppU<RT_DPP_XOR1>(v);
  v |= dppU<RT_DPP_XOR2>(v);
  v |= dppU<RT_DPP_HALF_MIRROR>(v);
  return v;
}
struct WideCand { float t; uint32_t gid; float u, v; };
template <int CTRL> RT_DEV void candMinStep(WideCand& c)
{
  const float ot = dppF<CTRL>(c.t); const uint32_t og = dppU<CTRL>(c.gid); const float ou = dppF<CTRL>(c.u), ov = dppF<CTRL>(c.v);
  const bool take = ot < c.t || (ot == c.t && og < c.gid);
  c.t = take ? ot : c.t; c.gid = take ? og : c.gid; c.u = take ? ou : c.u; c.v = take ? ov : c.v;
}
RT_DEV void groupMinCand(WideCand& c) { candMinStep<RT_DPP_XOR1>(c); candMinStep<RT_DPP_XOR2>(c); candMinStep<RT_DPP_HALF_MIRROR>(c); }

RT_DEV uint2 stackPopW(Trav& T, const uint2* stack) { --T.sp; return ldsLoadU2(stack + T.sp * WIDE_RAYS); }
RT_DEV void stackPushW(Trav& T, uint2* stack, uint2 g, int j) { if(j == 0) ldsStoreU2(stack + T.sp * WIDE_RAYS, g); T.sp++; }
RT_DEV uint32_t travNodeSelectW(Trav& T, uint2* stack, int j)
{
  uint2 ngroup = T.ngroup;
  if(ngroup.y <= 0x00FFFFFFu) ngroup = stackPopW(T, stack);
  const uint32_t hits = ngroup.y;
  const uint32_t bit = 31u - uint32_t(__clz(int(hits)));
  ngroup.y &= ~(1u << bit);
  if(ngroup.y > 0x00FFFFFFu) stackPushW(T, stack, ngroup, j);
  const uint32_t slot = (bit - 24u) ^ T.octinv;
  const uint32_t rel = uint32_t(__popc(hits & ~(0xFFFFFFFFu << slot) & 0xFFu));
  T.ngroup.y = 0u;
  return ngroup.x + rel;
}
RT_DEV uint32_t byteOf(uint32_t lo, uint32_t hi, int j) { return ((j < 4 ? lo : hi) >> (8 * (j & 3))) & 0xffu; }
RT_DEV void travNodeTestW(Trav& T, const NodeRegs& N, int j)
{
  const uint4 n0 = N.n0, n1 = N.n1, n2 = N.n2, n3 = N.n3, n4 = N.n4;
  const bool nx = T.d.x < 0.0f, ny = T.d.y < 0.0f, nz = T.d.z < 0.0f;
  const float adjx = rt_u2f((n0.w & 0xffu) << 23) * T.idx;
  const float adjy = rt_u2f(((n0.w >> 8) & 0xffu) << 23) * T.idy;
  const float adjz = rt_u2f(((n0.w >> 16) & 0xffu) << 23) * T.idz;
  const float orgx = (rt_u2f(n0.x) - T.o.x) * T.idx, orgy = (rt_u2f(n0.y) - T.o.y) * T.idy, orgz = (rt_u2f(n0.z) - T.o.z) * T.idz;
  const uint32_t imask = n0.w >> 24;
  const uint32_t meta = byteOf(n1.z, n1.w, j);
  const uint32_t isInner = (meta & (meta << 1)) & 0x10u;
  const uint32_t bitIndex = (meta ^ (isInner ? T.octinv : 0u)) & 0x1Fu;
  const uint32_t childBits = (meta >> 5) & 0x07u;
  const float qlx = float(byteOf(n2.x, n2.y, j)), qly = float(byteOf(n2.z, n2.w, j)), qlz = float(byteOf(n3.x, n3.y, j));
  const float qhx = float(byteOf(n3.z, n3.w, j)), qhy = float(byteOf(n4.x, n4.y, j)), qhz = float(byteOf(n4.z, n4.w, j));
  const float tlx = __builtin_fmaf(nx ? qhx : qlx, adjx, orgx), thx = __builtin_fmaf(nx ? qlx : qhx, adjx, orgx);
  const float tly = __builtin_fmaf(ny ? qhy : qly, adjy, orgy), thy = __builtin_fmaf(ny ? qly : qhy, adjy, orgy);
  const float tlz = __builtin_fmaf(nz ? qhz : qlz, adjz, orgz), thz = __builtin_fmaf(nz ? qlz : qhz, adjz, orgz);
  const float tn = fmaxf(fmaxf(tlx, tly), fmaxf(tlz, 0.0f));
  const float tf = fminf(fminf(thx, thy), fminf(thz, T.hit.t));
  const uint32_t hitmask = groupOr((tn <= tf) ? (childBits << bitIndex) : 0u);
  T.ngroup = make_uint2(n1.x, (hitmask & 0xFF000000u) | imask);
  T.tgroup = make_uint2(n1.y, hitmask & 0x00FFFFFFu);
}
template <int MODE>
RT_DEV void travTriW(const DevScene& S, Trav& T, int j, TravCounters& tc)
{
  const bool ANY = MODE == 2 ? T.isAny : MODE == 1;
  uint32_t rem = T.tgroup.y;
  int mine = -1;
#pragma unroll
  for(int k = 0; k < WIDE_G; k++) {
    if(rem != 0u) {
      const int b = 31 - __clz(int(rem));
      if(k == j) mine = b;
      rem &= ~(1u << b);
    }
  }
  T.tgroup.y = rem;
  WideCand c; c.t = __builtin_huge_valf(); c.gid = 0xffffffffu; c.u = 0.0f; c.v = 0.0f;
  bool ok = false;
#if RT_WAVEPROF
#define RT_PH(k) { __builtin_amdgcn_s_waitcnt(0); const uint64_t pn = clock64(); tc.ph[k] += uint32_t(pn - pc); pc = pn; }
  uint64_t pc = clock64(); tc.ph[7]++;
#else
#define RT_PH(k)
#endif
  if(mine >= 0) {
    float t, u, v; uint32_t gid, alphaIdx;
    const uint32_t ti = T.tgroup.x + uint32_t(mine);
    const TriRegs Q = triLoad(S, ti);
    const uint4* ap = reinterpret_cast<const uint4*>(S.alphaByTri + ti);
    AlphaRegs A; A.r0 = gLoadU4(ap); A.r1 = gLoadU4(ap + 1); A.r2 = gLoadU4(ap + 2); A.r3 = gLoadU4(ap + 3);
    RT_PH(0)
    const int s = triCandidateGeom(S, Q, T.o, T.d, ANY, T.tmax, T.hit.t, T.hit.gid, T.seed, t, u, v, gid, alphaIdx, tc);
    ok = s == 1;
    RT_PH(1)
    if(s == 2) {
      const AlphaFetch Fh = alphaAddr(A, u, v, reinterpret_cast<const uint8_t*>(S.alphaRec));
      RT_PH(2)
      uint8_t a00 = 0, a10 = 0, a01 = 0, a11 = 0;
      if(Fh.kind == 1) a00 = gLoadU8(Fh.p00);
      else if(Fh.kind == 2) { a00 = gLoadU8(Fh.p00); a10 = gLoadU8(Fh.p10); a01 = gLoadU8(Fh.p01); a11 = gLoadU8(Fh.p11); }
      RT_PH(3)
      ok = alphaFinish(A, Fh, a00, a10, a01, a11, gid, T.seed);
      RT_PH(4)
    }
    if(ok) { c.t = t; c.gid = gid; c.u = u; c.v = v; }
  }
  RT_PH(5)
  groupMinCand(c);
  const bool any = c.t < __builtin_huge_valf();
  if(any && (ANY || c.t < T.hit.t || (c.t == T.hit.t && c.gid < T.hit.gid))) {
    T.hit.t = c.t; T.hit.gid = c.gid; T.hit.u = c.u; T.hit.v = c.v;
    T.found = true;
    if(ANY) { T.tgroup.y = 0u; T.ngroup.y = 0u; T.sp = 0; }
  }
  RT_PH(6)
#undef RT_PH
  (void)ok;
}
template <int MODE>
RT_DEV bool travRoundW(const DevScene& S, Trav& T, bool live, int j, uint2* stack, TravCounters& tc)
{
  bool wantTri = live && travHasTris(T);
  bool wantNode = live && !wantTri;
  {
    const int nT = __popcll(__ballot(wantTri ? 1 : 0)), nN = __popcll(__ballot(wantNode ? 1 : 0));
    if(nT >= nN) wantNode = false; else wantTri = false;
  }
  if(wantTri) travTriW<MODE>(S, T, j, tc);
#if RT_WAVEPROF
  if(wantNode) {
    __builtin_amdgcn_s_waitcnt(0); const uint64_t q0 = clock64();
    const uint32_t ni = travNodeSelectW(T, stack, j);
    __builtin_amdgcn_s_waitcnt(0); const uint64_t q1 = clock64();
    const NodeRegs N = nodeLoad(S, ni);
    __builtin_amdgcn_s_waitcnt(0); const uint64_t q2 = clock64();
    travNodeTestW(T, N, j);
    const uint64_t q3 = clock64();
    tc.nph[0] += uint32_t(q1 - q0); tc.nph[1] += uint32_t(q2 - q1); tc.nph[2] += uint32_t(q3 - q2); tc.nph[3]++;
  }
#else
  if(wantNode) { const NodeRegs N = nodeLoad(S, travNodeSelectW(T, stack, j)); travNodeTestW(T, N, j); }
#endif
  return live && (travHasTris(T) || travHasNodes(T));
}

constexpr int GANG_BOX_UINT2 = 16;
constexpr int GANG_SCAN = 2;
constexpr int GANG_EXTRA = 20;
RT_DEV uint32_t leaderBits(unsigned long long m) { return uint32_t(((m & 0x0101010101010101ull) * 0x0102040810204080ull) >> 56); }
RT_DEV int nthSetBitFromTop(uint32_t v, int n)
{
  for(int k = 0; k < n; k++) v &= ~(1u << (31 - __clz(int(v))));
  return 31 - __clz(int(v));
}
RT_DEV uint32_t dropTopBits(uint32_t v, int n) { for(int k = 0; k < n; k++) v &= ~(1u << (31 - __clz(int(v)))); return v; }

RT_DEV void gangTail(const DevScene& S, float4* pool, uint2* waveStack, Trav& T, bool& live, int mySlot, TravCounters& tc)
{
  const int lane = int(threadIdx.x) & 63, j = lane & (WIDE_G - 1), g = lane >> 3;
  float4* gbox = reinterpret_cast<float4*>(waveStack + size_t(S.stackEntries) * WIDE_RAYS);
  const int wideRoom = S.stackEntries - S.stackTotal;
  bool working = false;
  int og = g;
  uint32_t wm = 0u;
  uint32_t lastOwners = 0u;
  for(;;) {
    const uint32_t owners = leaderBits(__ballot(live ? 1 : 0));
    if(owners == 0u) break;
    if(owners != lastOwners) {
      lastOwners = owners;
      const int n = __popc(owners);
      const bool mine = (owners >> g) & 1u;
      const uint32_t freeM = leaderBits(__ballot((!working && !mine) ? 1 : 0));
      const bool adopt = !working && !mine;
      if(mine && !working) {
        if(T.ngroup.y > 0x00FFFFFFu) { if(__builtin_expect(T.sp >= S.stackEntries, 0)) __builtin_trap(); stackPushW(T, waveStack + g, T.ngroup, j); T.ngroup.y = 0u; }
        og = g;
      }
      if(adopt) {
        uint32_t o = owners;
        for(int k = __popc(freeM & ((1u << g) - 1u)) % n; k > 0; k--) o &= o - 1u;
        og = __ffs(int(o)) - 1;
      }
      waveLdsSync();
      const int src = og * WIDE_G;
      const int slot = __shfl(mySlot, src);
      const int sp = __shfl(T.sp, src);
      const float bt = __shfl(T.hit.t, src), bu = __shfl(T.hit.u, src), bv = __shfl(T.hit.v, src);
      const uint32_t bg = uint32_t(__shfl(int(T.hit.gid), src));
      const int any = __shfl(T.isAny ? 1 : 0, src);
      if(adopt) {
        const float4 a = pool[slot * POOL_SLOT_F4], b = pool[slot * POOL_SLOT_F4 + 1];
        T.isAny = any != 0;
        (void)travInit<2>(T, mk3(a.x, a.y, a.z), mk3(a.w, b.x, b.y), b.z, rt_f2u(b.w));
        T.ngroup.y = 0u; T.tgroup.y = 0u;
        T.sp = sp; T.hit.t = bt; T.hit.gid = bg; T.hit.u = bu; T.hit.v = bv;
      }
      working = true;
      wm = 0u;
#pragma unroll
      for(int k = 0; k < WIDE_RAYS; k++) if(__builtin_amdgcn_readlane(og, k * WIDE_G) == og) wm |= 1u << k;
    }
    uint2* stack = waveStack + og;
    const bool hasTri = working && T.tgroup.y != 0u;
    if(__ballot(hasTri ? 1 : 0) != 0ull) {
      if(hasTri) travTriW<2>(S, T, j, tc);
      if(j == 0) gbox[g] = make_float4(T.hit.t, rt_u2f(T.hit.gid), T.hit.u, T.hit.v);
      waveLdsSync();
      uint32_t rest = wm & ~(1u << g);
      while(rest != 0u) {
        const int k = __ffs(int(rest)) - 1; rest &= rest - 1u;
        const float4 c = gbox[k];
        const uint32_t cg = rt_f2u(c.y);
        if(cg != 0xffffffffu && (T.hit.gid == 0xffffffffu || (!T.isAny && (c.x < T.hit.t || (c.x == T.hit.t && cg < T.hit.gid))))) { T.hit.t = c.x; T.hit.gid = cg; T.hit.u = c.z; T.hit.v = c.w; }
      }
      if(T.isAny && T.hit.gid != 0xffffffffu) { T.sp = 0; T.tgroup.y = 0u; T.ngroup.y = 0u; }
      waveLdsSync();
    }
    const bool wantNode = working && T.tgroup.y == 0u && T.sp > 0;
    const uint32_t wantM = leaderBits(__ballot(wantNode ? 1 : 0)) & wm;
    bool took = false; uint32_t child = 0u;
    if(wantNode) {
      const int iw = __popc(wantM & ((1u << g) - 1u)), nw = __popc(wantM);
      uint2 e[GANG_SCAN]; int cnt[GANG_SCAN]; int avail = 0;
#pragma unroll
      for(int k = 0; k < GANG_SCAN; k++) {
        e[k] = make_uint2(0u, 0u);
        if(T.sp > k) e[k] = stack[(T.sp - 1 - k) * WIDE_RAYS];
        cnt[k] = __popc(e[k].y >> 24); avail += cnt[k];
      }
      int nsel = min(nw, avail);
      if(T.sp + nsel > wideRoom) nsel = 1;
      int before = 0, nsp = T.sp; bool wrote = false; uint2 back = make_uint2(0u, 0u); int backAt = 0;
#pragma unroll
      for(int k = 0; k < GANG_SCAN; k++) {
        const int takeHere = max(0, min(cnt[k], nsel - before));
        if(iw >= before && iw < before + takeHere) {
          took = true;
          const int bit = nthSetBitFromTop(e[k].y & 0xFF000000u, iw - before);
          const uint32_t slotI = uint32_t(bit - 24) ^ T.octinv;
          child = e[k].x + uint32_t(__popc(e[k].y & ~(0xFFFFFFFFu << slotI) & 0xFFu));
        }
        if(takeHere > 0) {
          const uint32_t h = dropTopBits(e[k].y & 0xFF000000u, takeHere) | (e[k].y & 0x00FFFFFFu);
          if(h > 0x00FFFFFFu) { nsp = T.sp - k; wrote = true; back = make_uint2(e[k].x, h); backAt = T.sp - 1 - k; }
          else nsp = T.sp - 1 - k;
        }
        before += takeHere;
      }
      if(wrote && iw == 0 && j == 0) stack[backAt * WIDE_RAYS] = back;
      T.sp = nsp;
    }
    waveLdsSync();
    { const int sp2 = __shfl(T.sp, wantM != 0u ? (__ffs(int(wantM)) - 1) * WIDE_G : lane); if(working && !wantNode && wantM != 0u) T.sp = sp2; }
    if(took) { const NodeRegs N = nodeLoad(S, child); travNodeTestW(T, N, j); }
    const bool push = took && T.ngroup.y > 0x00FFFFFFu;
    const uint32_t pushM = leaderBits(__ballot(push ? 1 : 0)) & wm;
    if(working) {
      if(__builtin_expect(T.sp + __popc(pushM) > S.stackEntries, 0)) __builtin_trap();
      if(push && j == 0) stack[(T.sp + __popc(pushM & ~((2u << g) - 1u))) * WIDE_RAYS] = T.ngroup;
      T.sp += __popc(pushM);
      T.ngroup.y = 0u;
    }
    waveLdsSync();
    const uint32_t busyM = leaderBits(__ballot((working && (T.tgroup.y != 0u || T.sp > 0)) ? 1 : 0)) & wm;
    if(working && busyM == 0u) {
      if(live) { if(j == 0) pool[mySlot * POOL_SLOT_F4] = make_float4(T.hit.t, rt_u2f(T.hit.gid), T.hit.u, T.hit.v); live = false; }
      working = false;
    }
  }
}

RT_DEV void tracePoolWide(const DevScene& S, float4* pool, const unsigned char* list, int n, uint32_t* next, uint2* waveStack, TravCounters& tc)
{
  const int lane = int(threadIdx.x) & 63, j = lane & (WIDE_G - 1), r = lane >> 3;
  uint2* stack = waveStack + r;
  const unsigned long long leaders = 0x0101010101010101ull;
  const unsigned long long below = (1ull << (lane & ~(WIDE_G - 1))) - 1ull;
  bool live = false, exhausted = n == 0;
  int mySlot = 0;
  Trav T;
  T.isAny = false;
  for(;;) {
    unsigned long long liveMask = __ballot(live ? 1 : 0);
    const unsigned long long idle = ~liveMask & leaders;
    if(!exhausted && idle != 0ull) {
      const int nIdle = __popcll(idle);
      uint32_t base = 0u;
      if(lane == 0) base = atomicAdd(next, uint32_t(nIdle));
      base = uint32_t(__builtin_amdgcn_readfirstlane(int(base)));
      const int item = int(base) + __popcll(idle & below);
      if(!live && item < n) {
        const uint32_t e = list[item];
        mySlot = int(e & 0x7fu);
        const float4 a = pool[mySlot * POOL_SLOT_F4], b = pool[mySlot * POOL_SLOT_F4 + 1];
        T.isAny = (e & 0x80u) != 0u;
        live = travInit<2>(T, mk3(a.x, a.y, a.z), mk3(a.w, b.x, b.y), b.z, rt_f2u(b.w));
        if(!live && j == 0) pool[mySlot * POOL_SLOT_F4] = make_float4(T.hit.t, rt_u2f(T.hit.gid), T.hit.u, T.hit.v);
      }
      if(int(base) + nIdle >= n) exhausted = true;
      liveMask = __ballot(live ? 1 : 0);
    }
    if(liveMask == 0ull) {
      if(exhausted) break;
      continue;
    }
    if(exhausted && S.gangMax > 0 && __popcll(liveMask & leaders) <= S.gangMax && __popcll(liveMask & leaders) < WIDE_RAYS) {
      gangTail(S, pool, waveStack, T, live, mySlot, tc);
      break;
    }
#if RT_WAVEPROF
    const uint64_t pc0 = clock64();
    const bool anyTri = __ballot((live && travHasTris(T)) ? 1 : 0) != 0ull;
    tc.rC += uint32_t(__popcll(liveMask & leaders));
#endif
    const bool still = travRoundW<2>(S, T, live, j, stack, tc);
#if RT_WAVEPROF
    { const uint32_t dc = uint32_t(clock64() - pc0); if(anyTri) { tc.rT++; tc.cT += dc; } else { tc.rN++; tc.cN += dc; } }
#endif
    if(live && !still && j == 0) pool[mySlot * POOL_SLOT_F4] = make_float4(T.hit.t, rt_u2f(T.hit.gid), T.hit.u, T.hit.v);
    live = still;
  }
}
#endif

}
```

Before: 1426.

## Seed primary closest-hit traversal with previous frame's hit triangle

Each frame records the BVH triangle index that produced every pixel's primary hit into a per-pixel seed plane. The next frame tests that triangle first to set an initial hit distance, so closest-hit traversal can cull farther nodes sooner. Recording the index means carrying an extra field through the wide, gang and DPP reduction paths, plus extra LDS in the gang box and a reset memset whenever the scene, acceleration structure or resolution changes. The wide pooled path only writes seeds and never reads them, so there the change adds cost without shortening traversal.

```diff
diff --git a/cis-565-final-vr-raytracer_amd/csrc/dev_scene.h b/cis-565-final-vr-raytracer_amd/csrc/dev_scene.h
--- a/cis-565-final-vr-raytracer_amd/csrc/dev_scene.h
+++ b/cis-565-final-vr-raytracer_amd/csrc/dev_scene.h
@@ -73,6 +73,7 @@
   uint32_t* histMiss;
   int32_t stackLds;
   int32_t pad4;
+  const uint32_t* seedIn; uint32_t* seedOut;
 };
 
 struct OmCamera {
diff --git a/cis-565-final-vr-raytracer_amd/csrc/rt_api.cpp b/cis-565-final-vr-raytracer_amd/csrc/rt_api.cpp
--- a/cis-565-final-vr-raytracer_amd/csrc/rt_api.cpp
+++ b/cis-565-final-vr-raytracer_amd/csrc/rt_api.cpp
@@ -480,6 +480,13 @@
   return RT_OK;
 }
 
+static int resetSeedPlane(rt_ctx* c)
+{
+  if(!c->scratch.seedOut || c->W <= 0) return RT_OK;
+  RT_HIP(c, hipMemsetAsync(c->scratch.seedOut, 0xff, size_t(c->W) * size_t(c->H) * sizeof(uint32_t), c->stream));
+  return RT_OK;
+}
+
 int rt_upload_scene(rt_ctx* c, const rt_scene_desc* d)
 {
   if(!c) return RT_ERR_INVALID_ARG;
@@ -604,7 +611,7 @@
   RT_HIP(c, hipDeviceSynchronize());
   c->haveScene = true;
   reopenPriorityDecision(c);
-  return RT_OK;
+  return resetSeedPlane(c);
 }
 
 
@@ -757,6 +764,7 @@
   lt.lap("uploads (tree, alpha records)");
   c->haveAccel = true;
   reopenPriorityDecision(c);
+  if((rc = resetSeedPlane(c))) return rc;
   return ensureStackOverflow(c);
 }
 
@@ -816,12 +824,14 @@
   RT_SCRATCH(postRowSums, size_t(h) * 6, double); RT_SCRATCH(postMean, 8, float);
   RT_SCRATCH(postMipD, n + 64, float4); RT_SCRATCH(postMipI, n + 64, float4);
   RT_SCRATCH(tileOrder, (size_t(w / 2 + 7) / 8) * (size_t(h / 2 + 7) / 8 + 16 * 2) + 64 + 4096, uint32_t);
+  RT_SCRATCH(seedOut, n, uint32_t); X.seedIn = X.seedOut;
 #if RT_WAVEPROF
   RT_SCRATCH(waveProf, WAVEPROF_RECORDS * 16, uint32_t);
 #endif
 #undef RT_SCRATCH
   RT_HIP(c, hipDeviceSynchronize());
   c->W = w; c->H = h;
+  if((rc = resetSeedPlane(c))) return rc;
   if(c->objMotion != RT_OBJECT_MOTION_OFF && (rc = allocObjectMotion(c))) return rc;
   return ensureStackOverflow(c);
 }
@@ -995,6 +1005,7 @@
   F.W = c->W; F.H = c->H;
   const DevFrame& X = c->scratch;
   F.surf = X.surf; F.status = X.status; F.qcount = X.qcount; F.waveProf = X.waveProf;
+  F.seedIn = X.seedIn; F.seedOut = X.seedOut;
   F.histRow0 = c->histRow0; F.histRow1 = c->histRow1; F.histMiss = X.qcount + 250;
   F.geomN = X.geomN; F.geomP = X.geomP; F.geomNh = X.geomNh; F.geomPh = X.geomPh; F.tileOrder = X.tileOrder; F.postRowSums = X.postRowSums; F.postMean = X.postMean;
   return F;
@@ -2075,7 +2086,7 @@
   }
   c->refN = 0;
   B.stats = st;
-  return RT_OK;
+  return resetSeedPlane(c);
 }
 
 int rt_get_rebuild_stats(rt_ctx* c, rt_rebuild_stats* out)
diff --git a/cis-565-final-vr-raytracer_amd/csrc/shading.h b/cis-565-final-vr-raytracer_amd/csrc/shading.h
--- a/cis-565-final-vr-raytracer_amd/csrc/shading.h
+++ b/cis-565-final-vr-raytracer_amd/csrc/shading.h
@@ -247,9 +247,11 @@
   uint32_t cycClosest = 0, cycAny = 0;
   RT_DEV void ClosestHit(const Ray& r) { nClosest++; const uint64_t c0 = clock64(); traceRay<false>(S, r.origin, r.direction, RT_INFINITY, seed, stack, hit, tc); cycClosest += uint32_t(clock64() - c0); }
   RT_DEV bool AnyHit(const Ray& r, float maxDist) { nAny++; RayHit h; const uint64_t c0 = clock64(); const bool f = traceRay<true>(S, r.origin, r.direction, maxDist, seed, stack, h, tc); cycAny += uint32_t(clock64() - c0); return f; }
+  RT_DEV uint32_t ClosestHitSeeded(const Ray& r, uint32_t seedTri) { nClosest++; uint32_t rec; const uint64_t c0 = clock64(); traceRaySeeded(S, r.origin, r.direction, seed, seedTri, stack, hit, rec, tc); cycClosest += uint32_t(clock64() - c0); return rec; }
 #else
   RT_DEV void ClosestHit(const Ray& r) { nClosest++; traceRay<false>(S, r.origin, r.direction, RT_INFINITY, seed, stack, hit, tc); }
   RT_DEV bool AnyHit(const Ray& r, float maxDist) { nAny++; RayHit h; return traceRay<true>(S, r.origin, r.direction, maxDist, seed, stack, h, tc); }
+  RT_DEV uint32_t ClosestHitSeeded(const Ray& r, uint32_t seedTri) { nClosest++; uint32_t rec; traceRaySeeded(S, r.origin, r.direction, seed, seedTri, stack, hit, rec, tc); return rec; }
 #endif
 
   RT_DEV static f4 SRGBtoLINEAR(f4 c) { return mk4(rt_pow(c.x, 2.2f), rt_pow(c.y, 2.2f), rt_pow(c.z, 2.2f), c.w); }
diff --git a/cis-565-final-vr-raytracer_amd/csrc/stages.hip b/cis-565-final-vr-raytracer_amd/csrc/stages.hip
--- a/cis-565-final-vr-raytracer_amd/csrc/stages.hip
+++ b/cis-565-final-vr-raytracer_amd/csrc/stages.hip
@@ -202,11 +202,12 @@
   if(hasS) L.list[nC + __popcll(mS & lt)] = (unsigned char)((lane * 2 + 1) | 0x80);
   if(lane == 0) { L.ctrl[0] = uint32_t(nC + __popcll(mS)); L.ctrl[1] = 0u; L.ctrl[2] = 0u; }
 }
+template <bool REC>
 RT_DEV void groupTrace(const DevScene& S, const WideLds& L, TravCounters& tc)
 {
   __syncthreads();
   const int wave = int(threadIdx.x) >> 6;
-  tracePoolWide(S, L.pool, L.list, int(L.ctrl[0]), &L.ctrl[1], L.stacks + size_t(wave) * wideWaveStride(S.stackEntries), tc);
+  tracePoolWide<REC>(S, L.pool, L.list, int(L.ctrl[0]), &L.ctrl[1], L.stacks + size_t(wave) * wideWaveStride(S.stackEntries), tc);
   __syncthreads();
 }
 
@@ -239,7 +240,7 @@
 #if RT_WAVEPROF
   p1 = clock64();
 #endif
-  groupTrace(S, L, c.tc);
+  groupTrace<true>(S, L, c.tc);
 #if RT_WAVEPROF
   p2 = clock64();
 #endif
@@ -249,6 +250,7 @@
   bool wantShadow = false;
   if(mine) {
     c.hit = poolGet(L.pool, lane * 2);
+    F.seedOut[size_t(px.y) * st.size.x + px.x] = poolGetRec(L.pool, lane * 2);
     wantShadow = directPre(c, F RT_OM_ARG, st, px, r, K, shadowRay, shadowDist);
     if(wantShadow) { c.nAny++; poolPut(L.pool, lane * 2 + 1, shadowRay.origin, shadowRay.direction, shadowDist, c.seed); }
   }
@@ -256,7 +258,7 @@
 #if RT_WAVEPROF
   p3 = clock64();
 #endif
-  groupTrace(S, L, c.tc);
+  groupTrace<false>(S, L, c.tc);
 #if RT_WAVEPROF
   p4 = clock64();
 #endif
@@ -296,7 +298,11 @@
   c.imageCoords = px;
   c.seed = tea(uint32_t(st.size.x) * uint32_t(px.y) + uint32_t(px.x), st.time);
   const Ray r = c.raySpawn(px, i2{st.size.x, st.size.y});
-  c.ClosestHit(r);
+  {
+    const uint32_t seedTri = F.seedIn ? gLoadU32(F.seedIn + (uint32_t(st.size.x) * uint32_t(px.y) + uint32_t(px.x))) : 0xffffffffu;
+    const uint32_t rec = c.ClosestHitSeeded(r, seedTri);
+    F.seedOut[size_t(px.y) * st.size.x + px.x] = rec;
+  }
   DirectCont K;
   Ray shadowRay{mk3(0.0f), mk3(0.0f)};
   float shadowDist = 0.0f;
@@ -666,7 +672,7 @@
     for(;;) {
       __syncthreads();
       if(WL.ctrl[2] != 0u) break;
-      tracePoolWide(S, WL.pool, WL.list, int(WL.ctrl[0]), &WL.ctrl[1], WL.stacks + size_t(int(threadIdx.x) >> 6) * wideWaveStride(S.stackEntries), htc);
+      tracePoolWide<false>(S, WL.pool, WL.list, int(WL.ctrl[0]), &WL.ctrl[1], WL.stacks + size_t(int(threadIdx.x) >> 6) * wideWaveStride(S.stackEntries), htc);
       __syncthreads();
     }
     return;
@@ -755,9 +761,9 @@
 #if RT_LAT
     poolPublish(WL, hasBounce, hasShadow);
 #if RT_WAVEPROF
-    { const uint64_t g0 = clock64(); groupTrace(S, WL, c.tc); c.cycClosest += uint32_t(clock64() - g0); c.cycAny++; }
-#else
-    groupTrace(S, WL, c.tc);
+    { const uint64_t g0 = clock64(); groupTrace<false>(S, WL, c.tc); c.cycClosest += uint32_t(clock64() - g0); c.cycAny++; }
+#else
+    groupTrace<false>(S, WL, c.tc);
 #endif
 #else
     tracePool(S, pool, hasBounce, hasShadow, c.stack, c.tc);
diff --git a/cis-565-final-vr-raytracer_amd/csrc/traverse.h b/cis-565-final-vr-raytracer_amd/csrc/traverse.h
--- a/cis-565-final-vr-raytracer_amd/csrc/traverse.h
+++ b/cis-565-final-vr-raytracer_amd/csrc/traverse.h
@@ -225,6 +225,7 @@
   float tmax;
   uint32_t seed;
   RayHit hit;
+  uint32_t rec;
   bool found;
   bool isAny;
 };
@@ -238,7 +239,7 @@
   const bool ANY = MODE == 2 ? T.isAny : MODE == 1;
   T.o = o; T.d = d; T.tmax = tmax; T.seed = raySeed; T.found = false; T.sp = 0;
   T.hit.t = ANY ? tmax : RT_INFINITY;
-  T.hit.gid = 0xffffffffu; T.hit.u = 0.f; T.hit.v = 0.f;
+  T.hit.gid = 0xffffffffu; T.hit.u = 0.f; T.hit.v = 0.f; T.rec = 0xffffffffu;
   T.ngroup = make_uint2(0u, 0u);
   T.tgroup = make_uint2(0u, 0u);
   if(hasNan(o) || hasNan(d) || !(T.hit.t > 0.0f)) return false;
@@ -392,7 +393,7 @@
   tc.tris++;
   float t, u, v; uint32_t gid;
   if(!triCandidate(S, T.tgroup.x + bit, T.o, T.d, ANY, T.tmax, T.hit.t, T.hit.gid, T.seed, t, u, v, gid, tc)) return;
-  T.hit.t = t; T.hit.gid = gid; T.hit.u = u; T.hit.v = v;
+  T.hit.t = t; T.hit.gid = gid; T.hit.u = u; T.hit.v = v; T.rec = T.tgroup.x + bit;
   T.found = true;
   if(ANY) { T.tgroup.y = 0u; T.ngroup.y = 0u; T.sp = 0; }
 }
@@ -415,7 +416,7 @@
     const float tmax = laneF(T.tmax, l);
     const bool ANY = MODE == 2 ? (laneU(T.isAny ? 1u : 0u, l) != 0u) : MODE == 1;
     float bt = laneF(T.hit.t, l), bu = 0.0f, bv = 0.0f;
-    uint32_t bg = laneU(T.hit.gid, l);
+    uint32_t bg = laneU(T.hit.gid, l), br = 0u;
     bool found = false;
     if(lane == l) tc.tris += uint32_t(__popc(tbits));
     while(tbits != 0u && !(ANY && found)) {
@@ -434,14 +435,14 @@
         const int w = __builtin_ctzll(okm);
         okm &= okm - 1ull;
         const float wt = laneF(t, w); const uint32_t wg = laneU(gid, w);
-        if(ANY || wt < bt || (wt == bt && wg < bg)) { bt = wt; bg = wg; bu = laneF(u, w); bv = laneF(v, w); found = true; }
+        if(ANY || wt < bt || (wt == bt && wg < bg)) { bt = wt; bg = wg; bu = laneF(u, w); bv = laneF(v, w); br = tbase + laneU(uint32_t(mine), w); found = true; }
         if(ANY) break;
       }
     }
     if(lane == l) {
       T.tgroup.y = 0u;
       if(found) {
-        T.hit.t = bt; T.hit.gid = bg; T.hit.u = bu; T.hit.v = bv; T.found = true;
+        T.hit.t = bt; T.hit.gid = bg; T.hit.u = bu; T.hit.v = bv; T.rec = br; T.found = true;
         if(ANY) { T.ngroup.y = 0u; T.sp = 0; }
       }
     }
@@ -500,6 +501,26 @@
   return T.found;
 }
 
+RT_DEV bool traceRaySeeded(const DevScene& S, f3 o, f3 d, uint32_t raySeed, uint32_t seedTri, uint2* stack, RayHit& hit, uint32_t& rec, TravCounters& tc)
+{
+  float st = 0.0f, su = 0.0f, sv = 0.0f; uint32_t sg = 0xffffffffu;
+  bool seeded = false;
+  if(seedTri < S.numTris) {
+    tc.tris++;
+    seeded = triCandidate(S, seedTri, o, d, false, RT_INFINITY, RT_INFINITY, 0xffffffffu, raySeed, st, su, sv, sg, tc);
+  }
+  Trav T;
+  bool live = travInit<0>(T, o, d, RT_INFINITY, raySeed);
+  if(live && seeded) { T.hit.t = st; T.hit.gid = sg; T.hit.u = su; T.hit.v = sv; T.rec = seedTri; T.found = true; }
+  unsigned long long liveMask = __ballot(live ? 1 : 0);
+  while(liveMask != 0ull) {
+    live = travRoundMasked<0>(S, T, live, liveMask, stack, tc);
+    liveMask = __ballot(live ? 1 : 0);
+  }
+  hit = T.hit; rec = T.rec;
+  return T.found;
+}
+
 constexpr int POOL_SLOT_F4 = 2;
 constexpr int POOL_BYTES = 128 * 32 + 128;
 
@@ -514,6 +535,8 @@
   RayHit h; h.t = r.x; h.gid = rt_f2u(r.y); h.u = r.z; h.v = r.w;
   return h;
 }
+RT_DEV void poolPutRec(float4* pool, int slot, uint32_t rec) { reinterpret_cast<uint32_t*>(pool + slot * POOL_SLOT_F4 + 1)[0] = rec; }
+RT_DEV uint32_t poolGetRec(const float4* pool, int slot) { return reinterpret_cast<const uint32_t*>(pool + slot * POOL_SLOT_F4 + 1)[0]; }
 RT_DEV void waveLdsSync() { __builtin_amdgcn_fence(__ATOMIC_SEQ_CST, "wavefront"); __builtin_amdgcn_wave_barrier(); }
 
 RT_DEV void tracePool(const DevScene& S, float4* pool, bool hasC, bool hasS, uint2* stack, TravCounters& tc)
@@ -618,12 +641,12 @@
   v |= dppU<RT_DPP_HALF_MIRROR>(v);
   return v;
 }
-struct WideCand { float t; uint32_t gid; float u, v; };
+struct WideCand { float t; uint32_t gid; float u, v; uint32_t rec; };
 template <int CTRL> RT_DEV void candMinStep(WideCand& c)
 {
-  const float ot = dppF<CTRL>(c.t); const uint32_t og = dppU<CTRL>(c.gid); const float ou = dppF<CTRL>(c.u), ov = dppF<CTRL>(c.v);
+  const float ot = dppF<CTRL>(c.t); const uint32_t og = dppU<CTRL>(c.gid); const float ou = dppF<CTRL>(c.u), ov = dppF<CTRL>(c.v); const uint32_t orc = dppU<CTRL>(c.rec);
   const bool take = ot < c.t || (ot == c.t && og < c.gid);
-  c.t = take ? ot : c.t; c.gid = take ? og : c.gid; c.u = take ? ou : c.u; c.v = take ? ov : c.v;
+  c.t = take ? ot : c.t; c.gid = take ? og : c.gid; c.u = take ? ou : c.u; c.v = take ? ov : c.v; c.rec = take ? orc : c.rec;
 }
 RT_DEV void groupMinCand(WideCand& c) { candMinStep<RT_DPP_XOR1>(c); candMinStep<RT_DPP_XOR2>(c); candMinStep<RT_DPP_HALF_MIRROR>(c); }
 
@@ -682,7 +705,7 @@
     }
   }
   T.tgroup.y = rem;
-  WideCand c; c.t = __builtin_huge_valf(); c.gid = 0xffffffffu; c.u = 0.0f; c.v = 0.0f;
+  WideCand c; c.t = __builtin_huge_valf(); c.gid = 0xffffffffu; c.u = 0.0f; c.v = 0.0f; c.rec = 0xffffffffu;
   bool ok = false;
 #if RT_WAVEPROF
 #define RT_PH(k) { __builtin_amdgcn_s_waitcnt(0); const uint64_t pn = clock64(); tc.ph[k] += uint32_t(pn - pc); pc = pn; }
@@ -710,13 +733,13 @@
       ok = alphaFinish(A, Fh, a00, a10, a01, a11, gid, T.seed);
       RT_PH(4)
     }
-    if(ok) { c.t = t; c.gid = gid; c.u = u; c.v = v; }
+    if(ok) { c.t = t; c.gid = gid; c.u = u; c.v = v; c.rec = ti; }
   }
   RT_PH(5)
   groupMinCand(c);
   const bool any = c.t < __builtin_huge_valf();
   if(any && (ANY || c.t < T.hit.t || (c.t == T.hit.t && c.gid < T.hit.gid))) {
-    T.hit.t = c.t; T.hit.gid = c.gid; T.hit.u = c.u; T.hit.v = c.v;
+    T.hit.t = c.t; T.hit.gid = c.gid; T.hit.u = c.u; T.hit.v = c.v; T.rec = c.rec;
     T.found = true;
     if(ANY) { T.tgroup.y = 0u; T.ngroup.y = 0u; T.sp = 0; }
   }
@@ -751,7 +774,7 @@
   return live && (travHasTris(T) || travHasNodes(T));
 }
 
-constexpr int GANG_BOX_UINT2 = 16;
+constexpr int GANG_BOX_UINT2 = 20;
 constexpr int GANG_SCAN = 2;
 constexpr int GANG_EXTRA = 20;
 RT_DEV uint32_t leaderBits(unsigned long long m) { return uint32_t(((m & 0x0101010101010101ull) * 0x0102040810204080ull) >> 56); }
@@ -762,10 +785,12 @@
 }
 RT_DEV uint32_t dropTopBits(uint32_t v, int n) { for(int k = 0; k < n; k++) v &= ~(1u << (31 - __clz(int(v)))); return v; }
 
+template <bool REC>
 RT_DEV void gangTail(const DevScene& S, float4* pool, uint2* waveStack, Trav& T, bool& live, int mySlot, TravCounters& tc)
 {
   const int lane = int(threadIdx.x) & 63, j = lane & (WIDE_G - 1), g = lane >> 3;
   float4* gbox = reinterpret_cast<float4*>(waveStack + size_t(S.stackEntries) * WIDE_RAYS);
+  uint32_t* rbox = reinterpret_cast<uint32_t*>(gbox + WIDE_RAYS);
   const int wideRoom = S.stackEntries - S.stackTotal;
   bool working = false;
   int og = g;
@@ -796,12 +821,13 @@
       const float bt = __shfl(T.hit.t, src), bu = __shfl(T.hit.u, src), bv = __shfl(T.hit.v, src);
       const uint32_t bg = uint32_t(__shfl(int(T.hit.gid), src));
       const int any = __shfl(T.isAny ? 1 : 0, src);
+      const uint32_t brc = REC ? uint32_t(__shfl(int(T.rec), src)) : 0xffffffffu;
       if(adopt) {
         const float4 a = pool[slot * POOL_SLOT_F4], b = pool[slot * POOL_SLOT_F4 + 1];
         T.isAny = any != 0;
         (void)travInit<2>(T, mk3(a.x, a.y, a.z), mk3(a.w, b.x, b.y), b.z, rt_f2u(b.w));
         T.ngroup.y = 0u; T.tgroup.y = 0u;
-        T.sp = sp; T.hit.t = bt; T.hit.gid = bg; T.hit.u = bu; T.hit.v = bv;
+        T.sp = sp; T.hit.t = bt; T.hit.gid = bg; T.hit.u = bu; T.hit.v = bv; T.rec = brc;
       }
       working = true;
       wm = 0u;
@@ -812,14 +838,14 @@
     const bool hasTri = working && T.tgroup.y != 0u;
     if(__ballot(hasTri ? 1 : 0) != 0ull) {
       if(hasTri) travTriW<2>(S, T, j, tc);
-      if(j == 0) gbox[g] = make_float4(T.hit.t, rt_u2f(T.hit.gid), T.hit.u, T.hit.v);
+      if(j == 0) { gbox[g] = make_float4(T.hit.t, rt_u2f(T.hit.gid), T.hit.u, T.hit.v); if(REC) rbox[g] = T.rec; }
       waveLdsSync();
       uint32_t rest = wm & ~(1u << g);
       while(rest != 0u) {
         const int k = __ffs(int(rest)) - 1; rest &= rest - 1u;
         const float4 c = gbox[k];
         const uint32_t cg = rt_f2u(c.y);
-        if(cg != 0xffffffffu && (T.hit.gid == 0xffffffffu || (!T.isAny && (c.x < T.hit.t || (c.x == T.hit.t && cg < T.hit.gid))))) { T.hit.t = c.x; T.hit.gid = cg; T.hit.u = c.z; T.hit.v = c.w; }
+        if(cg != 0xffffffffu && (T.hit.gid == 0xffffffffu || (!T.isAny && (c.x < T.hit.t || (c.x == T.hit.t && cg < T.hit.gid))))) { T.hit.t = c.x; T.hit.gid = cg; T.hit.u = c.z; T.hit.v = c.w; if(REC) T.rec = rbox[k]; }
       }
       if(T.isAny && T.hit.gid != 0xffffffffu) { T.sp = 0; T.tgroup.y = 0u; T.ngroup.y = 0u; }
       waveLdsSync();
@@ -872,12 +898,13 @@
     waveLdsSync();
     const uint32_t busyM = leaderBits(__ballot((working && (T.tgroup.y != 0u || T.sp > 0)) ? 1 : 0)) & wm;
     if(working && busyM == 0u) {
-      if(live) { if(j == 0) pool[mySlot * POOL_SLOT_F4] = make_float4(T.hit.t, rt_u2f(T.hit.gid), T.hit.u, T.hit.v); live = false; }
+      if(live) { if(j == 0) { pool[mySlot * POOL_SLOT_F4] = make_float4(T.hit.t, rt_u2f(T.hit.gid), T.hit.u, T.hit.v); if(REC) poolPutRec(pool, mySlot, T.rec); } live = false; }
       working = false;
     }
   }
 }
 
+template <bool REC>
 RT_DEV void tracePoolWide(const DevScene& S, float4* pool, const unsigned char* list, int n, uint32_t* next, uint2* waveStack, TravCounters& tc)
 {
   const int lane = int(threadIdx.x) & 63, j = lane & (WIDE_G - 1), r = lane >> 3;
@@ -903,7 +930,7 @@
         const float4 a = pool[mySlot * POOL_SLOT_F4], b = pool[mySlot * POOL_SLOT_F4 + 1];
         T.isAny = (e & 0x80u) != 0u;
         live = travInit<2>(T, mk3(a.x, a.y, a.z), mk3(a.w, b.x, b.y), b.z, rt_f2u(b.w));
-        if(!live && j == 0) pool[mySlot * POOL_SLOT_F4] = make_float4(T.hit.t, rt_u2f(T.hit.gid), T.hit.u, T.hit.v);
+        if(!live && j == 0) { pool[mySlot * POOL_SLOT_F4] = make_float4(T.hit.t, rt_u2f(T.hit.gid), T.hit.u, T.hit.v); if(REC) poolPutRec(pool, mySlot, T.rec); }
       }
       if(int(base) + nIdle >= n) exhausted = true;
       liveMask = __ballot(live ? 1 : 0);
@@ -913,7 +940,7 @@
       continue;
     }
     if(exhausted && S.gangMax > 0 && __popcll(liveMask & leaders) <= S.gangMax && __popcll(liveMask & leaders) < WIDE_RAYS) {
-      gangTail(S, pool, waveStack, T, live, mySlot, tc);
+      gangTail<REC>(S, pool, waveStack, T, live, mySlot, tc);
       break;
     }
 #if RT_WAVEPROF
@@ -925,7 +952,7 @@
 #if RT_WAVEPROF
     { const uint32_t dc = uint32_t(clock64() - pc0); if(anyTri) { tc.rT++; tc.cT += dc; } else { tc.rN++; tc.cN += dc; } }
 #endif
-    if(live && !still && j == 0) pool[mySlot * POOL_SLOT_F4] = make_float4(T.hit.t, rt_u2f(T.hit.gid), T.hit.u, T.hit.v);
+    if(live && !still && j == 0) { pool[mySlot * POOL_SLOT_F4] = make_float4(T.hit.t, rt_u2f(T.hit.gid), T.hit.u, T.hit.v); if(REC) poolPutRec(pool, mySlot, T.rec); }
     live = still;
   }
 }
```

Result: faster. 1493 (median of 6 runs) (+4.7%).
